# serycjon/MFT

Measured on AMD Instinct MI355X. Metric: tracked frames/sec at 512x512, 12 RAFT iters; flow EPE vs reference, higher is better.
Workload: dtype f32 (update-block products as split fp16 x 3 on the fp16 matrix cores, fp32 accumulation; error per product <= ~2^-23, see DESIGN.md section 4 and parity below); 1 GPU; MFT.track on synthetic 512x512 video, deltas [inf,1,2,4,8,16,32], 7/7.00/7 (min/mean/max) flow pairs per timed frame, 12 RAFT iters, seeded synthetic weights (BASELINE.json configs[1]); parallelism=single GPU, frames_resident_in_hbm=True, preroll_frames=32

## Files before the change

### include/mftx.h

```cpp
#ifndef MFTX_H
#define MFTX_H

#include <stddef.h>
#include <stdint.h>

#ifdef __cplusplus
extern "C" {
#endif

#define MFTX_VERSION 400

#define MFTX_E_ARG (-1)
#define MFTX_E_ALIGN (-2)
#define MFTX_E_WORKSPACE (-3)
#define MFTX_E_STATE (-4)

#define MFTX_MAX_CANDIDATES 16

int mftx_version(void);
const char *mftx_last_error_string(void);

#define MFTX_PROFILE_CATEGORIES 14
int mftx_profile_begin(void);
int mftx_profile_end(double *ms, double *work, long long *count, int n);

int mftx_corr_pyramid(const float *f1, const float *f2, int P, int C, int h, int w,
                      float *lvl0, float *lvl1, float *lvl2, float *lvl3, void *stream);
int mftx_corr_pyramid_split(const float *f1, const float *f2, int P, int C, int h, int w,
                            float *lvl0, float *lvl1, float *lvl2, float *lvl3, float *f2_scratch, void *stream);
int mftx_corr_pyramid_layout(int h, int w, long long *stride, int *block_grid);

int mftx_corr_lookup(const float *lvl0, const float *lvl1, const float *lvl2, const float *lvl3,
                     const float *coords, int P, int h, int w, int r,
                     float *out, int ld_out, void *stream);

#define MFTX_LOOKUP_CONVC1_WEIGHT_BYTES 393216
int mftx_pack_lookup_convc1_weights(const float *wpk, int ld_w, void *wfused, void *stream);
int mftx_corr_lookup_convc1(const float *lvl0, const float *lvl1, const float *lvl2, const float *lvl3,
                            const float *coords, int P, int h, int w, const void *wfused, const float *bias,
                            float *out, int ld_out, int out_split, void *stream);

#define MFTX_FLOW_BRANCH_WEIGHT_BYTES 352256
int mftx_pack_flow_branch_weights(const float *w98, const float *w2pk, void *wflow, void *stream);
int mftx_flow_branch(const float *coords, int P, int h, int w, const void *wflow, const float *b1, const float *b2,
                     float *out, int ld_out, float *hx, int ld_hx, void *stream);

int mftx_fmap_pyramid(const float *f2, int P, int C, int h, int w, float *lvl1, float *lvl2, float *lvl3, void *stream);
int mftx_corr_lookup_ondemand(const float *f1, const float *f2l0, const float *f2l1, const float *f2l2, const float *f2l3,
                              const float *coords, int P, int C, int h, int w, int r,
                              float *out, int ld_out, void *stream);

typedef struct mftx_conv_desc {
    const float *a0; int lda0; int c0;
    const float *a1; int lda1; int c1;
    const float *wpk; const float *bias;
    float *out; int ldo;
    int P, h, w;
    int N;
    int kh, kw;
    int act;
    float out_scale;
    const float *addend; int ld_addend;
    int stride, hin, win, pad_y, pad_x, residual_mode;
    int arith;
    int a_split, out_split;
} mftx_conv_desc;
#define MFTX_ARITH_F32 0
#define MFTX_ARITH_SPLIT 1
int mftx_conv2d(const mftx_conv_desc *d, void *stream);
int mftx_conv2d_tile(const mftx_conv_desc *d, int tile, void *stream);

int mftx_pack_tile_conv_weights(const float *wpk, int N, int taps, int cin, int cin_pad, void *wtile, void *stream);
int mftx_tile_conv2d(const mftx_conv_desc *d, const void *wtile, void *stream);
#define MFTX_OU_HEADS_WTILE_BYTES 6635520
int mftx_pack_ou_heads_weights(const float *w1pk, int cin_pad, const float *w2pk, void *wtile, void *wproj, void *stream);
int mftx_ou_heads(const float *a_split, int lda, int P, int h, int w, const void *wtile, const float *b1, const void *wproj, const float *b2,
                  float *T, float *out, int ld_out, void *stream);
int mftx_gru_half(const float *h_in, int ld_hin, const float *motion, int ld_mo, const void *wzr, const void *wq, const float *pre_zr,
                  const float *pre_q, float *z, const float *hf_in, float *hf_out, float *h_out, int ld_hout, int P, int h, int w, int pass,
                  void *stream);
int mftx_tile_conv_fills_chip(int P, int h, int w);
#define MFTX_FLOW_HEAD_WEIGHT_BYTES 32768
int mftx_pack_flow_head_weights(const float *w2pk, void *wproj, void *stream);
int mftx_flow_head(const float *hsplit, int ld_h, int P, int h, int w, const void *wtile, const float *b1, const void *wproj,
                   const float *b2, float *T, float *delta, float *coords, void *stream);
int mftx_split_weights(const float *wpk, void *out, long long n_floats, void *stream);
#define MFTX_SPLIT_LIMIT 65504.0f
int mftx_count_not_below(const float *x, long long n, float limit, unsigned *count, void *stream);

typedef struct mftx_raft mftx_raft;
#define MFTX_RAFT_NUM_WEIGHTS 34
int mftx_raft_create(const float *const *weights, int n_weights, mftx_raft **out);
void mftx_raft_destroy(mftx_raft *r);
size_t mftx_raft_workspace_bytes(int P, int h, int w);
int mftx_raft_set_ondemand(mftx_raft *r, int on);
int mftx_raft_set_split_weights(mftx_raft *r, const void *const *split, int n);
int mftx_raft_arith(const mftx_raft *r);
int mftx_raft_set_lookup_fused(mftx_raft *r, const void *wfused);
int mftx_raft_set_flow_fused(mftx_raft *r, const void *wflow);
int mftx_raft_set_tile_weights(mftx_raft *r, const void *const *tile, int n);
int mftx_raft_set_flow_head(mftx_raft *r, const void *wproj);
int mftx_raft_set_ou_heads(mftx_raft *r, const void *wtile, const void *wproj);
int mftx_raft_set_coords_trace(mftx_raft *r, float *trace);
#define MFTX_RAFT_OPT_FORK 0
#define MFTX_RAFT_OPT_PRESPLIT 1
#define MFTX_RAFT_OPT_GROUP 2
#define MFTX_RAFT_OPT_FUSE_LOOKUP 3
#define MFTX_RAFT_OPT_GRAPH 4
#define MFTX_RAFT_OPT_FUSE_FLOW 5
#define MFTX_RAFT_OPT_TILE_CONV 6
#define MFTX_RAFT_OPT_FUSE_HEAD 7
#define MFTX_RAFT_OPT_TILE_VOLUME 8
#define MFTX_RAFT_OPT_FUSE_GRU 9
#define MFTX_RAFT_OPT_TILE_CELLS 10
#define MFTX_RAFT_OPT_FUSE_OU 11
#define MFTX_RAFT_OPT_TILE_CONV2P 12
int mftx_raft_set_option(mftx_raft *r, int option, int value);
#define MFTX_RAFT_PLAN_FIELDS 14
#define MFTX_FLOW_FUSED 0
#define MFTX_FLOW_SIDE 1
#define MFTX_FLOW_FIRST 2
#define MFTX_FLOW_AFTER_LOOKUP 3
#define MFTX_FLOW_WITH_LOOKUP 4
int mftx_raft_plan(const mftx_raft *r, int P, int h, int w, int ctx_supplied, int *out, int n);
int mftx_raft_set_nonfinite_counter(mftx_raft *r, unsigned *counter);
int mftx_raft_clear_graphs(mftx_raft *r);
int mftx_raft_graph_stats(const mftx_raft *r, unsigned long long *captures, unsigned long long *replays);
size_t mftx_raft_workspace_bytes_for(const mftx_raft *r, int P, int h, int w);
int mftx_raft_workspace_layout(int P, int h, int w, size_t *offsets, int n);
int mftx_raft_workspace_layout_for(const mftx_raft *r, int P, int h, int w, size_t *offsets, int n);
int mftx_raft_refine(mftx_raft *r, int P, int h, int w, int iters,
                     const float *fmap1, const float *fmap2, const float *net, const float *inp,
                     const float *flow_init,
                     int pad_left, int pad_right, int pad_top, int pad_bottom,
                     float *flow, float *occl, float *sigma, float *packed, float *flow_lr,
                     void *workspace, size_t workspace_bytes, void *stream);
int mftx_raft_refine_gather(mftx_raft *r, int P, int h, int w, int iters, const float *const *fmap1,
                            const float *const *fmap2, const float *const *net, const float *const *inp,
                            const float *flow_init, int pad_left, int pad_right, int pad_top, int pad_bottom,
                            float *flow, float *occl, float *sigma, float *packed, float *flow_lr_out,
                            void *workspace, size_t workspace_bytes, void *stream);
size_t mftx_raft_frame_prepare_bytes(int h, int w);
int mftx_raft_frame_prepare(mftx_raft *r, int h, int w, const float *fmap, const float *inp, float *ctx_zr1, float *ctx_q1,
                            float *ctx_zr2, float *ctx_q2, void *fmap_split, void *scratch, size_t scratch_bytes, void *stream);
int mftx_raft_refine_gather_ex(mftx_raft *r, int P, int h, int w, int iters, const float *const *fmap1,
                               const float *const *fmap2, const float *const *net, const float *const *inp,
                               const float *const *ctx_parts, const void *const *fmap1_split, const void *fmap2_split,
                               const float *flow_init, int pad_left, int pad_right, int pad_top, int pad_bottom,
                               float *flow, float *occl, float *sigma, float *packed, float *flow_lr_out,
                               void *workspace, size_t workspace_bytes, void *stream);
int mftx_volume_query_split(const float *in, void *out, long long n_floats, void *stream);

typedef struct mftx_encoder mftx_encoder;
int mftx_encoder_create(const float *const *weights, int n_weights, int instance_norm, mftx_encoder **out);
int mftx_encoder_set_split_weights(mftx_encoder *e, const void *const *split, int n);
int mftx_encoder_set_graph(mftx_encoder *e, int on);
void mftx_encoder_destroy(mftx_encoder *e);
size_t mftx_encoder_workspace_bytes(int H0, int W0);
int mftx_encoder_forward(mftx_encoder *e, const uint8_t *img, int H0, int W0, float *out0, float *out1,
                         void *workspace, size_t workspace_bytes, void *stream);
int mftx_encoder_prep(const uint8_t *img, int H0, int W0, float *out, void *stream);
size_t mftx_instance_norm_workspace_bytes(int C);
int mftx_instance_norm(float *x, int rows, int C, const float *res, int mode, int split, void *workspace,
                       size_t workspace_bytes, void *stream);

int mftx_convex_upsample(const float *flow_lr, const float *ou, int ld_ou, const float *mask,
                         int P, int h, int w,
                         int pad_left, int pad_right, int pad_top, int pad_bottom,
                         float *flow, float *occl, float *sigma, float *packed, void *stream);

int mftx_chain(const float *flowL, const float *occlL, const float *sigmaL,
               const float *flowR, const float *occlR, const float *sigmaR,
               int H, int W, float *flowO, float *occlO, float *sigmaO, void *stream);

int mftx_warp_backward(const float *flow, const float *img, int C, int H, int W, float *out, void *stream);

int mftx_select(int K, const float *const *flow, const float *const *occl, const float *const *sigma,
                float thr, int H, int W,
                float *flowO, float *occlO, float *sigmaO, int8_t *chosen, void *stream);

int mftx_chain_select(int K,
                      const float *const *flowL, const float *const *occlL, const float *const *sigmaL,
                      const float *const *flowR, const float *const *occlR, const float *const *sigmaR,
                      float thr, int H, int W,
                      float *flowO, float *occlO, float *sigmaO, int8_t *chosen, void *stream);

int mftx_chain_select_packed(int K,
                             const float *const *flowL, const float *const *occlL, const float *const *sigmaL,
                             const float *const *packedR,
                             float thr, int H, int W,
                             float *flowO, float *occlO, float *sigmaO, int8_t *chosen, void *stream);

int mftx_chain_select_multi(int T, const int *K,
                            const float *const *flowL, const float *const *occlL, const float *const *sigmaL,
                            const float *const *packedR,
                            float thr, int H, int W,
                            float *const *flowO, float *const *occlO, float *const *sigmaO, int8_t *const *chosen,
                            void *stream);

int mftx_sample_points(int T, const float *const *flow, const float *const *occl, const float *const *sigma,
                       int H, int W, int N, const int *tmpl, const float *xy,
                       float *table, long long row_stride, int column, void *stream);

#define MFTX_SPLAT_F32 0
#define MFTX_SPLAT_U8 1
int mftx_splat_forward(const float *flow, const void *img, int img_dtype, const uint8_t *mask, int C, int H, int W,
                       int S, int V, long long *acc, void *stream);

int mftx_splat_resolve(long long *acc, int C, int H, int W, int V, float fill, int clear, float *out, void *stream);

int mftx_overlay_edit(const float *flow, const float *occl, const uint8_t *edit, const uint8_t *frame, int H, int W,
                      int S, float alpha_div, long long *acc, uint8_t *out, void *stream);

int mftx_overlay_dots(const uint8_t *frame, uint8_t *out, int H, int W, const float *table, long long row_stride,
                      int N, double radius, int b, int g, int r, void *stream);

size_t mftx_quantize_workspace_bytes(void);
int mftx_quantize_u16(const float *x, long long n, uint16_t *q, float *lohi,
                      void *workspace, size_t workspace_bytes, void *stream);
int mftx_dequantize_u16(const uint16_t *q, long long n, float lo, float hi, float *x, void *stream);

size_t mftx_trackstore_workspace_bytes(void);
int mftx_trackstore_append(const float *flow, const float *occl, const float *sigma, int H, int W,
                           uint16_t *packed, float *lohi, void *workspace, size_t workspace_bytes, void *stream);

size_t mftx_trackstore_append_multi_workspace_bytes(int T);
int mftx_trackstore_append_multi(int T, const float *const *flow, const float *const *occl, const float *const *sigma,
                                 int H, int W, uint16_t *const *packed, float *const *lohi,
                                 void *workspace, size_t workspace_bytes, void *stream);

int mftx_trackstore_unpack(const uint16_t *packed, const float *lohi, int H, int W,
                           float *flow, float *occl, float *sigma, void *stream);

int mftx_trackstore_query(const uint16_t *const *chunks, const float *const *lohi_chunks, int n_chunks, int frames_per_chunk,
                          const int *slots, int T, int H, int W, int N, const float *xy,
                          float *table, long long row_stride, int column0, void *stream);

int mftx_trackstore_locate(const uint16_t *const *frames, const float *const *lohis, const int *group_start, int G,
                           const int *order, const int *group_of, int H, int W, int N, const float *xy,
                           float occlusion_threshold, unsigned long long *keys, float *table, int *cell, void *stream);

int mftx_trackstore_invert(const uint16_t *const *frames, const float *const *lohis, int G, int H, int W,
                           float occlusion_threshold, unsigned long long *keys ,
                           float *table, int *cell, void *stream);

int mftx_trackstore_invert_atlas(const uint16_t *const *frames, const float *const *lohis, const int *first_of ,
                                 const int *rank_of , int G, int J, int H, int W, float occlusion_threshold,
                                 unsigned long long *keys , float *table, int *cell, int *entry, void *stream);

int mftx_trackstore_flow_from(const float *table, const int *entry, const int *row_of, const uint16_t *const *frames,
                              const float *const *lohis, int n_ranks, int R, int T, int H, int W, int columns_per_block,
                              float *flow, float *occl, float *sigma, void *stream);

int mftx_trackstore_flow_from_best(const float *tables, const int *cells, const int *rank_of, const int *row_of,
                                   const uint16_t *const *frames, const float *const *lohis, int E, int R, int T, int H, int W,
                                   float occlusion_threshold, int columns_per_block, float *flow, float *occl, float *sigma,
                                   int *entry, void *stream);

int mftx_copy_bytes(const void *src, void *dst, long long n, void *stream);

int mftx_png_unfilter(uint8_t *rows, int height, int row_bytes, int bpp);

#ifdef __cplusplus
}
#endif
#endif
```

### mft_amd/_lib.py

```python
from __future__ import annotations

import ctypes as C
import os
from pathlib import Path

_HERE = Path(__file__).resolve().parent
LIB_PATH = _HERE / "libmftx.so"

MAX_CANDIDATES = 16
NUM_RAFT_WEIGHTS = 34
LOOKUP_CONVC1_WEIGHT_BYTES = 393216
FLOW_BRANCH_WEIGHT_BYTES = 352256
FLOW_HEAD_WEIGHT_BYTES = 32768
OU_HEADS_WTILE_BYTES = 6635520
SPLIT_LIMIT = 65504.0


class ConvDesc(C.Structure):
    _fields_ = [("a0", C.c_void_p), ("lda0", C.c_int), ("c0", C.c_int),
                ("a1", C.c_void_p), ("lda1", C.c_int), ("c1", C.c_int),
                ("wpk", C.c_void_p), ("bias", C.c_void_p),
                ("out", C.c_void_p), ("ldo", C.c_int),
                ("P", C.c_int), ("h", C.c_int), ("w", C.c_int),
                ("N", C.c_int), ("kh", C.c_int), ("kw", C.c_int),
                ("act", C.c_int), ("out_scale", C.c_float),
                ("addend", C.c_void_p), ("ld_addend", C.c_int),
                ("stride", C.c_int), ("hin", C.c_int), ("win", C.c_int), ("pad_y", C.c_int), ("pad_x", C.c_int),
                ("residual_mode", C.c_int), ("arith", C.c_int), ("a_split", C.c_int), ("out_split", C.c_int)]


_PP = C.POINTER(C.c_void_p)

SIGNATURES = {
    "mftx_version": (C.c_int, []),
    "mftx_last_error_string": (C.c_char_p, []),
    "mftx_profile_begin": (C.c_int, []),
    "mftx_profile_end": (C.c_int, [C.POINTER(C.c_double), C.POINTER(C.c_double), C.POINTER(C.c_longlong), C.c_int]),
    "mftx_corr_pyramid": (C.c_int, [C.c_void_p, C.c_void_p, C.c_int, C.c_int, C.c_int, C.c_int,
                                    C.c_void_p, C.c_void_p, C.c_void_p, C.c_void_p, C.c_void_p]),
    "mftx_corr_pyramid_split": (C.c_int, [C.c_void_p, C.c_void_p, C.c_int, C.c_int, C.c_int, C.c_int,
                                          C.c_void_p, C.c_void_p, C.c_void_p, C.c_void_p, C.c_void_p, C.c_void_p]),
    "mftx_corr_pyramid_layout": (C.c_int, [C.c_int, C.c_int, C.POINTER(C.c_longlong), C.POINTER(C.c_int)]),
    "mftx_corr_lookup": (C.c_int, [C.c_void_p] * 5 + [C.c_int] * 4 + [C.c_void_p, C.c_int, C.c_void_p]),
    "mftx_fmap_pyramid": (C.c_int, [C.c_void_p] + [C.c_int] * 4 + [C.c_void_p] * 4),
    "mftx_corr_lookup_ondemand": (C.c_int, [C.c_void_p] * 6 + [C.c_int] * 5 + [C.c_void_p, C.c_int, C.c_void_p]),
    "mftx_raft_set_ondemand": (C.c_int, [C.c_void_p, C.c_int]),
    "mftx_raft_workspace_bytes_for": (C.c_size_t, [C.c_void_p, C.c_int, C.c_int, C.c_int]),
    "mftx_conv2d": (C.c_int, [C.POINTER(ConvDesc), C.c_void_p]),
    "mftx_conv2d_tile": (C.c_int, [C.POINTER(ConvDesc), C.c_int, C.c_void_p]),
    "mftx_encoder_set_split_weights": (C.c_int, [C.c_void_p, _PP, C.c_int]),
    "mftx_raft_set_split_weights": (C.c_int, [C.c_void_p, _PP, C.c_int]),
    "mftx_raft_arith": (C.c_int, [C.c_void_p]),
    "mftx_raft_set_lookup_fused": (C.c_int, [C.c_void_p, C.c_void_p]),
    "mftx_raft_set_flow_fused": (C.c_int, [C.c_void_p, C.c_void_p]),
    "mftx_raft_set_tile_weights": (C.c_int, [C.c_void_p, _PP, C.c_int]),
    "mftx_raft_set_flow_head": (C.c_int, [C.c_void_p, C.c_void_p]),
    "mftx_raft_set_ou_heads": (C.c_int, [C.c_void_p, C.c_void_p, C.c_void_p]),
    "mftx_pack_ou_heads_weights": (C.c_int, [C.c_void_p, C.c_int, C.c_void_p, C.c_void_p, C.c_void_p, C.c_void_p]),
    "mftx_ou_heads": (C.c_int, [C.c_void_p, C.c_int, C.c_int, C.c_int, C.c_int, C.c_void_p, C.c_void_p, C.c_void_p, C.c_void_p, C.c_void_p,
                                C.c_void_p, C.c_int, C.c_void_p]),
    "mftx_pack_flow_head_weights": (C.c_int, [C.c_void_p, C.c_void_p, C.c_void_p]),
    "mftx_flow_head": (C.c_int, [C.c_void_p, C.c_int, C.c_int, C.c_int, C.c_int] + [C.c_void_p] * 8),
    "mftx_pack_tile_conv_weights": (C.c_int, [C.c_void_p, C.c_int, C.c_int, C.c_int, C.c_int, C.c_void_p, C.c_void_p]),
    "mftx_tile_conv2d": (C.c_int, [C.POINTER(ConvDesc), C.c_void_p, C.c_void_p]),
    "mftx_pack_flow_branch_weights": (C.c_int, [C.c_void_p, C.c_void_p, C.c_void_p, C.c_void_p]),
    "mftx_flow_branch": (C.c_int, [C.c_void_p, C.c_int, C.c_int, C.c_int, C.c_void_p, C.c_void_p, C.c_void_p, C.c_void_p,
                                   C.c_int, C.c_void_p, C.c_int, C.c_void_p]),
    "mftx_raft_set_option": (C.c_int, [C.c_void_p, C.c_int, C.c_int]),
    "mftx_raft_plan": (C.c_int, [C.c_void_p, C.c_int, C.c_int, C.c_int, C.c_int, C.POINTER(C.c_int), C.c_int]),
    "mftx_raft_set_coords_trace": (C.c_int, [C.c_void_p, C.c_void_p]),
    "mftx_gru_half": (C.c_int, [C.c_void_p, C.c_int, C.c_void_p, C.c_int, C.c_void_p, C.c_void_p, C.c_void_p, C.c_void_p, C.c_void_p, C.c_void_p,
                                C.c_void_p, C.c_void_p, C.c_int, C.c_int, C.c_int, C.c_int, C.c_int, C.c_void_p]),
    "mftx_tile_conv_fills_chip": (C.c_int, [C.c_int, C.c_int, C.c_int]),
    "mftx_raft_clear_graphs": (C.c_int, [C.c_void_p]),
    "mftx_raft_set_nonfinite_counter": (C.c_int, [C.c_void_p, C.c_void_p]),
    "mftx_raft_graph_stats": (C.c_int, [C.c_void_p, C.POINTER(C.c_ulonglong), C.POINTER(C.c_ulonglong)]),
    "mftx_pack_lookup_convc1_weights": (C.c_int, [C.c_void_p, C.c_int, C.c_void_p, C.c_void_p]),
    "mftx_corr_lookup_convc1": (C.c_int, [C.c_void_p] * 5 + [C.c_int] * 3 + [C.c_void_p, C.c_void_p, C.c_void_p,
                                                                            C.c_int, C.c_int, C.c_void_p]),
    "mftx_split_weights": (C.c_int, [C.c_void_p, C.c_void_p, C.c_longlong, C.c_void_p]),
    "mftx_count_not_below": (C.c_int, [C.c_void_p, C.c_longlong, C.c_float, C.c_void_p, C.c_void_p]),
    "mftx_raft_create": (C.c_int, [_PP, C.c_int, C.POINTER(C.c_void_p)]),
    "mftx_raft_destroy": (None, [C.c_void_p]),
    "mftx_raft_workspace_bytes": (C.c_size_t, [C.c_int, C.c_int, C.c_int]),
    "mftx_raft_workspace_layout": (C.c_int, [C.c_int, C.c_int, C.c_int, C.POINTER(C.c_size_t), C.c_int]),
    "mftx_raft_workspace_layout_for": (C.c_int, [C.c_void_p, C.c_int, C.c_int, C.c_int, C.POINTER(C.c_size_t), C.c_int]),
    "mftx_raft_refine": (C.c_int, [C.c_void_p, C.c_int, C.c_int, C.c_int, C.c_int,
                                   C.c_void_p, C.c_void_p, C.c_void_p, C.c_void_p, C.c_void_p,
                                   C.c_int, C.c_int, C.c_int, C.c_int,
                                   C.c_void_p, C.c_void_p, C.c_void_p, C.c_void_p, C.c_void_p,
                                   C.c_void_p, C.c_size_t, C.c_void_p]),
    "mftx_raft_refine_gather": (C.c_int, [C.c_void_p, C.c_int, C.c_int, C.c_int, C.c_int,
                                          _PP, _PP, _PP, _PP, C.c_void_p,
                                          C.c_int, C.c_int, C.c_int, C.c_int,
                                          C.c_void_p, C.c_void_p, C.c_void_p, C.c_void_p, C.c_void_p,
                                          C.c_void_p, C.c_size_t, C.c_void_p]),
    "mftx_raft_refine_gather_ex": (C.c_int, [C.c_void_p, C.c_int, C.c_int, C.c_int, C.c_int,
                                             _PP, _PP, _PP, _PP, _PP, _PP, C.c_void_p, C.c_void_p,
                                             C.c_int, C.c_int, C.c_int, C.c_int,
                                             C.c_void_p, C.c_void_p, C.c_void_p, C.c_void_p, C.c_void_p,
                                             C.c_void_p, C.c_size_t, C.c_void_p]),
    "mftx_raft_frame_prepare_bytes": (C.c_size_t, [C.c_int, C.c_int]),
    "mftx_raft_frame_prepare": (C.c_int, [C.c_void_p, C.c_int, C.c_int] + [C.c_void_p] * 8 + [C.c_size_t, C.c_void_p]),
    "mftx_volume_query_split": (C.c_int, [C.c_void_p, C.c_void_p, C.c_longlong, C.c_void_p]),
    "mftx_encoder_create": (C.c_int, [_PP, C.c_int, C.c_int, C.POINTER(C.c_void_p)]),
    "mftx_encoder_destroy": (None, [C.c_void_p]),
    "mftx_encoder_set_graph": (C.c_int, [C.c_void_p, C.c_int]),
    "mftx_encoder_workspace_bytes": (C.c_size_t, [C.c_int, C.c_int]),
    "mftx_encoder_forward": (C.c_int, [C.c_void_p, C.c_void_p, C.c_int, C.c_int, C.c_void_p, C.c_void_p,
                                       C.c_void_p, C.c_size_t, C.c_void_p]),
    "mftx_encoder_prep": (C.c_int, [C.c_void_p, C.c_int, C.c_int, C.c_void_p, C.c_void_p]),
    "mftx_instance_norm_workspace_bytes": (C.c_size_t, [C.c_int]),
    "mftx_instance_norm": (C.c_int, [C.c_void_p, C.c_int, C.c_int, C.c_void_p, C.c_int, C.c_int, C.c_void_p, C.c_size_t, C.c_void_p]),
    "mftx_convex_upsample": (C.c_int, [C.c_void_p, C.c_void_p, C.c_int, C.c_void_p] + [C.c_int] * 7
                             + [C.c_void_p] * 5),
    "mftx_chain": (C.c_int, [C.c_void_p] * 6 + [C.c_int, C.c_int] + [C.c_void_p] * 4),
    "mftx_warp_backward": (C.c_int, [C.c_void_p, C.c_void_p, C.c_int, C.c_int, C.c_int, C.c_void_p, C.c_void_p]),
    "mftx_select": (C.c_int, [C.c_int, _PP, _PP, _PP, C.c_float, C.c_int, C.c_int] + [C.c_void_p] * 5),
    "mftx_chain_select": (C.c_int, [C.c_int] + [_PP] * 6 + [C.c_float, C.c_int, C.c_int] + [C.c_void_p] * 5),
    "mftx_chain_select_packed": (C.c_int, [C.c_int] + [_PP] * 4 + [C.c_float, C.c_int, C.c_int] + [C.c_void_p] * 5),
    "mftx_chain_select_multi": (C.c_int, [C.c_int, C.POINTER(C.c_int)] + [_PP] * 4 + [C.c_float, C.c_int, C.c_int] + [_PP] * 4
                                + [C.c_void_p]),
    "mftx_sample_points": (C.c_int, [C.c_int, _PP, _PP, _PP, C.c_int, C.c_int, C.c_int, C.c_void_p, C.c_void_p,
                                     C.c_void_p, C.c_longlong, C.c_int, C.c_void_p]),
    "mftx_splat_forward": (C.c_int, [C.c_void_p, C.c_void_p, C.c_int, C.c_void_p, C.c_int, C.c_int, C.c_int, C.c_int, C.c_int,
                                     C.c_void_p, C.c_void_p]),
    "mftx_splat_resolve": (C.c_int, [C.c_void_p, C.c_int, C.c_int, C.c_int, C.c_int, C.c_float, C.c_int, C.c_void_p, C.c_void_p]),
    "mftx_overlay_edit": (C.c_int, [C.c_void_p, C.c_void_p, C.c_void_p, C.c_void_p, C.c_int, C.c_int, C.c_int, C.c_float,
                                    C.c_void_p, C.c_void_p, C.c_void_p]),
    "mftx_overlay_dots": (C.c_int, [C.c_void_p, C.c_void_p, C.c_int, C.c_int, C.c_void_p, C.c_longlong, C.c_int, C.c_double,
                                    C.c_int, C.c_int, C.c_int, C.c_void_p]),
    "mftx_quantize_workspace_bytes": (C.c_size_t, []),
    "mftx_quantize_u16": (C.c_int, [C.c_void_p, C.c_longlong, C.c_void_p, C.c_void_p, C.c_void_p, C.c_size_t, C.c_void_p]),
    "mftx_dequantize_u16": (C.c_int, [C.c_void_p, C.c_longlong, C.c_float, C.c_float, C.c_void_p, C.c_void_p]),
    "mftx_trackstore_workspace_bytes": (C.c_size_t, []),
    "mftx_trackstore_append": (C.c_int, [C.c_void_p, C.c_void_p, C.c_void_p, C.c_int, C.c_int, C.c_void_p, C.c_void_p,
                                         C.c_void_p, C.c_size_t, C.c_void_p]),
    "mftx_trackstore_append_multi_workspace_bytes": (C.c_size_t, [C.c_int]),
    "mftx_trackstore_append_multi": (C.c_int, [C.c_int, _PP, _PP, _PP, C.c_int, C.c_int, _PP, _PP, C.c_void_p, C.c_size_t,
                                               C.c_void_p]),
    "mftx_trackstore_invert_atlas": (C.c_int, [C.c_void_p, C.c_void_p, C.c_void_p, C.c_void_p, C.c_int, C.c_int, C.c_int, C.c_int,
                                               C.c_float, C.c_void_p, C.c_void_p, C.c_void_p, C.c_void_p, C.c_void_p]),
    "mftx_trackstore_flow_from": (C.c_int, [C.c_void_p, C.c_void_p, C.c_void_p, C.c_void_p, C.c_void_p, C.c_int, C.c_int, C.c_int,
                                            C.c_int, C.c_int, C.c_int, C.c_void_p, C.c_void_p, C.c_void_p, C.c_void_p]),
    "mftx_trackstore_flow_from_best": (C.c_int, [C.c_void_p] * 6 + [C.c_int] * 5 + [C.c_float, C.c_int] + [C.c_void_p] * 5),
    "mftx_trackstore_unpack": (C.c_int, [C.c_void_p, C.c_void_p, C.c_int, C.c_int, C.c_void_p, C.c_void_p, C.c_void_p,
                                         C.c_void_p]),
    "mftx_trackstore_query": (C.c_int, [_PP, _PP, C.c_int, C.c_int, C.c_void_p, C.c_int, C.c_int, C.c_int, C.c_int, C.c_void_p,
                                        C.c_void_p, C.c_longlong, C.c_int, C.c_void_p]),
    "mftx_trackstore_locate": (C.c_int, [C.c_void_p, C.c_void_p, C.c_void_p, C.c_int, C.c_void_p, C.c_void_p, C.c_int, C.c_int,
                                         C.c_int, C.c_void_p, C.c_float, C.c_void_p, C.c_void_p, C.c_void_p, C.c_void_p]),
    "mftx_trackstore_invert": (C.c_int, [C.c_void_p, C.c_void_p, C.c_int, C.c_int, C.c_int, C.c_float, C.c_void_p, C.c_void_p,
                                         C.c_void_p, C.c_void_p]),
    "mftx_png_unfilter":(C.c_int, [C.c_void_p, C.c_int, C.c_int, C.c_int]),
    "mftx_copy_bytes": (C.c_int, [C.c_void_p, C.c_void_p, C.c_longlong, C.c_void_p]),
}

_lib = None


class MftxError(RuntimeError):
    pass


def load():
    global _lib
    if _lib is not None:
        return _lib
    path = Path(os.environ.get("MFTX_LIB", LIB_PATH))
    if not path.exists():
        raise MftxError(f"{path} not found: build it with `python -c 'import __graft_entry__ as g; g.build()'` "
                        "(there is no CPU fallback for the MFT hot path)")
    lib = C.CDLL(str(path))
    for name, (res, args) in SIGNATURES.items():
        fn = getattr(lib, name)
        fn.restype = res
        fn.argtypes = args
    _lib = lib
    return lib


def check(code, what):
    if code != 0:
        msg = load().mftx_last_error_string().decode(errors="replace")
        raise MftxError(f"{what} failed ({code}): {msg}")


def ptr_array(ptrs):
    arr = (C.c_void_p * len(ptrs))(*ptrs)
    return C.cast(arr, _PP), arr
```

### mft_amd/csrc/common.h

```cpp
#pragma once
#include <hip/hip_runtime.h>
#include <cstdarg>
#include <cstdio>
#include <cstdint>
#include <cstdlib>
#include "../../include/mftx.h"

namespace mftx {

void set_error(const char *fmt, ...);

inline int fail(int code, const char *fmt, ...) {
    char buf[512];
    va_list ap;
    va_start(ap, fmt);
    vsnprintf(buf, sizeof buf, fmt, ap);
    va_end(ap);
    set_error("%s", buf);
    return code;
}

inline int check_launch(const char *what) {
    hipError_t e = hipGetLastError();
    if (e != hipSuccess) {
        set_error("%s: %s", what, hipGetErrorString(e));
        return (int)e;
    }
    return 0;
}

inline int tune_env(const char *name, int dflt) {
#ifdef MFTX_TUNING
    const char *e = getenv(name);
    return e ? atoi(e) : dflt;
#else
    (void)name;
    return dflt;
#endif
}

inline bool aligned16(const void *p) { return (reinterpret_cast<uintptr_t>(p) & 15u) == 0; }
inline int cdiv(int a, int b) { return (a + b - 1) / b; }
inline int round_up(int a, int b) { return cdiv(a, b) * b; }

struct PyramidLayout {
    int h[4], w[4];
    int hb[2], wb[2];
    int sbh, sbw;
    long long stride[4];
};
inline PyramidLayout pyramid_layout(int h, int w) {
    PyramidLayout L;
    for (int l = 0; l < 4; ++l) { L.h[l] = h >> l; L.w[l] = w >> l; }
    L.sbh = (h + 7) / 8; L.sbw = (w + 15) / 16;
    L.hb[0] = 2 * L.sbh; L.wb[0] = 2 * L.sbw; L.hb[1] = L.sbh; L.wb[1] = L.sbw;
    L.stride[0] = (long long)L.hb[0] * L.wb[0] * 32;
    L.stride[1] = (long long)L.hb[1] * L.wb[1] * 32;
    L.stride[2] = ((long long)L.h[2] * L.w[2] + 3) / 4 * 4;
    L.stride[3] = ((long long)L.h[3] * L.w[3] + 3) / 4 * 4;
    return L;
}

__host__ __device__ inline int split_row_offset(int c) { return (c >> 3) * 32 + (c & 7) * 2; }
#ifdef __HIPCC__
__device__ __forceinline__ unsigned split_halves(float v) {
    const _Float16 h = (_Float16)v;
    const _Float16 l = (_Float16)((v - (float)h) * 2048.f);
    return (unsigned)__builtin_bit_cast(unsigned short, h) | ((unsigned)__builtin_bit_cast(unsigned short, l) << 16);
}
__device__ __forceinline__ void store_split_pairwise(float *row, int c, float v, bool store) {
    const unsigned mine = split_halves(v);
    const unsigned other = (unsigned)__shfl_xor((int)mine, 1);
    const bool odd = (c & 1) != 0;
    const unsigned word = odd ? ((other >> 16) | (mine & 0xffff0000u)) : ((mine & 0xffffu) | (other << 16));
    char *dst = reinterpret_cast<char *>(row) + split_row_offset(c & ~1) + (odd ? 16 : 0);
    if (store) *reinterpret_cast<unsigned *>(dst) = word;
}
__device__ __forceinline__ float4 load_split4(const float *row, int c) {
    const char *src = reinterpret_cast<const char *>(row) + split_row_offset(c);
    const uint2 h = *reinterpret_cast<const uint2 *>(src), l = *reinterpret_cast<const uint2 *>(src + 16);
    auto dec = [](unsigned hh, unsigned ll, int hi) {
        const _Float16 a = __builtin_bit_cast(_Float16, (unsigned short)(hi ? hh >> 16 : hh));
        const _Float16 b = __builtin_bit_cast(_Float16, (unsigned short)(hi ? ll >> 16 : ll));
        return (float)a + (float)b * (1.f / 2048.f);
    };
    return make_float4(dec(h.x, l.x, 0), dec(h.x, l.x, 1), dec(h.y, l.y, 0), dec(h.y, l.y, 1));
}
__device__ __forceinline__ void store_split4v(float *row, int c, float4 v) {
    const unsigned a = split_halves(v.x), b = split_halves(v.y), cc = split_halves(v.z), d = split_halves(v.w);
    char *dst = reinterpret_cast<char *>(row) + split_row_offset(c);
    *reinterpret_cast<uint2 *>(dst) = make_uint2((a & 0xffffu) | (b << 16), (cc & 0xffffu) | (d << 16));
    *reinterpret_cast<uint2 *>(dst + 16) = make_uint2((a >> 16) | (b & 0xffff0000u), (cc >> 16) | (d & 0xffff0000u));
}
#endif
__host__ __device__ inline float relu_keep_nan(float v) { return v < 0.f ? 0.f : v; }
int launch_conv(const mftx_conv_desc &d, hipStream_t s, int tile = -1);
int launch_conv_pair(const mftx_conv_desc &a, const mftx_conv_desc &b, hipStream_t s);
struct GruEpilogue {
    int mode;
    float *hx;
    int ld_hx;
    float *z;
    float *rh;
    float *hf = nullptr;
    int ld_hf = 0;
};
int launch_conv_gru(const mftx_conv_desc &d, const GruEpilogue &g, hipStream_t s);
int launch_split_weights(const float *wpk, void *out, long long n_floats, hipStream_t s);
bool conv_small_applicable(const mftx_conv_desc &d);
int launch_conv_small(const mftx_conv_desc &d, hipStream_t s, float *accum = nullptr, int ld_accum = 0);
int launch_corr_pyramid(const float *f1, const float *f2, int P, int C, int h, int w, float *const lvl[4], hipStream_t s,
                        float *f2_split = nullptr, int tile_resident = 1);
bool volume_tile_applicable(int C);
constexpr int MFTX_MAX_GATHER = 16;
struct PairPtrs { const float *p[MFTX_MAX_GATHER]; };
int launch_volume_tile(const float *f1, const float *f2s, int P, int h, int w, float *const lvl[4], hipStream_t s,
                       const PairPtrs *f1p = nullptr, long long f2_bstride = -1, bool f1_split = false);
int launch_volume_query_split(const float *in, void *out, long long n_floats, hipStream_t s);
int launch_corr_lookup(const float *const lvl[4], const float *coords, int P, int h, int w,
                       float *out, int ld_out, hipStream_t s);
int launch_pack_lookup_convc1(const float *w, int ld_w, void *out, hipStream_t s);
bool lookup_convc1_applicable(int P, int h, int w, int ld_out);
int launch_lookup_convc1(const float *const lvl[4], const float *coords, int P, int h, int w, const void *wf,
                         const float *bias, float *out, int ld_out, int out_split, hipStream_t s);
int launch_pack_flow_branch(const float *w98, const float *w2pk, void *out, hipStream_t s);
int launch_flow_branch(const float *coords, int P, int h, int w, const void *wf, const float *b1, const float *b2, float *out,
                       int ld_out, float *hx, int ld_hx, hipStream_t s, const float *T = nullptr, const float *b2h = nullptr,
                       float *coords_out = nullptr, float *delta_out = nullptr);
struct TileConvLaunch {
    const float *a0; int lda0;
    const float *a1; int lda1;
    int cin;
    const void *wf;
    const float *bias;
    const float *addend; int ld_addend;
    float *out; int ldo; int out_split;
    float *z, *rh, *hf, *hx; int ld_hf, ld_hx;
    const void *wproj; float *tout;
    int P, h, w, N, kh, kw, epi;
    int cells;
};
struct GruHalfLaunch {
    const float *h_in; int ld_hin; const float *mo; int ld_mo;
    const void *wzr, *wq;
    const float *pre_zr, *pre_q;
    const float *const *ctx;
    float *z; const float *hf_in; float *hf_out;
    float *h_out; int ld_hout;
    int P, h, w, pass;
    int cells;
};
int launch_gru_half(const GruHalfLaunch &d, hipStream_t s);
int launch_pack_flow_head(const float *w2pk, void *out, hipStream_t s);
int launch_pack_tile_conv2p(const float *wpk, int N, int cin_pad, void *out, hipStream_t s);
int launch_tile_conv2p(const float *a, int lda, const void *wf, const float *bias, float *out, int ldo, int n_valid, int P, int h, int w, int cells,
                       hipStream_t s);
constexpr size_t OU_HEAD_WTILE_BYTES = 8ull * 5 * 9 * 9 * 128 * 16, OU_HEAD_WPROJ_BYTES = 32768;
int launch_pack_ou_head(const float *w1pk, int cin_pad, const float *w2pk, void *wtile, void *wproj, hipStream_t s);
struct OuGather { const float *hx, *corr; int ld_corr; const float *coords1, *delta; float *flow_lr; };
int launch_ou_heads(const float *a, int lda, int P, int h, int w, const void *wtile, const float *b1, const void *wproj, const float *b2, float *T,
                    float *out, int ld_out, int cells, hipStream_t s, const OuGather *ga = nullptr);
int launch_flow_head_sum(const float *T, const float *b2, float *delta, const float *coords_in, float *coords_out, int P, int h, int w, hipStream_t s);
bool tile_conv_applicable(int kh, int kw, int cin, int N);
bool tile_conv_small_tiles_fill(int P, int h, int w);
bool tile_conv_fills_chip(int P, int h, int w, int kh, int kw);
int launch_pack_tile_conv(const float *wpk, int N, int taps, int cin, int cin_pad, void *out, hipStream_t s);
int launch_tile_conv(const TileConvLaunch &d, hipStream_t s);
int launch_fmap_pyramid(const float *f2, int P, int C, int h, int w, float *const lvl[3], hipStream_t s);
int launch_corr_ondemand(const float *f1, const float *const f2lvl[4], const float *coords, int P, int h, int w,
                         float *out, int ld_out, hipStream_t s);
int launch_convex_upsample(const float *flow_lr, const float *ou, int ld_ou, const float *mask,
                           int P, int h, int w, int pl, int pr, int pt, int pb,
                           float *flow, float *occl, float *sigma, float *packed, hipStream_t s, unsigned *nonfinite = nullptr);

}
```

### mft_amd/csrc/raft_engine.hip

```cpp
#include "common.h"
#include "profile.h"
#include "motion_front.h"
#include "graph_cache.h"
#include <cstdlib>
#include <new>

namespace mftx {


struct InitGather { int on; PairPtrs netp, inpp; };
struct CtxTable { const float **table; const float *own[4]; int supplied; PairPtrs parts[4]; };
__global__ void init_state_kernel(const float *__restrict__ net, const float *__restrict__ inp,
                                  const float *__restrict__ flow_init, float *hx, float *hf, float *coords1, int M, int h,
                                  int w, InitGather ga, CtxTable ct) {
    const long long i = (long long)blockIdx.x * blockDim.x + threadIdx.x;
    if (i >= (long long)M * 64) return;
    if (ct.table != nullptr && i < (long long)(M / (h * w)) * 4) {
        const int b = (int)(i >> 2), k = (int)(i & 3);
        ct.table[i] = ct.supplied ? ct.parts[k].p[b] : ct.own[k] + (long long)b * h * w * ((k & 1) ? 128 : 256);
    }
    const int m = (int)(i >> 6), q = (int)(i & 63);
    if (ga.on) {
        const int b = m / (h * w);
        net = ga.netp.p[b] - (long long)b * h * w * 128;
        inp = ga.inpp.p[b] - (long long)b * h * w * 128;
    }
    const float4 v = (q < 32) ? reinterpret_cast<const float4 *>(net)[(long long)m * 32 + q]
                              : reinterpret_cast<const float4 *>(inp)[(long long)m * 32 + (q - 32)];
    if (hf != nullptr) {
        store_split4v(hx + (long long)m * 384, 4 * q, v);
        if (q < 32) reinterpret_cast<float4 *>(hf + (long long)m * 128)[q] = v;
    } else {
        reinterpret_cast<float4 *>(hx + (long long)m * 384)[q] = v;
    }
    if (q == 0) {
        const int rem = m % (h * w);
        float cx = (float)(rem % w), cy = (float)(rem / w);
        if (flow_init != nullptr) {
            cx += flow_init[2 * (long long)m];
            cy += flow_init[2 * (long long)m + 1];
        }
        coords1[2 * (long long)m] = cx;
        coords1[2 * (long long)m + 1] = cy;
    }
}

__global__ __launch_bounds__(256) void convf1_kernel(ConvF1Args q) {
    __shared__ __attribute__((aligned(16))) float patch[2][7][48];
    const int half = threadIdx.x >> 7;
    convf1_strip(q, blockIdx.x * 2 + half, patch[half], threadIdx.x & 127);
}

__global__ __launch_bounds__(256) void lookup_convf1_kernel(LookupArgs lp, ConvF1Args q, int lookup_blocks, int f1_blocks) {
    __shared__ __attribute__((aligned(16))) float patch[2][7][48];
    const int total = lookup_blocks + f1_blocks;
    const int b = blockIdx.x;
    const int f_lo = (int)((long long)b * f1_blocks / total), f_hi = (int)((long long)(b + 1) * f1_blocks / total);
    if (f_hi > f_lo) {
        const int half = threadIdx.x >> 7;
        convf1_strip(q, f_lo * 2 + half, patch[half], threadIdx.x & 127);
    } else {
        lookup_block_body<2>(lp, b - f_lo, lookup_blocks);
    }
}

__global__ void ou_gather_kernel(const float *__restrict__ hx, const float *__restrict__ corr, int ld_corr,
                                 const float *__restrict__ coords1, const float *__restrict__ delta,
                                 float *__restrict__ ouin, float *__restrict__ flow_lr, int M, int h, int w, int split) {
    const long long i = (long long)blockIdx.x * blockDim.x + threadIdx.x;
    if (i >= (long long)M * 178) return;
    const int m = (int)(i / 178), q = (int)(i - (long long)m * 178);
    float4 v;
    if (split) {
        if (q < 64) v = load_split4(hx + (long long)m * 384, 4 * q);
        else if (q < 145) v = reinterpret_cast<const float4 *>(corr + (long long)m * ld_corr)[q - 64];
        else if (q == 145) {
            const int rem = m % (h * w);
            const float fx = coords1[2 * (long long)m] - (float)(rem % w);
            const float fy = coords1[2 * (long long)m + 1] - (float)(rem / w);
            v = make_float4(fx, fy, delta[2 * (long long)m], delta[2 * (long long)m + 1]);
            flow_lr[2 * (long long)m] = fx;
            flow_lr[2 * (long long)m + 1] = fy;
        } else v = load_split4(hx + (long long)m * 384 + 256, 4 * (q - 146));
        store_split4v(ouin + (long long)m * 712, 4 * q, v);
        return;
    }
    if (q < 64) v = reinterpret_cast<const float4 *>(hx + (long long)m * 384)[q];
    else if (q < 145) v = reinterpret_cast<const float4 *>(corr + (long long)m * ld_corr)[q - 64];
    else if (q == 145) {
        const int rem = m % (h * w);
        const float fx = coords1[2 * (long long)m] - (float)(rem % w);
        const float fy = coords1[2 * (long long)m + 1] - (float)(rem / w);
        v = make_float4(fx, fy, delta[2 * (long long)m], delta[2 * (long long)m + 1]);
        flow_lr[2 * (long long)m] = fx;
        flow_lr[2 * (long long)m + 1] = fy;
    } else v = reinterpret_cast<const float4 *>(hx + (long long)m * 384 + 256)[q - 146];
    reinterpret_cast<float4 *>(ouin + (long long)m * 712)[q] = v;
}

enum WeightSlot {
    W_CONVC1, B_CONVC1, W_CONVC2, B_CONVC2, W_CONVF1, B_CONVF1, W_CONVF2, B_CONVF2, W_CONV, B_CONV,
    W_ZR1_DYN, W_ZR1_INP, B_ZR1, W_Q1_DYN, W_Q1_INP, B_Q1, W_ZR2_DYN, W_ZR2_INP, B_ZR2, W_Q2_DYN, W_Q2_INP, B_Q2,
    W_FH1, B_FH1, W_FH2, B_FH2, W_MASK0, B_MASK0, W_MASK2, B_MASK2,
    W_OU1, B_OU1, W_OU2, B_OU2, W_COUNT
};

struct Workspace {
    float *lvl[4];
    float *f2l[3];
    float *coords1, *corr, *cor1, *corflo, *flo1, *hx, *z, *rh, *fh, *delta, *mask, *ouin, *ouh, *ou, *flow_lr;
    float *pre_zr[2], *pre_q[2];
    float *f2s;
    float *hf;
    float *hb, *hfb;
    const float **ctx;
    int ld_corr;
    size_t bytes;
};

static Workspace carve(void *base, int P, int h, int w, bool ondemand = false, bool split = false) {
    Workspace ws{};
    const size_t N = (size_t)h * w, M = (size_t)P * N;
    size_t off = 0;
    auto take = [&](size_t floats) {
        float *p = base ? reinterpret_cast<float *>(static_cast<char *>(base) + off) : nullptr;
        off += (floats * sizeof(float) + 255) & ~size_t(255);
        return p;
    };
    const PyramidLayout L = pyramid_layout(h, w);
    for (int l = 0; l < 4; ++l) ws.lvl[l] = take(ondemand ? 0 : M * (size_t)L.stride[l]);
    for (int l = 1; l < 4; ++l) ws.f2l[l - 1] = take(ondemand ? (size_t)P * (h >> l) * (w >> l) * 256 : 0);
    ws.coords1 = take(M * 2);
    ws.ld_corr = 324;
    ws.corr = take(M * ws.ld_corr);
    ws.cor1 = take(M * 256);
    ws.corflo = take(M * 256);
    ws.flo1 = take(M * 128);
    ws.hx = take(M * 384);
    ws.z = take(M * 128);
    ws.rh = take(M * 128);
    ws.fh = take(M * 256);
    ws.delta = take(M * 2);
    ws.mask = take(M * 576);
    ws.ouin = take(M * 712);
    ws.ouh = take(M * 256);
    ws.ou = take(M * 4);
    ws.flow_lr = take(M * 2);
    for (int pass = 0; pass < 2; ++pass) { ws.pre_zr[pass] = take(M * 256); ws.pre_q[pass] = take(M * 128); }
    ws.f2s = take(ondemand || !split ? 0 : M * 256);
    ws.hf = take(split ? M * 128 : 0);
    ws.hb = take(split ? M * 128 : 0);
    ws.hfb = take(split ? M * 128 : 0);
    ws.ctx = reinterpret_cast<const float **>(take(split ? (size_t)P * 8 : 0));
    ws.bytes = off;
    return ws;
}

}

using namespace mftx;

static constexpr uint32_t RAFT_MAGIC = 0x4d465458;
struct mftx_raft {
    uint32_t magic = RAFT_MAGIC;
    int ondemand = 0;
    int arith = MFTX_ARITH_F32;
    const float *w[W_COUNT] = {};
    const float *wg[W_COUNT] = {};
    hipStream_t side = nullptr;
    hipEvent_t ev_fork = nullptr, ev_join = nullptr;
    float *coords_trace = nullptr;
    GraphCache *graphs = nullptr;
    const void *wfused = nullptr;
    const void *wflow = nullptr;
    const void *wproj = nullptr;
    const void *wt[W_COUNT] = {};
    const void *wou = nullptr, *wouproj = nullptr;
    int opt[13] = { -1,  1,  1,  1,  1,  1,  1,
                    1,  1,  1,  0,  1,  1};
    unsigned *nonfinite = nullptr;
};
static_assert(MFTX_RAFT_OPT_TILE_CONV2P == 12, "mftx_raft::opt lists one default per option");
static constexpr int GEMM_SLOTS[] = {W_CONVC1, W_CONVC2, W_CONVF2, W_CONV, W_ZR1_DYN, W_ZR1_INP, W_Q1_DYN, W_Q1_INP,
                                     W_ZR2_DYN, W_ZR2_INP, W_Q2_DYN, W_Q2_INP, W_FH1, W_MASK0, W_MASK2, W_OU1};

extern "C" int mftx_raft_create(const float *const *weights, int n_weights, mftx_raft **out) {
    if (!weights || !out) return fail(MFTX_E_ARG, "raft_create: null pointer");
    if (n_weights != W_COUNT) return fail(MFTX_E_ARG, "raft_create: expected %d weight tensors, got %d", (int)W_COUNT, n_weights);
    for (int i = 0; i < W_COUNT; ++i) {
        if (!weights[i]) return fail(MFTX_E_ARG, "raft_create: weight %d is null", i);
        if (!aligned16(weights[i])) return fail(MFTX_E_ALIGN, "raft_create: weight %d not 16-byte aligned", i);
    }
    mftx_raft *r = new (std::nothrow) mftx_raft;
    if (!r) return fail(MFTX_E_ARG, "raft_create: out of host memory");
    r->graphs = new (std::nothrow) GraphCache;
    for (int i = 0; i < W_COUNT; ++i) r->w[i] = r->wg[i] = weights[i];
    *out = r;
    return 0;
}

extern "C" void mftx_raft_destroy(mftx_raft *r) {
    if (r && r->magic == RAFT_MAGIC) {
        r->magic = 0;
        if (r->ev_fork) (void)hipEventDestroy(r->ev_fork);
        if (r->ev_join) (void)hipEventDestroy(r->ev_join);
        if (r->side) (void)hipStreamDestroy(r->side);
        delete r->graphs;
        delete r;
    }
}

static int ensure_side_stream(mftx_raft *r) {
    if (r->side) return 0;
    hipError_t e = hipStreamCreateWithFlags(&r->side, hipStreamNonBlocking);
    if (e == hipSuccess) e = hipEventCreateWithFlags(&r->ev_fork, hipEventDisableTiming);
    if (e == hipSuccess) e = hipEventCreateWithFlags(&r->ev_join, hipEventDisableTiming);
    if (e != hipSuccess) return fail((int)e, "raft_refine: side stream: %s", hipGetErrorString(e));
    return 0;
}

extern "C" size_t mftx_raft_workspace_bytes(int P, int h, int w) {
    if (P <= 0 || h <= 0 || w <= 0) return 0;
    return carve(nullptr, P, h, w).bytes;
}

extern "C" int mftx_raft_set_ondemand(mftx_raft *r, int on) {
    if (!r || r->magic != RAFT_MAGIC) return fail(MFTX_E_STATE, "raft_set_ondemand: bad handle");
    r->ondemand = on ? 1 : 0;
    if (r->graphs) r->graphs->clear();
    return 0;
}

extern "C" int mftx_raft_set_split_weights(mftx_raft *r, const void *const *split, int n) {
    if (!r || r->magic != RAFT_MAGIC) return fail(MFTX_E_STATE, "raft_set_split_weights: bad handle");
    if (r->graphs) r->graphs->clear();
    if (!split) {
        for (int i = 0; i < W_COUNT; ++i) r->wg[i] = r->w[i];
        r->arith = MFTX_ARITH_F32;
        return 0;
    }
    if (n != W_COUNT) return fail(MFTX_E_ARG, "raft_set_split_weights: expected %d slots, got %d", (int)W_COUNT, n);
    for (int slot : GEMM_SLOTS) {
        if (!split[slot]) return fail(MFTX_E_ARG, "raft_set_split_weights: slot %d (a GEMM layer) is null", slot);
        if (!aligned16(split[slot])) return fail(MFTX_E_ALIGN, "raft_set_split_weights: slot %d not 16-byte aligned", slot);
    }
    for (int slot : GEMM_SLOTS) r->wg[slot] = static_cast<const float *>(split[slot]);
    r->arith = MFTX_ARITH_SPLIT;
    return 0;
}

extern "C" int mftx_raft_set_lookup_fused(mftx_raft *r, const void *wfused) {
    if (!r || r->magic != RAFT_MAGIC) return fail(MFTX_E_STATE, "raft_set_lookup_fused: bad handle");
    if (wfused && !aligned16(wfused)) return fail(MFTX_E_ALIGN, "raft_set_lookup_fused: weights not 16-byte aligned");
    r->wfused = wfused;
    if (r->graphs) r->graphs->clear();
    return 0;
}

extern "C" int mftx_raft_set_flow_fused(mftx_raft *r, const void *wflow) {
    if (!r || r->magic != RAFT_MAGIC) return fail(MFTX_E_STATE, "raft_set_flow_fused: bad handle");
    if (wflow && !aligned16(wflow)) return fail(MFTX_E_ALIGN, "raft_set_flow_fused: weights not 16-byte aligned");
    r->wflow = wflow;
    if (r->graphs) r->graphs->clear();
    return 0;
}

extern "C" int mftx_raft_set_tile_weights(mftx_raft *r, const void *const *tile, int n) {
    if (!r || r->magic != RAFT_MAGIC) return fail(MFTX_E_STATE, "raft_set_tile_weights: bad handle");
    if (r->graphs) r->graphs->clear();
    if (!tile) { for (int i = 0; i < W_COUNT; ++i) r->wt[i] = nullptr; return 0; }
    if (n != W_COUNT) return fail(MFTX_E_ARG, "raft_set_tile_weights: expected %d slots, got %d", (int)W_COUNT, n);
    for (int i = 0; i < W_COUNT; ++i)
        if (tile[i] && !aligned16(tile[i])) return fail(MFTX_E_ALIGN, "raft_set_tile_weights: slot %d not 16-byte aligned", i);
    for (int i = 0; i < W_COUNT; ++i) r->wt[i] = tile[i];
    return 0;
}

extern "C" int mftx_raft_set_flow_head(mftx_raft *r, const void *wproj) {
    if (!r || r->magic != RAFT_MAGIC) return fail(MFTX_E_STATE, "raft_set_flow_head: bad handle");
    if (wproj && !aligned16(wproj)) return fail(MFTX_E_ALIGN, "raft_set_flow_head: weights not 16-byte aligned");
    r->wproj = wproj;
    if (r->graphs) r->graphs->clear();
    return 0;
}

extern "C" int mftx_raft_set_ou_heads(mftx_raft *r, const void *wtile, const void *wproj) {
    if (!r || r->magic != RAFT_MAGIC) return fail(MFTX_E_STATE, "raft_set_ou_heads: bad handle");
    if ((wtile == nullptr) != (wproj == nullptr)) return fail(MFTX_E_ARG, "raft_set_ou_heads: both weight streams, or neither");
    if (wtile && (!aligned16(wtile) || !aligned16(wproj))) return fail(MFTX_E_ALIGN, "raft_set_ou_heads: weights not 16-byte aligned");
    r->wou = wtile; r->wouproj = wproj;
    if (r->graphs) r->graphs->clear();
    return 0;
}

extern "C" int mftx_raft_set_coords_trace(mftx_raft *r, float *trace) {
    if (!r || r->magic != RAFT_MAGIC) return fail(MFTX_E_STATE, "raft_set_coords_trace: bad handle");
    r->coords_trace = trace;
    return 0;
}

extern "C" int mftx_raft_clear_graphs(mftx_raft *r) {
    if (!r || r->magic != RAFT_MAGIC) return fail(MFTX_E_STATE, "raft_clear_graphs: bad handle");
    if (r->graphs) r->graphs->clear();
    return 0;
}

extern "C" int mftx_raft_set_nonfinite_counter(mftx_raft *r, unsigned *counter) {
    if (!r || r->magic != RAFT_MAGIC) return fail(MFTX_E_STATE, "raft_set_nonfinite_counter: bad handle");
    if (counter && (reinterpret_cast<uintptr_t>(counter) & 3)) return fail(MFTX_E_ALIGN, "raft_set_nonfinite_counter: counter not 4-byte aligned");
    r->nonfinite = counter;
    return 0;
}

extern "C" int mftx_raft_set_option(mftx_raft *r, int option, int value) {
    if (!r || r->magic != RAFT_MAGIC) return fail(MFTX_E_STATE, "raft_set_option: bad handle");
    if (option < 0 || option > MFTX_RAFT_OPT_TILE_CONV2P) return fail(MFTX_E_ARG, "raft_set_option: unknown option %d", option);
    r->opt[option] = value;
    if (r->graphs) r->graphs->clear();
    return 0;
}

extern "C" int mftx_raft_arith(const mftx_raft *r) {
    return (r && r->magic == RAFT_MAGIC) ? r->arith : -1;
}

extern "C" size_t mftx_raft_workspace_bytes_for(const mftx_raft *r, int P, int h, int w) {
    if (!r || r->magic != RAFT_MAGIC || P <= 0 || h <= 0 || w <= 0) return 0;
    return carve(nullptr, P, h, w, r->ondemand != 0, r->arith == MFTX_ARITH_SPLIT).bytes;
}

static int workspace_layout(const mftx_raft *r, int P, int h, int w, size_t *offsets, int n) {
    if (P <= 0 || h <= 0 || w <= 0 || !offsets || n != 19) return fail(MFTX_E_ARG, "workspace_layout: need 19 slots");
    char *base = reinterpret_cast<char *>(uintptr_t(1) << 40);
    Workspace ws = carve(base, P, h, w, r && r->ondemand != 0, r && r->arith == MFTX_ARITH_SPLIT);
    float *ptrs[19] = {ws.lvl[0], ws.lvl[1], ws.lvl[2], ws.lvl[3], ws.coords1, ws.corr, ws.cor1, ws.corflo, ws.flo1,
                       ws.hx, ws.z, ws.rh, ws.fh, ws.delta, ws.mask, ws.ouin, ws.ouh, ws.ou, ws.flow_lr};
    for (int i = 0; i < 19; ++i) offsets[i] = (size_t)(reinterpret_cast<char *>(ptrs[i]) - base);
    return 0;
}
extern "C" int mftx_raft_workspace_layout(int P, int h, int w, size_t *offsets, int n) {
    return workspace_layout(nullptr, P, h, w, offsets, n);
}
extern "C" int mftx_raft_workspace_layout_for(const mftx_raft *r, int P, int h, int w, size_t *offsets, int n) {
    if (!r || r->magic != RAFT_MAGIC) return fail(MFTX_E_STATE, "workspace_layout_for: bad handle");
    return workspace_layout(r, P, h, w, offsets, n);
}

#define TRY(expr) do { int _e = (expr); if (_e) return _e; } while (0)

enum FlowSchedule { FLOW_FUSED = MFTX_FLOW_FUSED, FLOW_SIDE = MFTX_FLOW_SIDE, FLOW_FIRST = MFTX_FLOW_FIRST, FLOW_AFTER_LOOKUP = MFTX_FLOW_AFTER_LOOKUP,
                    FLOW_WITH_LOOKUP = MFTX_FLOW_WITH_LOOKUP };

struct RefinePlan {
    bool SP, fuse_lookup, tiles_on, gru_fused, ctx_supplied, two_pass;
    FlowSchedule flow;
    bool pair_second;
    bool head_fused, defer_update, ou_fused, ou_materialised, use_graph, side_stream;
};

static RefinePlan refine_plan(const mftx_raft &r, int P, int h, int w, bool gather_has_ctx, bool prof, bool trace) {
    const int *opt = r.opt;
    const bool split = r.arith == MFTX_ARITH_SPLIT, ondemand = r.ondemand != 0;
    RefinePlan p{};
    p.SP = split && opt[MFTX_RAFT_OPT_PRESPLIT] != 0;
    p.fuse_lookup = p.SP && !ondemand && r.wfused != nullptr && opt[MFTX_RAFT_OPT_FUSE_LOOKUP] != 0 && lookup_convc1_applicable(P, h, w, 256);
    p.tiles_on = p.SP && opt[MFTX_RAFT_OPT_TILE_CONV] != 0 && (opt[MFTX_RAFT_OPT_TILE_CONV] == 2 ||
                 (tile_conv_fills_chip(P, h, w, 3, 3) && tile_conv_fills_chip(P, h, w, 1, 5) && tile_conv_fills_chip(P, h, w, 5, 1)));
    auto tile_w = [&](int slot) { return p.tiles_on && r.wt[slot] != nullptr; };
    p.gru_fused = tile_w(W_ZR1_DYN) && tile_w(W_Q1_DYN) && tile_w(W_ZR2_DYN) && tile_w(W_Q2_DYN) && opt[MFTX_RAFT_OPT_FUSE_GRU] != 0;
    p.ctx_supplied = gather_has_ctx && p.gru_fused;
    p.two_pass = p.tiles_on && opt[MFTX_RAFT_OPT_TILE_CONV2P] != 0 && r.wt[W_CONVC2] && r.wt[W_CONV];
    const bool grouped = opt[MFTX_RAFT_OPT_GROUP] != 0;
    const int fork = opt[MFTX_RAFT_OPT_FORK];
    const bool fuse_flow = p.SP && r.wflow != nullptr && opt[MFTX_RAFT_OPT_FUSE_FLOW] != 0 && grouped;
    const bool serial = fuse_flow || prof || !grouped || (split && (fork == 0 || fork == 2));
    const bool forked = !serial && split;
    const bool flow_first = !fuse_flow && serial && p.fuse_lookup && fork == 2 && !prof && grouped;
    const bool lookup_alone = p.fuse_lookup || prof || !grouped || ondemand;
    p.flow = fuse_flow ? FLOW_FUSED : forked ? FLOW_SIDE : flow_first ? FLOW_FIRST : lookup_alone ? FLOW_AFTER_LOOKUP : FLOW_WITH_LOOKUP;
    p.pair_second = !forked && grouped && r.arith == MFTX_ARITH_F32;
    p.head_fused = tile_w(W_FH1) && r.wproj != nullptr && opt[MFTX_RAFT_OPT_FUSE_HEAD] != 0;
    p.defer_update = p.head_fused && fuse_flow && opt[MFTX_RAFT_OPT_FUSE_HEAD] != 2 && !trace;
    p.ou_fused = p.tiles_on && r.wou != nullptr && opt[MFTX_RAFT_OPT_FUSE_OU] != 0;
    p.ou_materialised = !p.ou_fused || opt[MFTX_RAFT_OPT_FUSE_OU] == 2;
    p.use_graph = r.graphs && opt[MFTX_RAFT_OPT_GRAPH] != 0 && !prof && !trace && !ondemand;
    p.side_stream = split && fork != 0;
    return p;
}

extern "C" int mftx_raft_plan(const mftx_raft *r, int P, int h, int w, int ctx_supplied, int *out, int n) {
    if (!r || r->magic != RAFT_MAGIC) return fail(MFTX_E_STATE, "raft_plan: bad handle");
    if (P <= 0 || h <= 0 || w <= 0) return fail(MFTX_E_ARG, "raft_plan: need P, h, w >= 1");
    if (!out || n != MFTX_RAFT_PLAN_FIELDS) return fail(MFTX_E_ARG, "raft_plan: need %d slots", MFTX_RAFT_PLAN_FIELDS);
    const RefinePlan p = refine_plan(*r, P, h, w, ctx_supplied != 0, prof_enabled(), r->coords_trace != nullptr);
    const int v[MFTX_RAFT_PLAN_FIELDS] = {p.SP, p.fuse_lookup, p.tiles_on, p.gru_fused, p.ctx_supplied, p.two_pass, (int)p.flow, p.pair_second,
                                          p.head_fused, p.defer_update, p.ou_fused, p.ou_materialised, p.use_graph, p.side_stream};
    for (int i = 0; i < n; ++i) out[i] = v[i];
    return 0;
}

struct RefineGather { PairPtrs f1, f2, net, inp; bool f2_shared; bool has_ctx, has_f1s; PairPtrs ctx[4], f1s; const float *f2s; };

struct Coords { float *cur, *alt; bool pending; };
struct Seg { const float *p; int ld, c; };
struct Out { float *p; int ld, N; };
enum { ACT_NONE, ACT_RELU, ACT_GRU_ZR, ACT_GRU_Q };

struct RefineCall {
    mftx_raft *r;
    const float *const *W, *const *G;
    RefinePlan plan;
    hipStream_t s;
    int P, h, w, iters;
    Workspace ws;
    const float *lv[4];
    const float *fmap1, *f2lv[4];
    float *flow_lr;

    mftx_conv_desc conv_desc(Seg a0, Seg a1, const float *wpk, const float *bias, Out out, int kh, int kw, int act) const {
        mftx_conv_desc d{};
        d.a0 = a0.p; d.lda0 = a0.ld; d.c0 = a0.c; d.a1 = a1.p; d.lda1 = a1.ld; d.c1 = a1.c;
        d.wpk = wpk; d.bias = bias; d.out = out.p; d.ldo = out.ld; d.N = out.N; d.P = P; d.h = h; d.w = w;
        d.kh = kh; d.kw = kw; d.act = act; d.out_scale = 1.f;
        return d;
    }
    mftx_conv_desc gemm(mftx_conv_desc d, bool a = true, bool o = false) const {
        d.arith = r->arith; d.a_split = plan.SP && a; d.out_split = plan.SP && o; return d;
    }
    TileConvLaunch tile_launch(int slot, const float *bias, Seg a0, Seg a1, int N, int kh, int kw, int epi) const {
        TileConvLaunch t{};
        t.a0 = a0.p; t.lda0 = a0.ld; t.a1 = a1.p; t.lda1 = a1.ld; t.cin = a1.p ? 256 : 128; t.wf = r->wt[slot]; t.bias = bias;
        t.P = P; t.h = h; t.w = w; t.N = N; t.kh = kh; t.kw = kw; t.epi = epi;
        t.cells = r->opt[MFTX_RAFT_OPT_TILE_CELLS];
        return t;
    }
    int conv_layer(int slot, const float *bias, Seg a0, Seg a1, Out out, int kh, int kw, int act, bool out_split, const GruEpilogue *g = nullptr,
                   const float *addend = nullptr, int ld_addend = 0) const {
        if (plan.tiles_on && r->wt[slot]) {
            TileConvLaunch t = tile_launch(slot, bias, a0, a1, out.N, kh, kw, act);
            t.addend = addend; t.ld_addend = ld_addend;
            if (!g) { t.out = out.p; t.ldo = out.ld; t.out_split = out_split ? 1 : 0; }
            else {
                t.z = g->z; t.hf = g->hf; t.ld_hf = g->ld_hf;
                if (act == ACT_GRU_ZR) t.rh = g->rh; else { t.hx = g->hx; t.ld_hx = g->ld_hx; }
            }
            return launch_tile_conv(t, s);
        }
        mftx_conv_desc d = gemm(conv_desc(a0, a1, G[slot], bias, out, kh, kw, act), true, out_split);
        d.addend = addend; d.ld_addend = ld_addend;
        return g ? launch_conv_gru(d, *g, s) : launch_conv(d, s);
    }
    int context_parts(const float *inp, int ld, float *const zr[2], float *const q[2]) const {
        for (int pass = 0; pass < 2; ++pass) {
            const int kh = pass ? 5 : 1, kw = pass ? 1 : 5;
            TRY(conv_layer(pass ? W_ZR2_INP : W_ZR1_INP, W[pass ? B_ZR2 : B_ZR1], Seg{inp, ld, 128}, Seg{}, Out{zr[pass], 256, 256}, kh, kw, ACT_NONE, false));
            TRY(conv_layer(pass ? W_Q2_INP : W_Q1_INP, W[pass ? B_Q2 : B_Q1], Seg{inp, ld, 128}, Seg{}, Out{q[pass], 128, 128}, kh, kw, ACT_NONE, false));
        }
        return 0;
    }
    int volume(const float *fmap2, const RefineGather *gather) const {
        if (r->ondemand) return launch_fmap_pyramid(fmap2, P, 256, h, w, ws.f2l, s);
        if (!gather) return launch_corr_pyramid(fmap1, fmap2, P, 256, h, w, ws.lvl, s, r->arith == MFTX_ARITH_SPLIT ? ws.f2s : nullptr, r->opt[MFTX_RAFT_OPT_TILE_VOLUME]);
        const long long pair_floats = (long long)h * w * 256;
        const float *f2s = ws.f2s;
        if (gather->f2_shared && gather->f2s) f2s = gather->f2s;
        else if (gather->f2_shared) TRY(launch_split_weights(gather->f2.p[0], ws.f2s, pair_floats, s));
        else for (int b = 0; b < P; ++b) TRY(launch_split_weights(gather->f2.p[b], ws.f2s + b * pair_floats, pair_floats, s));
        return launch_volume_tile(nullptr, f2s, P, h, w, ws.lvl, s, gather->has_f1s ? &gather->f1s : &gather->f1, gather->f2_shared ? 0 : pair_floats,
                                  gather->has_f1s);
    }
    int init_state(const float *net, const float *inp, const float *flow_init, const RefineGather *gather) const {
        const int M = P * h * w;
        const long long slots = (long long)M * 64;
        ProfScope prof(PC_GLUE, s, 0);
        InitGather ga{};
        if (gather) { ga.on = 1; ga.netp = gather->net; ga.inpp = gather->inp; }
        CtxTable ct{};
        if (plan.gru_fused) {
            ct.table = ws.ctx;
            ct.own[0] = ws.pre_zr[0]; ct.own[1] = ws.pre_q[0]; ct.own[2] = ws.pre_zr[1]; ct.own[3] = ws.pre_q[1];
            ct.supplied = plan.ctx_supplied ? 1 : 0;
            if (plan.ctx_supplied) for (int k = 0; k < 4; ++k) ct.parts[k] = gather->ctx[k];
        }
        hipLaunchKernelGGL(init_state_kernel, dim3((unsigned)((slots + 255) / 256)), dim3(256), 0, s, net, inp,
                           flow_init, ws.hx, plan.SP ? ws.hf : nullptr, ws.coords1, M, h, w, ga, ct);
        return check_launch("init_state");
    }
    int conv256(int slot, const float *bias, const float *in, Out out, const mftx_conv_desc *pair = nullptr) const {
        if (plan.two_pass) return launch_tile_conv2p(in, 256, r->wt[slot], bias, out.p, out.ld, out.N, P, h, w, r->opt[MFTX_RAFT_OPT_TILE_CELLS], s);
        const mftx_conv_desc d = gemm(conv_desc(Seg{in, 256, 256}, Seg{}, G[slot], bias, out, 3, 3, ACT_RELU), true, true);
        return pair ? launch_conv_pair(d, *pair, s) : launch_conv(d, s);
    }
    int corr_branch(const float *coords, bool last, const ConvF1Args *f1 = nullptr, int f1_blocks = 0, const mftx_conv_desc *pair = nullptr) const {
        if (plan.flow == FLOW_WITH_LOOKUP) {
            const LookupArgs la = make_lookup_args(lv, coords, P, h, w, ws.corr, ws.ld_corr);
            const int lookup_blocks = cdiv(cdiv(la.cells, 2), LK_WAVES);
            hipLaunchKernelGGL(lookup_convf1_kernel, dim3(lookup_blocks + f1_blocks), dim3(256), 0, s, la, *f1, lookup_blocks, f1_blocks);
        } else {
            if (plan.fuse_lookup) {
                if (last && plan.flow != FLOW_SIDE) TRY(launch_corr_lookup(lv, coords, P, h, w, ws.corr, ws.ld_corr, s));
                TRY(launch_lookup_convc1(lv, coords, P, h, w, r->wfused, W[B_CONVC1], ws.cor1, 256, 1, s));
            } else if (r->ondemand) TRY(launch_corr_ondemand(fmap1, f2lv, coords, P, h, w, ws.corr, ws.ld_corr, s));
            else TRY(launch_corr_lookup(lv, coords, P, h, w, ws.corr, ws.ld_corr, s));
            if (f1) {
                ProfScope prof(PC_CONVF1, s, 2.0 * P * h * w * 128 * 98);
                hipLaunchKernelGGL(convf1_kernel, dim3(f1_blocks), dim3(256), 0, s, *f1);
            }
        }
        TRY(check_launch("lookup + convf1"));
        if (!plan.fuse_lookup)
            TRY(launch_conv(gemm(conv_desc(Seg{ws.corr, ws.ld_corr, ws.ld_corr}, Seg{}, G[W_CONVC1], W[B_CONVC1], Out{ws.cor1, 256, 256}, 1, 1, ACT_RELU), false, true), s));
        return conv256(W_CONVC2, W[B_CONVC2], ws.cor1, Out{ws.corflo, 256, 192}, pair);
    }
    int motion_encoder(Coords &x, bool last) const {
        const int strips = cdiv(w, F1_CELLS);
        const ConvF1Args f1{x.cur, W[W_CONVF1], W[B_CONVF1], ws.flo1, ws.hx, h, w, strips, P * h * strips, plan.SP ? 1 : 0};
        const int f1_blocks = cdiv(f1.n_strips, 2);
        const Out flo{ws.corflo + 192, 256, 64};
        const mftx_conv_desc f2 = gemm(conv_desc(Seg{ws.flo1, 128, 128}, Seg{}, G[W_CONVF2], W[B_CONVF2], flo, 3, 3, ACT_RELU), true, true);
        switch (plan.flow) {
        case FLOW_FUSED:
            if (x.pending) {
                TRY(launch_flow_branch(x.cur, P, h, w, r->wflow, W[B_CONVF1], W[B_CONVF2], flo.p, flo.ld, ws.hx, 384, s, ws.fh, W[B_FH2], x.alt, ws.delta));
                x = Coords{x.alt, x.cur, false};
            } else TRY(launch_flow_branch(x.cur, P, h, w, r->wflow, W[B_CONVF1], W[B_CONVF2], flo.p, flo.ld, ws.hx, 384, s));
            TRY(corr_branch(x.cur, last));
            break;
        case FLOW_SIDE:
            TRY(ensure_side_stream(r));
            if (hipEventRecord(r->ev_fork, s) != hipSuccess || hipStreamWaitEvent(r->side, r->ev_fork, 0) != hipSuccess)
                return fail(MFTX_E_STATE, "raft_refine: fork onto the side stream failed");
            hipLaunchKernelGGL(convf1_kernel, dim3(f1_blocks), dim3(256), 0, r->side, f1);
            TRY(check_launch("convf1"));
            TRY(launch_conv(f2, r->side));
            if (plan.fuse_lookup && last) TRY(launch_corr_lookup(lv, x.cur, P, h, w, ws.corr, ws.ld_corr, r->side));
            if (hipEventRecord(r->ev_join, r->side) != hipSuccess) return fail(MFTX_E_STATE, "raft_refine: join event failed");
            TRY(corr_branch(x.cur, last));
            if (hipStreamWaitEvent(s, r->ev_join, 0) != hipSuccess) return fail(MFTX_E_STATE, "raft_refine: join failed");
            break;
        case FLOW_FIRST:
            hipLaunchKernelGGL(convf1_kernel, dim3(f1_blocks), dim3(256), 0, s, f1);
            TRY(check_launch("convf1"));
            TRY(launch_conv(f2, s));
            TRY(corr_branch(x.cur, last));
            break;
        case FLOW_AFTER_LOOKUP: case FLOW_WITH_LOOKUP:
            TRY(corr_branch(x.cur, last, &f1, f1_blocks, plan.pair_second ? &f2 : nullptr));
            if (!plan.pair_second) TRY(launch_conv(f2, s));
            break;
        }
        return conv256(W_CONV, W[B_CONV], ws.corflo, Out{ws.hx + 256, 384, 126});
    }
    int gru() const {
        for (int pass = 0; pass < 2; ++pass) {
            const int kh = pass ? 5 : 1, kw = pass ? 1 : 5;
            const int szr = pass ? W_ZR2_DYN : W_ZR1_DYN, sq = pass ? W_Q2_DYN : W_Q1_DYN;
            if (plan.gru_fused) {
                GruHalfLaunch g{};
                g.h_in = pass ? ws.hb : ws.hx; g.ld_hin = pass ? 128 : 384; g.h_out = pass ? ws.hx : ws.hb; g.ld_hout = pass ? 384 : 128;
                g.mo = ws.hx + 256; g.ld_mo = 384; g.wzr = r->wt[szr]; g.wq = r->wt[sq]; g.pre_zr = ws.pre_zr[pass]; g.pre_q = ws.pre_q[pass]; g.ctx = ws.ctx;
                g.z = ws.z; g.hf_in = pass ? ws.hfb : ws.hf; g.hf_out = pass ? ws.hf : ws.hfb; g.P = P; g.h = h; g.w = w; g.pass = pass; g.cells = r->opt[MFTX_RAFT_OPT_TILE_CELLS];
                TRY(launch_gru_half(g, s));
                continue;
            }
            const Seg motion{ws.hx + 256, 384, 128};
            const GruEpilogue g1{1, ws.hx, 384, ws.z, ws.rh, plan.SP ? ws.hf : nullptr, 128}, g2{2, ws.hx, 384, ws.z, ws.rh, plan.SP ? ws.hf : nullptr, 128};
            TRY(conv_layer(szr, nullptr, Seg{ws.hx, 384, 128}, motion, Out{ws.z, 128, 256}, kh, kw, ACT_GRU_ZR, true, &g1, ws.pre_zr[pass], 256));
            TRY(conv_layer(sq, nullptr, Seg{ws.rh, 128, 128}, motion, Out{ws.hx, 384, 128}, kh, kw, ACT_GRU_Q, true, &g2, ws.pre_q[pass], 128));
        }
        return 0;
    }
    int flow_head(Coords &x, bool last) const {
        const Seg hidden{ws.hx, 384, 128};
        if (plan.head_fused) {
            TileConvLaunch t = tile_launch(W_FH1, W[B_FH1], hidden, Seg{}, 256, 3, 3, 4);
            t.wproj = r->wproj; t.tout = ws.fh;
            TRY(launch_tile_conv(t, s));
            if (!last && plan.defer_update) { x.pending = true; return 0; }
            float *dst = last ? ws.coords1 : x.cur;
            TRY(launch_flow_head_sum(ws.fh, W[B_FH2], ws.delta, x.cur, dst, P, h, w, s));
            x.cur = dst;
            return 0;
        }
        TRY(conv_layer(W_FH1, W[B_FH1], hidden, Seg{}, Out{ws.fh, 256, 256}, 3, 3, ACT_RELU, false));
        const mftx_conv_desc fh2 = conv_desc(Seg{ws.fh, 256, 256}, Seg{}, W[W_FH2], W[B_FH2], Out{ws.delta, 2, 2}, 3, 3, ACT_NONE);
        if (!conv_small_applicable(fh2)) return fail(MFTX_E_STATE, "raft_refine: flow-head layer does not fit the small-N kernel");
        return launch_conv_small(fh2, s, x.cur, 2);
    }
    int final_heads(const float *coords) const {
        const int M = P * h * w;
        TRY(conv_layer(W_MASK0, W[B_MASK0], Seg{ws.hx, 384, 128}, Seg{}, Out{ws.fh, 256, 256}, 3, 3, ACT_RELU, true));
        mftx_conv_desc mask2 = gemm(conv_desc(Seg{ws.fh, 256, 256}, Seg{}, G[W_MASK2], W[B_MASK2], Out{ws.mask, 576, 576}, 1, 1, ACT_NONE));
        mask2.out_scale = 0.25f;
        TRY(launch_conv(mask2, s));
        if (plan.ou_materialised) {
            const long long slots = (long long)M * 178;
            ProfScope prof(PC_GLUE, s, 0);
            hipLaunchKernelGGL(ou_gather_kernel, dim3((unsigned)((slots + 255) / 256)), dim3(256), 0, s, ws.hx,
                               ws.corr, ws.ld_corr, coords, ws.delta, ws.ouin, flow_lr, M, h, w, plan.SP ? 1 : 0);
            TRY(check_launch("ou_gather"));
        }
        if (plan.ou_fused) {
            const OuGather ga{ws.hx, ws.corr, ws.ld_corr, coords, ws.delta, flow_lr};
            return launch_ou_heads(plan.ou_materialised ? ws.ouin : nullptr, 712, P, h, w, r->wou, W[B_OU1], r->wouproj, W[B_OU2], ws.ouh, ws.ou, 4, r->opt[MFTX_RAFT_OPT_TILE_CELLS], s,
                                   plan.ou_materialised ? nullptr : &ga);
        }
        TRY(launch_conv(gemm(conv_desc(Seg{ws.ouin, 712, 712}, Seg{}, G[W_OU1], W[B_OU1], Out{ws.ouh, 256, 256}, 3, 3, ACT_RELU)), s));
        return launch_conv(conv_desc(Seg{ws.ouh, 256, 256}, Seg{}, W[W_OU2], W[B_OU2], Out{ws.ou, 4, 3}, 3, 3, ACT_NONE), s);
    }
    int core() const {
        const size_t n = (size_t)P * h * w * 2;
        float *trace = r->coords_trace;
        if (!plan.ctx_supplied) TRY(context_parts(ws.hx + 128, 384, ws.pre_zr, ws.pre_q));
        Coords x{ws.coords1, ws.flo1, false};
        for (int it = 0; it < iters; ++it) {
            const bool last = (it == iters - 1);
            if (trace && hipMemcpyAsync(trace + it * n, x.cur, n * 4, hipMemcpyDeviceToDevice, s) != hipSuccess)
                return fail(MFTX_E_STATE, "raft_refine: coords trace copy failed");
            TRY(motion_encoder(x, last));
            TRY(gru());
            TRY(flow_head(x, last));
        }
        if (trace && hipMemcpyAsync(trace + iters * n, x.cur, n * 4, hipMemcpyDeviceToDevice, s) != hipSuccess)
            return fail(MFTX_E_STATE, "raft_refine: coords trace copy failed");
        return final_heads(x.cur);
    }
};

static int refine_impl(mftx_raft *r, int P, int h, int w, int iters, const float *fmap1, const float *fmap2, const float *net,
                       const float *inp, const float *flow_init, int pad_left, int pad_right, int pad_top, int pad_bottom, float *flow, float *occl,
                       float *sigma, float *packed, float *flow_lr_out, void *workspace, size_t workspace_bytes, void *stream, const RefineGather *gather) {
    if (!r || r->magic != RAFT_MAGIC) return fail(MFTX_E_STATE, "raft_refine: bad handle");
    const bool planar = flow && occl && sigma;
    if (gather) { fmap1 = gather->f1.p[0]; fmap2 = gather->f2.p[0]; net = gather->net.p[0]; inp = gather->inp.p[0]; }
    if (!fmap1 || !fmap2 || !net || !inp || !workspace || (!planar && (flow || occl || sigma || !packed)))
        return fail(MFTX_E_ARG, "raft_refine: null pointer (outputs: flow + occl + sigma, or packed, or both)");
    if (P <= 0 || h < 16 || w < 16 || iters < 1)
        return fail(MFTX_E_ARG, "raft_refine: need P >= 1, h, w >= 16 (level 3 of the pyramid needs >= 2 cells), iters >= 1");
    if ((long long)P * h * w > (1ll << 24)) return fail(MFTX_E_ARG, "raft_refine: batch too large");
    if (!aligned16(fmap1) || !aligned16(fmap2) || !aligned16(net) || !aligned16(inp) || (reinterpret_cast<uintptr_t>(workspace) & 255))
        return fail(MFTX_E_ALIGN, "raft_refine: inputs must be 16-byte and the workspace 256-byte aligned");
    if (pad_left < 0 || pad_right < 0 || pad_top < 0 || pad_bottom < 0 || pad_left + pad_right >= 8 || pad_top + pad_bottom >= 8)
        return fail(MFTX_E_ARG, "raft_refine: bad padding");
    const RefinePlan plan = refine_plan(*r, P, h, w, gather && gather->has_ctx, prof_enabled(), r->coords_trace != nullptr);
    const Workspace ws = carve(workspace, P, h, w, r->ondemand != 0, r->arith == MFTX_ARITH_SPLIT);
    if (ws.bytes > workspace_bytes)
        return fail(MFTX_E_WORKSPACE, "raft_refine: workspace %zu < %zu bytes", workspace_bytes, ws.bytes);
    hipStream_t s = (hipStream_t)stream, caller = s;
    bool proxied = false;
    if (plan.use_graph && s == nullptr) {
        hipStream_t own = r->graphs->proxy.enter(s);
        if (own) { s = own; proxied = true; }
    }
    struct Leave { GraphCache *g; hipStream_t caller; bool on; ~Leave() { if (on) g->proxy.leave(caller); } } leave{r->graphs, caller, proxied};
    const RefineCall c{r, r->w, r->wg, plan, s, P, h, w, iters, ws, {ws.lvl[0], ws.lvl[1], ws.lvl[2], ws.lvl[3]},
                       fmap1, {fmap2, ws.f2l[0], ws.f2l[1], ws.f2l[2]}, flow_lr_out ? flow_lr_out : ws.flow_lr};
    TRY(c.volume(fmap2, gather));
    TRY(c.init_state(net, inp, flow_init, gather));
    if (plan.use_graph) {
        if (plan.side_stream) TRY(ensure_side_stream(r));
        GraphKey key{};
        key.v[0] = (uintptr_t)P; key.v[1] = (uintptr_t)h; key.v[2] = (uintptr_t)w; key.v[3] = (uintptr_t)iters;
        key.v[4] = reinterpret_cast<uintptr_t>(workspace); key.v[5] = reinterpret_cast<uintptr_t>(flow_lr_out);
        key.v[6] = (uintptr_t)r->arith; key.v[7] = reinterpret_cast<uintptr_t>(r->wfused); key.v[8] = reinterpret_cast<uintptr_t>(s);
        key.v[9] = reinterpret_cast<uintptr_t>(r->wflow); key.v[10] = reinterpret_cast<uintptr_t>(r->wt[W_ZR1_DYN]); key.v[11] = reinterpret_cast<uintptr_t>(r->wproj);
        key.v[12] = reinterpret_cast<uintptr_t>(r->wou); key.v[13] = plan.ctx_supplied ? 1 : 0;
        TRY(r->graphs->run(key, s, [&c]() { return c.core(); }));
    } else TRY(c.core());
    return launch_convex_upsample(c.flow_lr, ws.ou, 4, ws.mask, P, h, w, pad_left, pad_right, pad_top, pad_bottom,
                                  flow, occl, sigma, packed, s, r->nonfinite);
}

extern "C" int mftx_raft_refine(mftx_raft *r, int P, int h, int w, int iters, const float *fmap1,
                                const float *fmap2, const float *net, const float *inp, const float *flow_init,
                                int pad_left, int pad_right, int pad_top, int pad_bottom, float *flow, float *occl,
                                float *sigma, float *packed, float *flow_lr_out, void *workspace,
                                size_t workspace_bytes, void *stream) {
    return refine_impl(r, P, h, w, iters, fmap1, fmap2, net, inp, flow_init, pad_left, pad_right, pad_top, pad_bottom, flow, occl, sigma,
                       packed, flow_lr_out, workspace, workspace_bytes, stream, nullptr);
}

extern "C" int mftx_raft_refine_gather(mftx_raft *r, int P, int h, int w, int iters, const float *const *fmap1,
                                       const float *const *fmap2, const float *const *net, const float *const *inp,
                                       const float *flow_init, int pad_left, int pad_right, int pad_top, int pad_bottom,
                                       float *flow, float *occl, float *sigma, float *packed, float *flow_lr_out,
                                       void *workspace, size_t workspace_bytes, void *stream) {
    return mftx_raft_refine_gather_ex(r, P, h, w, iters, fmap1, fmap2, net, inp, nullptr, nullptr, nullptr, flow_init, pad_left, pad_right, pad_top,
                                      pad_bottom, flow, occl, sigma, packed, flow_lr_out, workspace, workspace_bytes, stream);
}

extern "C" int mftx_raft_refine_gather_ex(mftx_raft *r, int P, int h, int w, int iters, const float *const *fmap1,
                                          const float *const *fmap2, const float *const *net, const float *const *inp,
                                          const float *const *ctx_parts, const void *const *fmap1_split, const void *fmap2_split,
                                          const float *flow_init, int pad_left, int pad_right, int pad_top, int pad_bottom,
                                          float *flow, float *occl, float *sigma, float *packed, float *flow_lr_out,
                                          void *workspace, size_t workspace_bytes, void *stream) {
    if (!r || r->magic != RAFT_MAGIC) return fail(MFTX_E_STATE, "raft_refine_gather: bad handle");
    if (!fmap1 || !fmap2 || !net || !inp) return fail(MFTX_E_ARG, "raft_refine_gather: null pointer");
    if (P < 1 || P > MFTX_MAX_GATHER) return fail(MFTX_E_ARG, "raft_refine_gather: 1 .. %d pairs", MFTX_MAX_GATHER);
    if (r->arith != MFTX_ARITH_SPLIT || r->ondemand || r->opt[MFTX_RAFT_OPT_TILE_VOLUME] == 0)
        return fail(MFTX_E_STATE, "raft_refine_gather: needs the split arithmetic with the stored, tile-resident correlation volume (use mftx_raft_refine)");
    RefineGather g{};
    g.f2_shared = true;
    for (int b = 0; b < P; ++b) {
        if (!fmap1[b] || !fmap2[b] || !net[b] || !inp[b]) return fail(MFTX_E_ARG, "raft_refine_gather: pair %d has a null map", b);
        if (!aligned16(fmap1[b]) || !aligned16(fmap2[b]) || !aligned16(net[b]) || !aligned16(inp[b])) return fail(MFTX_E_ALIGN, "raft_refine_gather: maps must be 16-byte aligned");
        g.f1.p[b] = fmap1[b]; g.f2.p[b] = fmap2[b]; g.net.p[b] = net[b]; g.inp.p[b] = inp[b];
        if (fmap2[b] != fmap2[0]) g.f2_shared = false;
    }
    if (ctx_parts) {
        for (int i = 0; i < 4 * P; ++i)
            if (!ctx_parts[i] || !aligned16(ctx_parts[i])) return fail(MFTX_E_ALIGN, "raft_refine_gather: context part %d of pair %d null or not 16-byte aligned", i & 3, i >> 2);
        g.has_ctx = true;
        for (int b = 0; b < P; ++b) for (int k = 0; k < 4; ++k) g.ctx[k].p[b] = ctx_parts[4 * b + k];
    }
    if (fmap1_split) {
        for (int b = 0; b < P; ++b) {
            if (!fmap1_split[b] || !aligned16(fmap1_split[b])) return fail(MFTX_E_ALIGN, "raft_refine_gather: split map of pair %d null or not 16-byte aligned", b);
            g.f1s.p[b] = static_cast<const float *>(fmap1_split[b]);
        }
        g.has_f1s = true;
    }
    if (fmap2_split) {
        if (!aligned16(fmap2_split)) return fail(MFTX_E_ALIGN, "raft_refine_gather: the second map's split form must be 16-byte aligned");
        if (!g.f2_shared) return fail(MFTX_E_ARG, "raft_refine_gather: a split second map goes with ONE second map for all pairs");
        g.f2s = static_cast<const float *>(fmap2_split);
    }
    return refine_impl(r, P, h, w, iters, nullptr, nullptr, nullptr, nullptr, flow_init, pad_left, pad_right, pad_top, pad_bottom, flow, occl,
                       sigma, packed, flow_lr_out, workspace, workspace_bytes, stream, &g);
}

__global__ void split_rows_kernel(const float *__restrict__ in, float *__restrict__ out, long long slots, int c4) {
    const long long i = (long long)blockIdx.x * blockDim.x + threadIdx.x;
    if (i >= slots) return;
    const long long m = i / c4;
    const int q = (int)(i - m * c4);
    store_split4v(out + m * 4 * c4, 4 * q, reinterpret_cast<const float4 *>(in)[i]);
}

extern "C" size_t mftx_raft_frame_prepare_bytes(int h, int w) {
    if (h <= 0 || w <= 0) return 0;
    return ((size_t)h * w * 128 * sizeof(float) + 255) & ~size_t(255);
}

extern "C" int mftx_raft_frame_prepare(mftx_raft *r, int h, int w, const float *fmap, const float *inp, float *ctx_zr1, float *ctx_q1,
                                       float *ctx_zr2, float *ctx_q2, void *fmap_split, void *scratch, size_t scratch_bytes, void *stream) {
    if (!r || r->magic != RAFT_MAGIC) return fail(MFTX_E_STATE, "raft_frame_prepare: bad handle");
    if (h < 16 || w < 16 || (long long)h * w > (1ll << 24)) return fail(MFTX_E_ARG, "raft_frame_prepare: bad size");
    const bool want_ctx = ctx_zr1 || ctx_q1 || ctx_zr2 || ctx_q2;
    if (!want_ctx && !fmap_split) return fail(MFTX_E_ARG, "raft_frame_prepare: nothing to write");
    if (r->arith != MFTX_ARITH_SPLIT || r->opt[MFTX_RAFT_OPT_PRESPLIT] == 0)
        return fail(MFTX_E_STATE, "raft_frame_prepare: needs the split arithmetic with split-form activations");
    hipStream_t s = (hipStream_t)stream;
    const long long N = (long long)h * w;
    if (fmap_split) {
        if (!fmap) return fail(MFTX_E_ARG, "raft_frame_prepare: a split map needs fmap");
        TRY(launch_split_weights(fmap, fmap_split, N * 256, s));
    }
    if (!want_ctx) return 0;
    if (!inp || !ctx_zr1 || !ctx_q1 || !ctx_zr2 || !ctx_q2 || !scratch) return fail(MFTX_E_ARG, "raft_frame_prepare: the context parts need inp, all four outputs and the scratch");
    if (r->opt[MFTX_RAFT_OPT_TILE_CONV] == 1)
        return fail(MFTX_E_STATE, "raft_frame_prepare: MFTX_RAFT_OPT_TILE_CONV must be pinned (0 or 2), the batch decides otherwise");
    if (!aligned16(inp) || !aligned16(ctx_zr1) || !aligned16(ctx_q1) || !aligned16(ctx_zr2) || !aligned16(ctx_q2) ||
        (reinterpret_cast<uintptr_t>(scratch) & 255))
        return fail(MFTX_E_ALIGN, "raft_frame_prepare: maps must be 16-byte and the scratch 256-byte aligned");
    if (scratch_bytes < mftx_raft_frame_prepare_bytes(h, w))
        return fail(MFTX_E_WORKSPACE, "raft_frame_prepare: scratch %zu < %zu bytes", scratch_bytes, mftx_raft_frame_prepare_bytes(h, w));
    float *inps = static_cast<float *>(scratch);
    {
        const long long slots = N * 32;
        hipLaunchKernelGGL(split_rows_kernel, dim3((unsigned)((slots + 255) / 256)), dim3(256), 0, s, inp, inps, slots, 32);
        TRY(check_launch("split_rows"));
    }
    float *const zr[2] = {ctx_zr1, ctx_zr2}, *const q[2] = {ctx_q1, ctx_q2};
    RefinePlan plan{};
    plan.SP = true; plan.tiles_on = r->opt[MFTX_RAFT_OPT_TILE_CONV] == 2;
    const RefineCall c{r, r->w, r->wg, plan, s, 1, h, w};
    return c.context_parts(inps, 128, zr, q);
}

extern "C" int mftx_volume_query_split(const float *in, void *out, long long n_floats, void *stream) {
    if (!in || !out) return fail(MFTX_E_ARG, "volume_query_split: null pointer");
    return launch_volume_query_split(in, out, n_floats, (hipStream_t)stream);
}

extern "C" int mftx_raft_graph_stats(const mftx_raft *r, unsigned long long *captures, unsigned long long *replays) {
    if (!r || r->magic != RAFT_MAGIC || !captures || !replays) return fail(MFTX_E_STATE, "raft_graph_stats: bad arguments");
    *captures = r->graphs ? r->graphs->captures : 0;
    *replays = r->graphs ? r->graphs->replays : 0;
    return 0;
}

extern "C" int mftx_corr_pyramid(const float *f1, const float *f2, int P, int C, int h, int w, float *lvl0,
                                 float *lvl1, float *lvl2, float *lvl3, void *stream) {
    if (!f1 || !f2 || !lvl0 || !lvl1 || !lvl2 || !lvl3) return fail(MFTX_E_ARG, "corr_pyramid: null pointer");
    if (P <= 0 || C <= 0 || C % 32 || h < 8 || w < 8) return fail(MFTX_E_ARG, "corr_pyramid: need C %% 32 == 0, h, w >= 8");
    if (!aligned16(f1) || !aligned16(f2)) return fail(MFTX_E_ALIGN, "corr_pyramid: features must be 16-byte aligned");
    if (!aligned16(lvl0) || !aligned16(lvl1) || !aligned16(lvl2) || !aligned16(lvl3))
        return fail(MFTX_E_ALIGN, "corr_pyramid: levels must be 16-byte aligned");
    float *const lv[4] = {lvl0, lvl1, lvl2, lvl3};
    return launch_corr_pyramid(f1, f2, P, C, h, w, lv, (hipStream_t)stream);
}

extern "C" int mftx_corr_pyramid_split(const float *f1, const float *f2, int P, int C, int h, int w, float *lvl0,
                                       float *lvl1, float *lvl2, float *lvl3, float *f2_scratch, void *stream) {
    if (!f1 || !f2 || !lvl0 || !lvl1 || !lvl2 || !lvl3 || !f2_scratch) return fail(MFTX_E_ARG, "corr_pyramid_split: null pointer");
    if (P <= 0 || C <= 0 || C % 32 || h < 8 || w < 8) return fail(MFTX_E_ARG, "corr_pyramid_split: need C %% 32 == 0, h, w >= 8");
    if (!aligned16(f1) || !aligned16(f2) || (reinterpret_cast<uintptr_t>(f2_scratch) & 31))
        return fail(MFTX_E_ALIGN, "corr_pyramid_split: features must be 16-byte aligned, the scratch 32-byte aligned");
    if (!aligned16(lvl0) || !aligned16(lvl1) || !aligned16(lvl2) || !aligned16(lvl3))
        return fail(MFTX_E_ALIGN, "corr_pyramid_split: levels must be 16-byte aligned");
    float *const lv[4] = {lvl0, lvl1, lvl2, lvl3};
    return launch_corr_pyramid(f1, f2, P, C, h, w, lv, (hipStream_t)stream, f2_scratch);
}

extern "C" int mftx_corr_pyramid_layout(int h, int w, long long *stride, int *block_grid) {
    if (h < 8 || w < 8 || !stride || !block_grid) return fail(MFTX_E_ARG, "corr_pyramid_layout: bad arguments");
    const PyramidLayout L = pyramid_layout(h, w);
    for (int l = 0; l < 4; ++l) stride[l] = L.stride[l];
    block_grid[0] = L.hb[0]; block_grid[1] = L.wb[0]; block_grid[2] = L.hb[1]; block_grid[3] = L.wb[1];
    return 0;
}

extern "C" int mftx_corr_lookup(const float *lvl0, const float *lvl1, const float *lvl2, const float *lvl3,
                                const float *coords, int P, int h, int w, int r, float *out, int ld_out,
                                void *stream) {
    if (!lvl0 || !lvl1 || !lvl2 || !lvl3 || !coords || !out) return fail(MFTX_E_ARG, "corr_lookup: null pointer");
    if (r != 4) return fail(MFTX_E_ARG, "corr_lookup: only radius 4 (RAFT basic) is built");
    if (P <= 0 || h < 8 || w < 8 || ld_out < 324) return fail(MFTX_E_ARG, "corr_lookup: bad sizes");
    if (!aligned16(lvl0) || !aligned16(lvl1)) return fail(MFTX_E_ALIGN, "corr_lookup: levels 0 and 1 must be 16-byte aligned");
    const float *lv[4] = {lvl0, lvl1, lvl2, lvl3};
    return launch_corr_lookup(lv, coords, P, h, w, out, ld_out, (hipStream_t)stream);
}

extern "C" int mftx_pack_lookup_convc1_weights(const float *wpk, int ld_w, void *wfused, void *stream) {
    if (!wpk || !wfused) return fail(MFTX_E_ARG, "pack_lookup_convc1_weights: null pointer");
    if (ld_w < 324) return fail(MFTX_E_ARG, "pack_lookup_convc1_weights: need ld_w >= 324");
    if (!aligned16(wfused)) return fail(MFTX_E_ALIGN, "pack_lookup_convc1_weights: output must be 16-byte aligned");
    return launch_pack_lookup_convc1(wpk, ld_w, wfused, (hipStream_t)stream);
}

extern "C" int mftx_corr_lookup_convc1(const float *lvl0, const float *lvl1, const float *lvl2, const float *lvl3,
                                       const float *coords, int P, int h, int w, const void *wfused, const float *bias,
                                       float *out, int ld_out, int out_split, void *stream) {
    if (!lvl0 || !lvl1 || !lvl2 || !lvl3 || !coords || !wfused || !bias || !out) return fail(MFTX_E_ARG, "corr_lookup_convc1: null pointer");
    if (P <= 0 || h < 8 || w < 8 || ld_out < 256 || ld_out % 4) return fail(MFTX_E_ARG, "corr_lookup_convc1: bad sizes");
    if (!lookup_convc1_applicable(P, h, w, ld_out)) return fail(MFTX_E_ARG, "corr_lookup_convc1: batch too large");
    if (!aligned16(wfused) || !aligned16(bias) || !aligned16(out) || !aligned16(coords) ||
        (out_split && (ld_out % 8 || (reinterpret_cast<uintptr_t>(out) & 31))))
        return fail(MFTX_E_ALIGN, "corr_lookup_convc1: operands must be 16-byte aligned (a split-form output: 32-byte rows)");
    const float *lv[4] = {lvl0, lvl1, lvl2, lvl3};
    return launch_lookup_convc1(lv, coords, P, h, w, wfused, bias, out, ld_out, out_split ? 1 : 0, (hipStream_t)stream);
}

extern "C" int mftx_pack_tile_conv_weights(const float *wpk, int N, int taps, int cin, int cin_pad, void *wtile, void *stream) {
    if (taps == 9 && cin == 256) return launch_pack_tile_conv2p(wpk, N, cin_pad, wtile, (hipStream_t)stream);
    return launch_pack_tile_conv(wpk, N, taps, cin, cin_pad, wtile, (hipStream_t)stream);
}

extern "C" int mftx_tile_conv2d(const mftx_conv_desc *d, const void *wtile, void *stream) {
    if (!d || !wtile) return fail(MFTX_E_ARG, "tile_conv2d: null pointer");
    if (d->arith != MFTX_ARITH_SPLIT || !d->a_split) return fail(MFTX_E_ARG, "tile_conv2d: split arithmetic with a split-form input only");
    if (d->act != 0 && d->act != 1) return fail(MFTX_E_ARG, "tile_conv2d: activation none or relu");
    if (d->stride > 1 || d->residual_mode != 0 || d->out_scale != 1.f || (d->hin && d->hin != d->h) || (d->win && d->win != d->w) || d->pad_y != 0 || d->pad_x != 0)
        return fail(MFTX_E_ARG, "tile_conv2d: stride 1, same padding, no output scale");
    if (d->kh == 3 && d->kw == 3 && d->c0 == 256 && d->c1 == 0) {
        if (d->act != 1 || !d->out_split || d->addend || !d->bias) return fail(MFTX_E_ARG, "tile_conv2d: 3 x 3 over 256 channels comes with bias, relu and a split-form output");
        return launch_tile_conv2p(d->a0, d->lda0, wtile, d->bias, d->out, d->ldo, d->N, d->P, d->h, d->w, 0, (hipStream_t)stream);
    }
    if (d->c0 != 128 || (d->c1 != 0 && d->c1 != 128)) return fail(MFTX_E_ARG, "tile_conv2d: channel segments of 128");
    TileConvLaunch t{};
    t.a0 = d->a0; t.lda0 = d->lda0; t.a1 = d->c1 ? d->a1 : nullptr; t.lda1 = d->lda1; t.cin = d->c0 + d->c1; t.wf = wtile; t.bias = d->bias;
    t.addend = d->addend; t.ld_addend = d->ld_addend; t.out = d->out; t.ldo = d->ldo; t.out_split = d->out_split;
    t.P = d->P; t.h = d->h; t.w = d->w; t.N = d->N; t.kh = d->kh; t.kw = d->kw; t.epi = d->act;
    return launch_tile_conv(t, (hipStream_t)stream);
}

extern "C" int mftx_gru_half(const float *h_in, int ld_hin, const float *motion, int ld_mo, const void *wzr, const void *wq, const float *pre_zr,
                             const float *pre_q, float *z, const float *hf_in, float *hf_out, float *h_out, int ld_hout, int P, int h, int w, int pass,
                             void *stream) {
    GruHalfLaunch g{};
    g.h_in = h_in; g.ld_hin = ld_hin; g.mo = motion; g.ld_mo = ld_mo; g.wzr = wzr; g.wq = wq; g.pre_zr = pre_zr; g.pre_q = pre_q;
    g.z = z; g.hf_in = hf_in; g.hf_out = hf_out; g.h_out = h_out; g.ld_hout = ld_hout; g.P = P; g.h = h; g.w = w; g.pass = pass;
    return launch_gru_half(g, (hipStream_t)stream);
}

extern "C" int mftx_tile_conv_fills_chip(int P, int h, int w) {
    if (P <= 0 || h <= 0 || w <= 0) return 0;
    return tile_conv_fills_chip(P, h, w, 3, 3) || tile_conv_small_tiles_fill(P, h, w) ? 1 : 0;
}

extern "C" int mftx_pack_ou_heads_weights(const float *w1pk, int cin_pad, const float *w2pk, void *wtile, void *wproj, void *stream) {
    return launch_pack_ou_head(w1pk, cin_pad, w2pk, wtile, wproj, (hipStream_t)stream);
}

extern "C" int mftx_ou_heads(const float *a_split, int lda, int P, int h, int w, const void *wtile, const float *b1, const void *wproj, const float *b2,
                             float *T, float *out, int ld_out, void *stream) {
    return launch_ou_heads(a_split, lda, P, h, w, wtile, b1, wproj, b2, T, out, ld_out, 0, (hipStream_t)stream);
}

extern "C" int mftx_pack_flow_head_weights(const float *w2pk, void *wproj, void *stream) {
    return launch_pack_flow_head(w2pk, wproj, (hipStream_t)stream);
}

extern "C" int mftx_flow_head(const float *hsplit, int ld_h, int P, int h, int w, const void *wtile, const float *b1, const void *wproj,
                              const float *b2, float *T, float *delta, float *coords, void *stream) {
    if (!hsplit || !wtile || !b1 || !wproj || !b2 || !T || !delta) return fail(MFTX_E_ARG, "flow_head: null pointer");
    TileConvLaunch t{};
    t.a0 = hsplit; t.lda0 = ld_h; t.cin = 128; t.wf = wtile; t.bias = b1; t.wproj = wproj; t.tout = T;
    t.P = P; t.h = h; t.w = w; t.N = 256; t.kh = 3; t.kw = 3; t.epi = 4;
    if (int e = launch_tile_conv(t, (hipStream_t)stream)) return e;
    return launch_flow_head_sum(T, b2, delta, coords, coords, P, h, w, (hipStream_t)stream);
}

extern "C" int mftx_pack_flow_branch_weights(const float *w98, const float *w2pk, void *wflow, void *stream) {
    if (!w98 || !w2pk || !wflow) return fail(MFTX_E_ARG, "pack_flow_branch_weights: null pointer");
    if (!aligned16(wflow)) return fail(MFTX_E_ALIGN, "pack_flow_branch_weights: output not 16-byte aligned");
    return launch_pack_flow_branch(w98, w2pk, wflow, (hipStream_t)stream);
}

extern "C" int mftx_flow_branch(const float *coords, int P, int h, int w, const void *wflow, const float *b1, const float *b2,
                                float *out, int ld_out, float *hx, int ld_hx, void *stream) {
    return launch_flow_branch(coords, P, h, w, wflow, b1, b2, out, ld_out, hx, ld_hx, (hipStream_t)stream);
}

extern "C" int mftx_fmap_pyramid(const float *f2, int P, int C, int h, int w, float *lvl1, float *lvl2, float *lvl3,
                                 void *stream) {
    if (!f2 || !lvl1 || !lvl2 || !lvl3) return fail(MFTX_E_ARG, "fmap_pyramid: null pointer");
    if (P <= 0 || C <= 0 || C % 4 || h < 8 || w < 8) return fail(MFTX_E_ARG, "fmap_pyramid: need C %% 4 == 0, h, w >= 8");
    if (!aligned16(f2) || !aligned16(lvl1) || !aligned16(lvl2) || !aligned16(lvl3))
        return fail(MFTX_E_ALIGN, "fmap_pyramid: maps must be 16-byte aligned");
    float *const lv[3] = {lvl1, lvl2, lvl3};
    return launch_fmap_pyramid(f2, P, C, h, w, lv, (hipStream_t)stream);
}

extern "C" int mftx_corr_lookup_ondemand(const float *f1, const float *f2l0, const float *f2l1, const float *f2l2,
                                         const float *f2l3, const float *coords, int P, int C, int h, int w, int r,
                                         float *out, int ld_out, void *stream) {
    if (!f1 || !f2l0 || !f2l1 || !f2l2 || !f2l3 || !coords || !out) return fail(MFTX_E_ARG, "corr_lookup_ondemand: null pointer");
    if (r != 4 || C != 256) return fail(MFTX_E_ARG, "corr_lookup_ondemand: only radius 4, 256 channels (RAFT basic) are built");
    if (P <= 0 || h < 8 || w < 8 || ld_out < 324) return fail(MFTX_E_ARG, "corr_lookup_ondemand: bad sizes");
    if (!aligned16(f1) || !aligned16(f2l0) || !aligned16(f2l1) || !aligned16(f2l2) || !aligned16(f2l3))
        return fail(MFTX_E_ALIGN, "corr_lookup_ondemand: feature maps must be 16-byte aligned");
    const float *lv[4] = {f2l0, f2l1, f2l2, f2l3};
    return launch_corr_ondemand(f1, lv, coords, P, h, w, out, ld_out, (hipStream_t)stream);
}

extern "C" int mftx_split_weights(const float *wpk, void *out, long long n_floats, void *stream) {
    if (!wpk || !out) return fail(MFTX_E_ARG, "split_weights: null pointer");
    return launch_split_weights(wpk, out, n_floats, (hipStream_t)stream);
}

extern "C" int mftx_conv2d(const mftx_conv_desc *d, void *stream) {
    if (!d) return fail(MFTX_E_ARG, "conv2d: null descriptor");
    return launch_conv(*d, (hipStream_t)stream);
}

extern "C" int mftx_conv2d_tile(const mftx_conv_desc *d, int tile, void *stream) {
    if (!d) return fail(MFTX_E_ARG, "conv2d_tile: null descriptor");
    if (tile < -1 || tile > 15) return fail(MFTX_E_ARG, "conv2d_tile: tile must be -1 (the library's choice) or 0..15");
    return launch_conv(*d, (hipStream_t)stream, tile);
}

extern "C" int mftx_convex_upsample(const float *flow_lr, const float *ou, int ld_ou, const float *mask, int P,
                                    int h, int w, int pad_left, int pad_right, int pad_top, int pad_bottom,
                                    float *flow, float *occl, float *sigma, float *packed, void *stream) {
    const bool planar = flow && occl && sigma;
    if (!flow_lr || !ou || !mask || (!planar && (flow || occl || sigma || !packed)))
        return fail(MFTX_E_ARG, "convex_upsample: null pointer (outputs: flow + occl + sigma, or packed, or both)");
    if (P <= 0 || h <= 0 || w <= 0 || ld_ou < 3) return fail(MFTX_E_ARG, "convex_upsample: bad sizes");
    return launch_convex_upsample(flow_lr, ou, ld_ou, mask, P, h, w, pad_left, pad_right, pad_top, pad_bottom, flow,
                                  occl, sigma, packed, (hipStream_t)stream);
}
```

### mft_amd/csrc/volume_tile.hip

```cpp
#include "common.h"
#include "profile.h"
#include "device_prims.h"

namespace mftx {

constexpr int VT_C = 256;
constexpr int VT_ROW = VT_C * 4 + 16;
constexpr int VT_TARGETS = 128 * VT_ROW;
constexpr int VT_LDS = VT_TARGETS + 8 * 1024;

struct VolTileArgs {
    const float *f1;
    const float *f2s;
    float *lvl0, *lvl1, *lvl2, *lvl3;
    long long s0, s1, s2, s3;
    int P, N, h, w, sbw, n_sb, wb0;
    float scale;
    int qchunks, blocks_per_chunk;
    int ablate;
    int gathered;
    long long f2_bstride;
    PairPtrs f1p;
};

template <int N>
__device__ __forceinline__ float vt_shl(float v) {
    return __builtin_bit_cast(float, __builtin_amdgcn_update_dpp(0, __builtin_bit_cast(int, v), 0x100 + N, 0xf, 0xf, true));
}
template <int N>
__device__ __forceinline__ float vt_shr(float v) {
    return __builtin_bit_cast(float, __builtin_amdgcn_update_dpp(0, __builtin_bit_cast(int, v), 0x110 + N, 0xf, 0xf, true));
}

template <bool QSPLIT>
__global__ __launch_bounds__(512, 2) void volume_tile_kernel(VolTileArgs p) {
    extern __shared__ __attribute__((aligned(16))) unsigned char vt_lds[];
    unsigned char *lds = vt_lds;
    const int tid = (int)threadIdx.x, lane = tid & 63, wv = __builtin_amdgcn_readfirstlane(tid >> 6);
    const int wg = (int)blockIdx.x;
    const int qc = wg % p.qchunks, sb = (wg / p.qchunks) % p.n_sb, bz = wg / (p.qchunks * p.n_sb);
    const int sby = sb / p.sbw, sbx = sb - sby * p.sbw;
    const float k2048 = __builtin_bit_cast(float, __builtin_amdgcn_readfirstlane(0x45000000));

    {
        const float *f2p = p.f2s + (long long)bz * p.f2_bstride;
#pragma unroll 4
        for (int k = 0; k < 16; ++k) {
            const int q = k * 512 + tid, m = q >> 6, pc = q & 63;
            const int j = m >> 5, mm = m & 31;
            const int ty = 8 * sby + 4 * (j >> 1) + (mm >> 3), tx = 16 * sbx + 8 * (j & 1) + (mm & 7);
            uint4 v = make_uint4(0u, 0u, 0u, 0u);
            if (ty < p.h && tx < p.w) v = *reinterpret_cast<const uint4 *>(f2p + ((long long)ty * p.w + tx) * VT_C + pc * 4);
            *reinterpret_cast<uint4 *>(lds + m * VT_ROW + pc * 16) = v;
        }
    }
    lds_barrier();

    const unsigned char *abase = lds + (lane & 31) * VT_ROW + (lane >> 5) * 32;
    const int n_blocks = (p.N + 31) >> 5;
    const int b_lo = qc * p.blocks_per_chunk, b_hi = (b_lo + p.blocks_per_chunk < n_blocks) ? b_lo + p.blocks_per_chunk : n_blocks;
    const long long qbase = (long long)bz * p.N;
    const float inv2048 = 1.f / 2048.f;
    const int hf = lane >> 5;
    const int h2 = p.h >> 2, w2 = p.w >> 2, h3 = p.h >> 3, w3 = p.w >> 3;

    const int pp = lane & 31;
    const int l1_src = 4 * (32 * hf + 2 * (pp & 3) + 16 * ((pp >> 3) & 1) + ((pp >> 2) & 1) + 8 * (pp >> 4));
    const int l3_src = 4 * ((lane + 16) & 63);
    constexpr int PF = 3;
    f32x4 raw[PF][2];
    const float *f1base = p.gathered ? p.f1p.p[bz] : p.f1 + qbase * VT_C;
    auto row_of = [&](int qb) {
        const int q = qb * 32 + (lane & 31);
        return f1base + (long long)(q < p.N ? q : p.N - 1) * VT_C + 8 * hf;
    };
    auto prefetch = [&](const float *src) {
#pragma unroll
        for (int g = 0; g < PF; ++g) {
            raw[g][0] = *reinterpret_cast<const f32x4 *>(src + 16 * g);
            raw[g][1] = *reinterpret_cast<const f32x4 *>(src + 16 * g + 4);
        }
    };
    if (b_lo + wv < b_hi) prefetch(row_of(b_lo + wv));
    for (int qb = b_lo + wv; qb < b_hi; qb += 8) {
        const float *src = row_of(qb);
        f32x16 acc[4], accx[4];
#pragma unroll
        for (int j = 0; j < 4; ++j)
#pragma unroll
            for (int r = 0; r < 16; ++r) { acc[j][r] = 0.f; accx[j][r] = 0.f; }
        f16x8 ah[2][4], al[2][4];
        auto read_a = [&](int g, int set) {
#pragma unroll
            for (int j = 0; j < 4; ++j) {
                ah[set][j] = *reinterpret_cast<const f16x8 *>(abase + j * 32 * VT_ROW + g * 64);
                al[set][j] = *reinterpret_cast<const f16x8 *>(abase + j * 32 * VT_ROW + g * 64 + 16);
            }
        };
        read_a(0, 0);
#pragma unroll
        for (int g = 0; g < 16; ++g) {
            const int set = g & 1;
            f16x8 bh, bl;
            if constexpr (QSPLIT) {
                bh = __builtin_bit_cast(f16x8, raw[g % PF][0]);
                bl = __builtin_bit_cast(f16x8, raw[g % PF][1]);
            } else split8(raw[g % PF][0], raw[g % PF][1], k2048, bh, bl);
            __builtin_amdgcn_sched_barrier(0);
            if (g + 1 < 16) read_a(g + 1, set ^ 1);
            if (g + PF < 16) {
                raw[g % PF][0] = *reinterpret_cast<const f32x4 *>(src + 16 * (g + PF));
                raw[g % PF][1] = *reinterpret_cast<const f32x4 *>(src + 16 * (g + PF) + 4);
            }
            __builtin_amdgcn_sched_barrier(0);
#pragma unroll
            for (int j = 0; j < 4; ++j) acc[j] = mfma_f16(bh, ah[set][j], acc[j]);
#pragma unroll
            for (int j = 0; j < 4; ++j) accx[j] = mfma_f16(bh, al[set][j], accx[j]);
#pragma unroll
            for (int j = 0; j < 4; ++j) accx[j] = mfma_f16(bl, ah[set][j], accx[j]);
            __builtin_amdgcn_sched_barrier(0);
        }

        if (qb + 8 < b_hi) prefetch(row_of(qb + 8));
        __builtin_amdgcn_sched_barrier(0);

        const int m = lane & 31;
        const int q0 = qb * 32;
        const long long blk0 = ((long long)(2 * sby) * p.wb0 + 2 * sbx) * 32 + m;
        const int rows_ok = p.N - q0 < 32 ? p.N - q0 : 32;
        const __amdgpu_buffer_rsrc_t r0 = __builtin_amdgcn_make_buffer_rsrc(p.lvl0 + (qbase + q0) * p.s0, 0, (unsigned)((long long)rows_ok * p.s0 * 4), 0x00020000);
        const __amdgpu_buffer_rsrc_t r1 = __builtin_amdgcn_make_buffer_rsrc(p.lvl1 + (qbase + q0) * p.s1, 0, (unsigned)((long long)rows_ok * p.s1 * 4), 0x00020000);
        const unsigned v1off = (unsigned)((4 * hf * p.s1 + ((long long)sby * p.sbw + sbx) * 32 + m) * 4);
        const unsigned s0b = (unsigned)(p.s0 * 4), s1b = (unsigned)(p.s1 * 4), jrow = (unsigned)(p.wb0 * 128);
        int le = lane;
        asm volatile("" : "+v"(le));
        const int d2c = le & 7, d2hf = (le >> 3) & 1, d2i = le >> 4;
        const int l2_pull = 4 * (32 * d2hf + 16 * (d2c >> 2) + 2 * (d2c & 3));
        const int l2_y = 2 * sby + (d2c >> 2), l2_x = 4 * sbx + (d2c & 3);
        const bool l2_ok = l2_y < h2 && l2_x < w2;
        const int l2_off = l2_y * w2 + l2_x, l2_row = 4 * d2hf + d2i;
        const int d3c = le & 1, d3hf = (le >> 1) & 1, d3r = le >> 2;
        const int l3_pull = 4 * (32 * d3hf + 4 * d3c);
        const int l3_x = 2 * sbx + d3c;
        const bool l3_ok = sby < h3 && l3_x < w3;
        const int l3_off = sby * w3 + l3_x, l3_row = 8 * (d3r >> 2) + 4 * d3hf + (d3r & 3);
        float *slab = reinterpret_cast<float *>(lds + VT_TARGETS + wv * 1024);
        const unsigned v0off4 = (unsigned)((le >> 3) * s0b) + (unsigned)((blk0 - m) * 4) + (unsigned)(le & 7) * 16u;
        float acc2 = 0.f, acc3 = 0.f;
#pragma unroll
        for (int g = 0; g < 4; ++g) {
#ifdef MFTX_TUNING
            const bool st0g = !(p.ablate & 1);
#else
            const bool st0g = true;
#endif
            float vv[4][4];
#pragma unroll
            for (int i = 0; i < 4; ++i)
#pragma unroll
                for (int j = 0; j < 4; ++j) vv[i][j] = (acc[j][4 * g + i] + accx[j][4 * g + i] * inv2048) * p.scale;
            f32x4 line[4];
#pragma unroll
            for (int j = 0; j < 4; ++j) {
#pragma unroll
                for (int i = 0; i < 4; ++i) slab[(4 * hf + i) * 32 + m] = vv[i][j];
                line[j] = *reinterpret_cast<const f32x4 *>(slab + (le >> 3) * 32 + (le & 7) * 4);
            }
            if (st0g) {
#pragma unroll
                for (int j = 0; j < 4; ++j)
                    __builtin_amdgcn_raw_buffer_store_b128(__builtin_bit_cast(u32x4, line[j]), r0, v0off4 + (j >> 1) * jrow + (j & 1) * 128u, (unsigned)(8 * g) * s0b, 0);
            }
#pragma unroll
        for (int i = 0; i < 4; ++i) {
            const int r = 4 * g + i;
            const int qrow = q0 + 8 * (r >> 2) + 4 * hf + (r & 3);
            const bool row_ok = qrow < p.N;
#ifdef MFTX_TUNING
            const bool st1 = row_ok && !(p.ablate & 2);
#define MFTX_VT_ST23 (!(p.ablate & 10))
#else
            const bool st1 = row_ok;
#define MFTX_VT_ST23 true
#endif
            float merged = 0.f;
#pragma unroll
            for (int j = 0; j < 4; ++j) {
                const float v = vv[i][j];
                float t = v + vt_shl<1>(v);
                t = t + vt_shl<8>(v);
                t = (t + vt_shl<9>(v)) * 0.25f;
                if (j == 0) merged = t;
                else {
                    float sh = j == 1 ? vt_shr<1>(t) : (j == 2 ? vt_shr<8>(t) : vt_shr<9>(t));
                    asm volatile("" : "+v"(sh));
                    const bool take = j == 1 ? (m & 1) != 0 : (j == 2 ? ((m >> 3) & 1) && !(m & 1) : ((m >> 3) & 1) && (m & 1));
                    merged = take ? sh : merged;
                }
            }
            const float l1 = __builtin_bit_cast(float, __builtin_amdgcn_ds_bpermute(l1_src, __builtin_bit_cast(int, merged)));
            if (st1) __builtin_amdgcn_raw_buffer_store_b32(__builtin_bit_cast(unsigned, l1), r1, v1off, (unsigned)(8 * (r >> 2) + (r & 3)) * s1b, 0);
            float t2 = l1 + vt_shl<1>(l1);
            t2 = t2 + vt_shl<8>(l1);
            t2 = (t2 + vt_shl<9>(l1)) * 0.25f;
            asm volatile("" : "+v"(t2));
            {
                const float pulled = __builtin_bit_cast(float, __builtin_amdgcn_ds_bpermute(l2_pull, __builtin_bit_cast(int, t2)));
                acc2 = d2i == (r & 3) ? pulled : acc2;
                if ((r & 3) == 3) {
                    const int row2 = q0 + 8 * (r >> 2) + l2_row;
                    if (MFTX_VT_ST23 && l2_ok && row2 < p.N) p.lvl2[(qbase + row2) * p.s2 + l2_off] = acc2;
                }
            }
            const float bq = vt_shl<2>(t2);
            const float cq = __builtin_bit_cast(float, __builtin_amdgcn_ds_bpermute(l3_src, __builtin_bit_cast(int, t2)));
            const float dq = __builtin_bit_cast(float, __builtin_amdgcn_ds_bpermute(l3_src + 8, __builtin_bit_cast(int, t2)));
            float v3 = (((t2 + bq) + cq) + dq) * 0.25f;
            asm volatile("" : "+v"(v3));
            {
                const float pulled = __builtin_bit_cast(float, __builtin_amdgcn_ds_bpermute(l3_pull, __builtin_bit_cast(int, v3)));
                acc3 = d3r == r ? pulled : acc3;
                if (r == 15) {
                    const int row3 = q0 + l3_row;
                    if (MFTX_VT_ST23 && l3_ok && row3 < p.N) p.lvl3[(qbase + row3) * p.s3 + l3_off] = acc3;
                }
            }
        }
        }
    }
}

static int vt_num_cus() {
    static const int n = [] {
        int dev = 0, cus = 256;
        hipDeviceProp_t prop;
        if (hipGetDevice(&dev) == hipSuccess && hipGetDeviceProperties(&prop, dev) == hipSuccess && prop.multiProcessorCount > 0) cus = prop.multiProcessorCount;
        return cus;
    }();
    return n;
}

bool volume_tile_applicable(int C) { return C == VT_C; }

__global__ void vt_query_split_kernel(const float *__restrict__ in, uint4 *__restrict__ out, long long n8) {
    const long long i = (long long)blockIdx.x * blockDim.x + threadIdx.x;
    const float k2048 = __builtin_bit_cast(float, __builtin_amdgcn_readfirstlane(0x45000000));
    if (i >= n8) return;
    const f32x4 u = *reinterpret_cast<const f32x4 *>(in + i * 8), v = *reinterpret_cast<const f32x4 *>(in + i * 8 + 4);
    f16x8 hi, lo;
    split8(u, v, k2048, hi, lo);
    out[2 * i] = __builtin_bit_cast(uint4, hi);
    out[2 * i + 1] = __builtin_bit_cast(uint4, lo);
}

int launch_volume_query_split(const float *in, void *out, long long n, hipStream_t s) {
    if (n <= 0 || n % 8) return fail(MFTX_E_ARG, "volume_query_split: a positive multiple of 8 floats");
    if (!aligned16(in) || !aligned16(out)) return fail(MFTX_E_ALIGN, "volume_query_split: operands must be 16-byte aligned");
    const long long n8 = n / 8;
    hipLaunchKernelGGL(vt_query_split_kernel, dim3((unsigned)((n8 + 255) / 256)), dim3(256), 0, s, in, reinterpret_cast<uint4 *>(out), n8);
    return check_launch("volume_query_split");
}

int launch_volume_tile(const float *f1, const float *f2s, int P, int h, int w, float *const lvl[4], hipStream_t s, const PairPtrs *f1p, long long f2_bstride,
                       bool f1_split) {
    if (f1p && P > MFTX_MAX_GATHER) return fail(MFTX_E_ARG, "corr_pyramid: at most %d gathered pairs", MFTX_MAX_GATHER);
    const PyramidLayout L = pyramid_layout(h, w);
    VolTileArgs a{};
    a.f1 = f1; a.f2s = f2s; a.lvl0 = lvl[0]; a.lvl1 = lvl[1]; a.lvl2 = lvl[2]; a.lvl3 = lvl[3];
    a.s0 = L.stride[0]; a.s1 = L.stride[1]; a.s2 = L.stride[2]; a.s3 = L.stride[3];
    a.P = P; a.N = h * w; a.h = h; a.w = w; a.sbw = L.sbw; a.n_sb = L.sbh * L.sbw; a.wb0 = L.wb[0];
    a.scale = 1.0f / sqrtf((float)VT_C);
    a.gathered = f1p ? 1 : 0;
    if (f1p) a.f1p = *f1p;
    a.f2_bstride = f2_bstride >= 0 ? f2_bstride : (long long)a.N * VT_C;
    const int n_blocks = (a.N + 31) / 32;
    const long long base = (long long)P * a.n_sb;
    a.ablate = tune_env("MFTX_VT_ABLATE", 0);
    static const int q_forced = tune_env("MFTX_VT_QCHUNKS", 0);
    int qchunks = q_forced > 0 ? q_forced : (base * 4 >= 3LL * vt_num_cus() ? 1 : (int)((vt_num_cus() + base - 1) / base));
    if (qchunks < 1) qchunks = 1;
    if (qchunks > (n_blocks + 7) / 8) qchunks = (n_blocks + 7) / 8;
    a.blocks_per_chunk = (n_blocks + qchunks - 1) / qchunks;
    a.qchunks = (n_blocks + a.blocks_per_chunk - 1) / a.blocks_per_chunk;
    const long long wgs = base * a.qchunks;
    if (wgs > 0x7fffffffLL) return fail(MFTX_E_ARG, "corr_pyramid: too many workgroups");
    static bool attr_set = false;
    if (!attr_set) {
        if (hipFuncSetAttribute(reinterpret_cast<const void *>(volume_tile_kernel<false>), hipFuncAttributeMaxDynamicSharedMemorySize, VT_LDS) != hipSuccess ||
            hipFuncSetAttribute(reinterpret_cast<const void *>(volume_tile_kernel<true>), hipFuncAttributeMaxDynamicSharedMemorySize, VT_LDS) != hipSuccess)
            return fail(MFTX_E_STATE, "corr_pyramid: cannot reserve %d bytes of LDS", VT_LDS);
        attr_set = true;
    }
    ProfScope prof(PC_CORR_VOLUME, s, 2.0 * a.N * a.N * (double)VT_C * P);
    if (f1_split) hipLaunchKernelGGL(volume_tile_kernel<true>, dim3((unsigned)wgs), dim3(512), VT_LDS, s, a);
    else hipLaunchKernelGGL(volume_tile_kernel<false>, dim3((unsigned)wgs), dim3(512), VT_LDS, s, a);
    return check_launch("volume_tile");
}

}
```

### mft_amd/ops.py

```python
from __future__ import annotations

import ctypes as C
import math
from typing import NamedTuple

import numpy as np
import torch

from . import _lib
from ._lib import ConvDesc, MftxError, check

ACT = {None: 0, "none": 0, "relu": 1, "sigmoid": 2, "tanh": 3}


def _stream():
    return C.c_void_p(torch.cuda.current_stream().cuda_stream)


def _device_visible(t):
    return isinstance(t, torch.Tensor) and (t.is_cuda or t.is_pinned())


def copy_bytes(src: torch.Tensor, dst: torch.Tensor):
    if not (_device_visible(src) and _device_visible(dst)):
# ... 748 lines not shown
        if x.data_ptr() % 16:
            x = x.clone()
    _chk(x, "x")
    if x.numel() == 0:
        raise MftxError("quantize_u16: empty channel")
    ws = _quant_ws.get(x.device)
    if ws is None:
        ws = _quant_ws[x.device] = torch.empty(lib.mftx_quantize_workspace_bytes(), dtype=torch.uint8, device=x.device)
    q = torch.empty(x.shape, dtype=torch.uint16, device=x.device)
    lohi = torch.empty(2, dtype=torch.float32, device=x.device)
    check(lib.mftx_quantize_u16(x.data_ptr(), x.numel(), q.data_ptr(), lohi.data_ptr(), ws.data_ptr(), ws.numel(),
                                _stream()), "mftx_quantize_u16")
    return q, lohi


def dequantize_u16(q, lo, hi):
    lib = _lib.load()
    if isinstance(q, torch.Tensor) and q.is_cuda:
        q = q.contiguous()
        if q.data_ptr() % 16:
            q = q.clone()
    _chk(q, "q", torch.uint16)
    x = torch.empty(q.shape, dtype=torch.float32, device=q.device)
    check(lib.mftx_dequantize_u16(q.data_ptr(), q.numel(), float(lo), float(hi), x.data_ptr(), _stream()),
          "mftx_dequantize_u16")
    return x



_trackstore_ws = {}


def _trackstore_frame(packed, lohi, H, W):
    if tuple(packed.shape) != (H, W, 4) or tuple(lohi.shape) != (4, 2):
        raise MftxError("trackstore: packed must be [H,W,4] uint16 and lohi [4,2] float32")
    return _chk(packed, "packed", torch.uint16), _chk(lohi, "lohi")


def trackstore_append(planes, packed, lohi):
    lib = _lib.load()
    _, H, W = planes[0].shape
    H, W = int(H), int(W)
    fp, op, sp = _planes(planes, H, W)
    pp, lp = _trackstore_frame(packed, lohi, H, W)
    dev = packed.device
    ws = _trackstore_ws.get(dev)
    if ws is None:
        ws = _trackstore_ws[dev] = torch.empty(lib.mftx_trackstore_workspace_bytes(), dtype=torch.uint8, device=dev)
    check(lib.mftx_trackstore_append(fp, op, sp, H, W, pp, lp, ws.data_ptr(), ws.numel(), _stream()), "mftx_trackstore_append")
    return packed, lohi


TRACKSTORE_APPEND_MULTI_FRAMES = 64
_trackstore_multi_ws = {}


def trackstore_append_multi(frames):
    lib = _lib.load()
    frames = list(frames)
    T = len(frames)
    if T == 0:
        return
    _, H, W = frames[0][0][0].shape
    H, W = int(H), int(W)
    cols = [_planes(planes, H, W) for planes, _, _ in frames]
    outs = [_trackstore_frame(packed, lohi, H, W) for _, packed, lohi in frames]
    dev = frames[0][1].device
    need = lib.mftx_trackstore_append_multi_workspace_bytes(T)
    ws = _trackstore_multi_ws.get(dev)
    if ws is None or ws.numel() < need:
        ws = _trackstore_multi_ws[dev] = torch.empty(need, dtype=torch.uint8, device=dev)
    arrs = [_lib.ptr_array(list(c)) for c in zip(*cols)] + [_lib.ptr_array(list(c)) for c in zip(*outs)]
    check(lib.mftx_trackstore_append_multi(T, arrs[0][0], arrs[1][0], arrs[2][0], H, W, arrs[3][0], arrs[4][0], ws.data_ptr(),
                                           ws.numel(), _stream()), "mftx_trackstore_append_multi")


def trackstore_unpack(packed, lohi, out=None):
    lib = _lib.load()
    H, W = int(packed.shape[0]), int(packed.shape[1])
    pp, lp = _trackstore_frame(packed, lohi, H, W)
    if out is None:
        out = _new_result(H, W, packed.device)
    fp, op, sp = _planes(out, H, W)
    check(lib.mftx_trackstore_unpack(pp, lp, H, W, fp, op, sp, _stream()), "mftx_trackstore_unpack")
    return out


def _trackstore_chunks(chunks, lohi_chunks, name):
    chunks, lohi_chunks = list(chunks), list(lohi_chunks)
    if not chunks or len(chunks) != len(lohi_chunks):
        raise MftxError(f"{name}: as many lohi tables as chunks, at least one")
    fpc, H, W = (int(s) for s in chunks[0].shape[:3])
    for c, l in zip(chunks, lohi_chunks):
        if tuple(c.shape) != (fpc, H, W, 4) or tuple(l.shape) != (fpc, 4, 2):
            raise MftxError(f"{name}: chunks must be [frames_per_chunk,H,W,4] with lohi [frames_per_chunk,4,2]")
    return fpc, H, W, [_chk(c, "chunk", torch.uint16) for c in chunks], [_chk(l, "lohi chunk") for l in lohi_chunks]


def _slot_addresses(slots, chunk_ptrs, lohi_ptrs, frames_per_chunk, frame_bytes):
    chunk, within = slots // frames_per_chunk, slots % frames_per_chunk
    return np.asarray(chunk_ptrs, dtype=np.int64)[chunk] + within * frame_bytes, np.asarray(lohi_ptrs, dtype=np.int64)[chunk] + within * 32


def trackstore_slot_addresses(chunks, lohi_chunks, slots):
    fpc, H, W, cptr, lptr = _trackstore_chunks(chunks, lohi_chunks, "trackstore_slot_addresses")
    slots = np.asarray(slots, dtype=np.int64)
    if slots.size and (slots.min() < -1 or slots.max() >= fpc * len(cptr)):
        raise MftxError("trackstore_slot_addresses: slots must be slots of the store, or -1")
    held = slots >= 0
    packed, lohi = _slot_addresses(np.where(held, slots, 0), cptr, lptr, fpc, H * W * 8)
    return np.where(held, packed, 0), np.where(held, lohi, 0)


def _pack_tables(int64_parts, int32_parts):
    n64, n32 = sum(map(len, int64_parts)), sum(map(len, int32_parts))
    buf = np.zeros(n64 + (n32 + 1) // 2, np.int64)
    tail = buf[n64:].view(np.int32)
    offsets, at = [], 0
    for part in int64_parts:
        buf[at:at + len(part)] = part
        offsets.append(8 * at)
        at += len(part)
    at = 0
    for part in int32_parts:
        tail[at:at + len(part)] = part
        offsets.append(8 * n64 + 4 * at)
        at += len(part)
    return buf, tuple(offsets)


def _upload_tables(device, int64_parts, int32_parts):
    buf, offsets = _pack_tables(int64_parts, int32_parts)
    tables = torch.from_numpy(buf).pin_memory().to(device, non_blocking=True)
    return tables, tuple(tables.data_ptr() + o for o in offsets)


def trackstore_query(chunks, lohi_chunks, slots, xy, table, column0=0):
    lib = _lib.load()
    fpc, H, W, cptr, lptr = _trackstore_chunks(chunks, lohi_chunks, "trackstore_query")
    if xy.dim() != 2 or int(xy.shape[1]) != 2 or slots.dim() != 1:
        raise MftxError("trackstore_query: slots must be [T], xy [N, 2]")
    N, T = int(xy.shape[0]), int(slots.shape[0])
    if table.dim() != 3 or int(table.shape[0]) != N or int(table.shape[2]) != 4:
        raise MftxError("trackstore_query: the table must be [N, frames, 4]")
    carr, larr = _lib.ptr_array(cptr), _lib.ptr_array(lptr)
    if N == 0 or T == 0:
        return table
    check(lib.mftx_trackstore_query(carr[0], larr[0], len(cptr), fpc, _chk(slots, "slots", torch.int32), T, H, W, N,
                                    _chk(xy, "xy"), _chk(table, "table"), 4 * int(table.shape[1]), int(column0), _stream()),
          "mftx_trackstore_query")
    return table


def _locate_parts(point_slots, chunk_ptrs, lohi_ptrs, frames_per_chunk, frame_bytes):
    slots = np.asarray(point_slots, dtype=np.int64).reshape(-1)
    N = int(slots.shape[0])
    order = np.argsort(slots, kind="stable")
    sorted_slots = slots[order]
    first = np.flatnonzero(np.concatenate([[True], sorted_slots[1:] != sorted_slots[:-1]]))
    G = int(first.shape[0])
    group_start = np.concatenate([first, [N]])
    group_of = np.empty(N, np.int32)
    group_of[order] = np.repeat(np.arange(G, dtype=np.int32), np.diff(group_start))
    return G, _slot_addresses(sorted_slots[first], chunk_ptrs, lohi_ptrs, frames_per_chunk, frame_bytes), (group_start, order, group_of)


def locate_tables(point_slots, chunk_ptrs, lohi_ptrs, frames_per_chunk, frame_bytes):
    G, int64_parts, int32_parts = _locate_parts(point_slots, chunk_ptrs, lohi_ptrs, frames_per_chunk, frame_bytes)
    buf, offsets = _pack_tables(int64_parts, int32_parts)
    return buf, G, offsets


def _locate_call(name, slots_what, H, W, chunk_ptrs, lohi_ptrs, frames_per_chunk, point_slots, xy, table, cell, occlusion_threshold):
    lib = _lib.load()
    if xy.dim() != 2 or int(xy.shape[1]) != 2:
        raise MftxError(f"{name}: xy must be [N, 2]")
    N = int(xy.shape[0])
    slots = np.asarray(point_slots, dtype=np.int64).reshape(-1)
    if int(slots.shape[0]) != N or (N and (slots.min() < 0 or slots.max() >= frames_per_chunk * len(chunk_ptrs))):
        raise MftxError(f"{name}: {slots_what}")
    if tuple(table.shape) != (N, 4) or tuple(cell.shape) != (N,):
        raise MftxError(f"{name}: the table must be [N, 4], cell [N]")
    xp, tp, cp = _chk(xy, "xy"), _chk(table, "table"), _chk(cell, "cell", torch.int32)
    if N == 0:
        return table, cell
    G, int64_parts, int32_parts = _locate_parts(slots, chunk_ptrs, lohi_ptrs, frames_per_chunk, H * W * 8)
    tables, (frames, lohis, group_start, order, group_of) = _upload_tables(xy.device, int64_parts, int32_parts)
    keys = torch.empty(N, dtype=torch.int64, device=xy.device)
    check(lib.mftx_trackstore_locate(frames, lohis, group_start, G, order, group_of, H, W, N, xp, float(occlusion_threshold),
                                     keys.data_ptr(), tp, cp, _stream()), "mftx_trackstore_locate")
    return table, cell


def trackstore_locate(chunks, lohi_chunks, point_slots, xy, table, cell, occlusion_threshold=0.5):
    fpc, H, W, cptr, lptr = _trackstore_chunks(chunks, lohi_chunks, "trackstore_locate")
    return _locate_call("trackstore_locate", "point_slots must be N slots of the store", H, W, cptr, lptr, fpc, point_slots, xy,
                        table, cell, occlusion_threshold)


def trackstore_invert(chunks, lohi_chunks, slots, table, cell, occlusion_threshold=0.5):
    lib = _lib.load()
    fpc, H, W, cptr, lptr = _trackstore_chunks(chunks, lohi_chunks, "trackstore_invert")
    slots = np.asarray(slots, dtype=np.int64).reshape(-1)
    G = int(slots.shape[0])
    if G and (slots.min() < 0 or slots.max() >= fpc * len(cptr)):
        raise MftxError("trackstore_invert: slots must be slots of the store")
    if tuple(table.shape) != (G, H, W, 4) or tuple(cell.shape) != (G, H, W):
        raise MftxError("trackstore_invert: the table must be [G, H, W, 4], cell [G, H, W]")
    tp, cp = _chk(table, "table"), _chk(cell, "cell", torch.int32)
    if G == 0:
        return table, cell
    tables, (frames, lohis) = _upload_tables(table.device, _slot_addresses(slots, cptr, lptr, fpc, H * W * 8), ())
    keys = torch.empty(G * H * W, dtype=torch.int64, device=table.device)
    check(lib.mftx_trackstore_invert(frames, lohis, G, H, W, float(occlusion_threshold), keys.data_ptr(), tp, cp, _stream()),
          "mftx_trackstore_invert")
    return table, cell


def _trackstore_frame_ptrs(frames, name):
    frames = list(frames)
    if not frames:
        raise MftxError(f"{name}: at least one stored frame")
    H, W = int(frames[0][0].shape[0]), int(frames[0][0].shape[1])
    ptrs = [_trackstore_frame(p, l, H, W) for p, l in frames]
    return H, W, np.asarray([p for p, _ in ptrs], dtype=np.int64), np.asarray([l for _, l in ptrs], dtype=np.int64)


def trackstore_locate_frames(frames, point_frame, xy, table, cell, occlusion_threshold=0.5):
    H, W, pptr, lptr = _trackstore_frame_ptrs(frames, "trackstore_locate_frames")
    return _locate_call("trackstore_locate_frames", "point_frame must be N indices into frames", H, W, pptr, lptr, 1, point_frame,
                        xy, table, cell, occlusion_threshold)


TRACKSTORE_ATLAS_ENTRIES = 256
TRACKSTORE_ATLAS_CELLS = 1 << 24


def trackstore_invert_atlas(frames, first_of, rank_of, table, cell, entry, occlusion_threshold=0.5):
    lib = _lib.load()
    frames = list(frames)
    first_of = np.asarray(first_of, dtype=np.int64).reshape(-1)
    rank_of = np.asarray(rank_of, dtype=np.int64).reshape(-1)
    G, J = int(first_of.shape[0]) - 1, len(frames)
    if table.dim() != 4 or int(table.shape[3]) != 4 or int(table.shape[0]) != G or tuple(cell.shape) != tuple(table.shape[:3]) \
            or tuple(entry.shape) != tuple(table.shape[:3]):
        raise MftxError("trackstore_invert_atlas: the table must be [G, H, W, 4], cell and entry [G, H, W], first_of [G + 1]")
    H, W = int(table.shape[1]), int(table.shape[2])
    if G < 0 or int(rank_of.shape[0]) != J or first_of[0] != 0 or first_of[-1] != J or (np.diff(first_of) < 0).any():
        raise MftxError("trackstore_invert_atlas: first_of must ascend from 0 to the number of frames, rank_of name every frame")
    if G and np.diff(first_of).max() > TRACKSTORE_ATLAS_ENTRIES:
        raise MftxError(f"trackstore_invert_atlas: more than {TRACKSTORE_ATLAS_ENTRIES} entries in a plane")
    if (H - 1) * (W - 1) > TRACKSTORE_ATLAS_CELLS:
        raise MftxError("trackstore_invert_atlas: more than 2^24 cells")
    tp, cp, ep = _chk(table, "table"), _chk(cell, "cell", torch.int32), _chk(entry, "entry", torch.int32)
    if J:
        fH, fW, pptr, lptr = _trackstore_frame_ptrs(frames, "trackstore_invert_atlas")
        if (fH, fW) != (H, W):
            raise MftxError("trackstore_invert_atlas: the frames must be of the table's H x W")
    else:
        pptr = lptr = np.zeros(0, np.int64)
    if G == 0:
        return table, cell, entry
    tables, (fr, lh, fo, ro) = _upload_tables(table.device, (pptr, lptr), (first_of, rank_of))
    keys = torch.empty(G * H * W, dtype=torch.int64, device=table.device)
    check(lib.mftx_trackstore_invert_atlas(fr if J else None, lh if J else None, fo, ro if J else None, G, J, H, W,
                                           float(occlusion_threshold), keys.data_ptr(), tp, cp, ep, _stream()),
          "mftx_trackstore_invert_atlas")
    return table, cell, entry


TRACKSTORE_FLOW_COLUMNS = 16


def trackstore_flow_from(table, entry, row_of, frame_ptrs, lohi_ptrs, flow, occl, sigma, columns_per_block=0):
    lib = _lib.load()
    row_of = np.asarray(row_of, dtype=np.int64).reshape(-1)
    frame_ptrs, lohi_ptrs = np.asarray(frame_ptrs, dtype=np.int64), np.asarray(lohi_ptrs, dtype=np.int64)
    if table.dim() != 3 or int(table.shape[2]) != 4 or tuple(entry.shape) != tuple(table.shape[:2]):
        raise MftxError("trackstore_flow_from: the table must be [H, W, 4], entry [H, W]")
    H, W = int(table.shape[0]), int(table.shape[1])
    if frame_ptrs.ndim != 2 or frame_ptrs.shape != lohi_ptrs.shape or frame_ptrs.shape[0] < 1 or ((frame_ptrs == 0) != (lohi_ptrs == 0)).any():
        raise MftxError("trackstore_flow_from: frame_ptrs and lohi_ptrs must be [R, T] with R >= 1, zero in the same places")
    R, T = (int(s) for s in frame_ptrs.shape)
    n_ranks = int(row_of.shape[0])
    if n_ranks < 1 or row_of.min() < 0 or row_of.max() >= R:
        raise MftxError("trackstore_flow_from: row_of must name a row for at least one rank")
    if tuple(flow.shape) != (T, 2, H, W) or tuple(occl.shape) != (T, 1, H, W) or tuple(sigma.shape) != (T, 1, H, W):
        raise MftxError("trackstore_flow_from: flow must be [T, 2, H, W], occl and sigma [T, 1, H, W]")
    tp, ep = _chk(table, "table"), _chk(entry, "entry", torch.int32)
    fp, op, sp = _chk(flow, "flow"), _chk(occl, "occl"), _chk(sigma, "sigma")
    if T == 0:
        return flow, occl, sigma
    tables, (frames, lohis, rows) = _upload_tables(table.device, (frame_ptrs.reshape(-1), lohi_ptrs.reshape(-1)), (row_of,))
    check(lib.mftx_trackstore_flow_from(tp, ep, rows, frames, lohis, n_ranks, R, T, H, W, int(columns_per_block), fp, op, sp,
                                        _stream()), "mftx_trackstore_flow_from")
    return flow, occl, sigma


class RaftEngine:

    GEMM_SLOTS = (0, 2, 6, 8, 10, 11, 13, 14, 16, 17, 19, 20, 22, 26, 28, 30)

    OPTIONS = {"fork": 0, "presplit": 1, "group": 2, "fuse_lookup": 3, "graph": 4, "fuse_flow": 5, "tile_conv": 6, "fuse_head": 7, "tile_volume": 8, "fuse_gru": 9, "tile_cells": 10, "fuse_ou": 11, "tile_conv2p": 12}
    TILE_SLOTS = {2: (192, 256), 8: (128, 256), 10: (256, 256), 11: (256, 128), 13: (128, 256), 14: (128, 128), 16: (256, 256),
                  17: (256, 128), 19: (128, 256), 20: (128, 128), 22: (256, 128), 26: (256, 128)}

    def __init__(self, state_dict: dict, device, ondemand_corr=False, arith=ARITH_SPLIT, options=None):
        lib = _lib.load()
        self.device = torch.device(device)
        self.weights = pack_raft_weights(state_dict, self.device)
        arr, self._keep = _lib.ptr_array([_chk(t, "weight") for t in self.weights])
        handle = C.c_void_p()
        check(lib.mftx_raft_create(arr, len(self.weights), C.byref(handle)), "mftx_raft_create")
        self._h = handle
        self._ws = None
        self.arith = int(arith)
        if self.arith == ARITH_SPLIT:
            self.split = [split_weights(t) if i in self.GEMM_SLOTS else None for i, t in enumerate(self.weights)]
            sarr, self._keep_split = _lib.ptr_array([t.data_ptr() if t is not None else None for t in self.split])
            check(lib.mftx_raft_set_split_weights(self._h, sarr, len(self.split)), "mftx_raft_set_split_weights")
            self.wfused = pack_lookup_convc1_weights(self.weights[0])
            check(lib.mftx_raft_set_lookup_fused(self._h, self.wfused.data_ptr()), "mftx_raft_set_lookup_fused")
            self.wflow = pack_flow_branch_weights(self.weights[4], self.weights[6])
            check(lib.mftx_raft_set_flow_fused(self._h, self.wflow.data_ptr()), "mftx_raft_set_flow_fused")
            self.wtile = [pack_tile_conv_weights(t, *self.TILE_SLOTS[i]) if i in self.TILE_SLOTS else None
                          for i, t in enumerate(self.weights)]
            tarr, self._keep_tile = _lib.ptr_array([t.data_ptr() if t is not None else None for t in self.wtile])
            check(lib.mftx_raft_set_tile_weights(self._h, tarr, len(self.wtile)), "mftx_raft_set_tile_weights")
            self.wproj = pack_flow_head_weights(self.weights[24])
            check(lib.mftx_raft_set_flow_head(self._h, self.wproj.data_ptr()), "mftx_raft_set_flow_head")
            self.wou, self.wouproj = pack_ou_heads_weights(self.weights[30], self.weights[32])
            check(lib.mftx_raft_set_ou_heads(self._h, self.wou.data_ptr(), self.wouproj.data_ptr()), "mftx_raft_set_ou_heads")
        elif self.arith != ARITH_F32:
            raise MftxError(f"unknown arithmetic {arith!r}")
        self._nonfinite = torch.zeros(4, dtype=torch.int32, device=self.device)
        check(lib.mftx_raft_set_nonfinite_counter(self._h, self._nonfinite.data_ptr()), "mftx_raft_set_nonfinite_counter")
        options = dict(options or {})
        self._gather = bool(options.pop("gather", 1))
        for k, v in options.items():
            self.set_option(k, v)
        self.ondemand_corr = bool(ondemand_corr)
        if self.ondemand_corr:
            check(lib.mftx_raft_set_ondemand(self._h, 1), "mftx_raft_set_ondemand")

    def __del__(self):
        try:
            if getattr(self, "_h", None):
                _lib.load().mftx_raft_destroy(self._h)
                self._h = None
        except Exception:
            pass

    def debug_refine(self, fmap1, fmap2, net, inp, h, w, iters, pads=(0, 0, 0, 0), flow_init=None):
        lib = _lib.load()
        P = fmap1.shape[0]
        M = P * h * w
        trace = torch.empty(iters + 1, M, 2, dtype=torch.float32, device=self.device)
        check(lib.mftx_raft_set_coords_trace(self._h, trace.data_ptr()), "mftx_raft_set_coords_trace")
        try:
            out = self.refine(fmap1, fmap2, net, inp, h, w, iters, pads=pads, flow_init=flow_init)
        finally:
            check(lib.mftx_raft_set_coords_trace(self._h, None), "mftx_raft_set_coords_trace")
        if self.ondemand_corr:
            pyramid = None
        else:
            stride, _ = pyramid_layout(h, w)
            pyramid = []
            for l in range(4):
                lvl = self.region(f"lvl{l}", P, h, w, stride[l]).reshape(P, h * w, stride[l])
                pyramid.append(unblock_level(lvl, l, h, w).reshape(M, 1, h >> l, w >> l).cpu())
        to_map = lambda t: t.reshape(P, h, w, 2).permute(0, 3, 1, 2).contiguous().cpu()
        ys, xs = torch.meshgrid(torch.arange(h, dtype=torch.float32), torch.arange(w, dtype=torch.float32), indexing="ij")
        debug = {"costvolume_pyramid": pyramid,
                 "coords_left": torch.stack([xs, ys])[None].repeat(P, 1, 1, 1),
                 "iterations": [{"coords": to_map(trace[i])} for i in range(iters + 1)]}
        return out, debug

    PLAN_FIELDS = ("presplit", "fuse_lookup", "tiles_on", "gru_fused", "ctx_supplied", "two_pass", "flow", "pair_second", "head_fused",
                   "defer_update", "ou_fused", "ou_materialised", "use_graph", "side_stream")
    FLOW_SCHEDULES = ("fused", "side", "first", "after_lookup", "with_lookup")

    def plan(self, P, h, w, ctx_supplied=False):
        out = (C.c_int * len(self.PLAN_FIELDS))()
        check(_lib.load().mftx_raft_plan(self._h, P, h, w, int(bool(ctx_supplied)), out, len(out)), "mftx_raft_plan")
        plan = {k: bool(v) for k, v in zip(self.PLAN_FIELDS, out)}
        plan["flow"] = self.FLOW_SCHEDULES[out[self.PLAN_FIELDS.index("flow")]]
        return plan

    def graph_stats(self):
        c, r = C.c_ulonglong(), C.c_ulonglong()
        check(_lib.load().mftx_raft_graph_stats(self._h, C.byref(c), C.byref(r)), "mftx_raft_graph_stats")
        return int(c.value), int(r.value)

    def nonfinite_count(self, reset=False):
        n = int(self._nonfinite[0].item())
        if reset and n:
            self._nonfinite.zero_()
        return n

    def nonfinite_snapshot(self, host_words):
        copy_bytes(self._nonfinite, host_words)

    def set_option(self, name, value):
        if name not in self.OPTIONS:
            raise MftxError(f"unknown engine option {name!r} (known: {', '.join(sorted(self.OPTIONS))}, gather)")
        check(_lib.load().mftx_raft_set_option(self._h, self.OPTIONS[name], int(value)), "mftx_raft_set_option")
        if name == "tile_conv":
            self._tile_conv = int(value)
        if name == "tile_volume":
            self._tile_volume = int(value)

    def workspace(self, P, h, w):
        need = _lib.load().mftx_raft_workspace_bytes_for(self._h, P, h, w)
        if self._ws is None or self._ws.numel() < need:
            if self._ws is not None:
                check(_lib.load().mftx_raft_clear_graphs(self._h), "mftx_raft_clear_graphs")
            self._ws = torch.empty(need, dtype=torch.uint8, device=self.device)
        return self._ws

    REGIONS = ("lvl0", "lvl1", "lvl2", "lvl3", "coords1", "corr", "cor1", "corflo", "flo1", "hx", "z", "rh", "fh",
               "delta", "mask", "ouin", "ouh", "ou", "flow_lr")

    SPLIT_REGIONS = {"cor1": 256, "corflo": 256, "flo1": 128, "hx": 384, "rh": 128, "ouin": 712}

    def region(self, name, P, h, w, cols, split=None):
        offs = (C.c_size_t * 19)()
        check(_lib.load().mftx_raft_workspace_layout_for(self._h, P, h, w, offs, 19), "mftx_raft_workspace_layout_for")
        off = offs[self.REGIONS.index(name)]
        M = P * h * w
        if split is None:
            split = self.arith == ARITH_SPLIT and name in self.SPLIT_REGIONS and self.plan(P, h, w)["presplit"]
        if split:
            ld = self.SPLIT_REGIONS.get(name, cols)
            raw = self._ws[off: off + 4 * M * ld].view(torch.float32).reshape(M, ld)
            return unsplit_activations(raw)[:, :cols]
        return self._ws[off: off + 4 * M * cols].view(torch.float32).reshape(M, cols)

    MAX_GATHER = 16

    def can_gather(self, P):
        return (self.arith == ARITH_SPLIT and not self.ondemand_corr and P <= self.MAX_GATHER and
                getattr(self, "_tile_volume", 1) != 0 and getattr(self, "_gather", True))

    def prepare_frame(self, fmap, inp, h, w, context=True, split=True):
        lib = _lib.load()
        N = h * w
        dev = self.device
        ctx = fsplit = scratch = None
        if context:
            ctx = tuple(torch.empty(N, c, dtype=torch.float32, device=dev) for c in (256, 128, 256, 128))
            scratch = torch.empty(lib.mftx_raft_frame_prepare_bytes(h, w), dtype=torch.uint8, device=dev)
        if split:
            fsplit = torch.empty(N, 256, dtype=torch.float32, device=dev)
        cp = [t.data_ptr() for t in ctx] if context else [None] * 4
        check(lib.mftx_raft_frame_prepare(self._h, h, w, _chk(fmap, "fmap") if split else None, _chk(inp, "inp") if context else None,
                                          *cp, fsplit.data_ptr() if split else None,
                                          scratch.data_ptr() if context else None, scratch.numel() if context else 0, _stream()),
              "mftx_raft_frame_prepare")
        return ctx, fsplit

    def refine(self, fmap1, fmap2, net, inp, h, w, iters, pads=(0, 0, 0, 0), want_flow_lr=False, flow_init=None,
               packed=None, planar=True, prepared=None):
        lib = _lib.load()
        gathered = isinstance(fmap1, (list, tuple))
        P = len(fmap1) if gathered else fmap1.shape[0]
        pl, pr, pt, pb = pads
        H0, W0 = 8 * h - pt - pb, 8 * w - pl - pr
        dev = self.device
        if not planar and packed is None:
            raise MftxError("refine: planar=False needs a packed output")
        flow = torch.empty(P, 2, H0, W0, dtype=torch.float32, device=dev) if planar else None
        occl = torch.empty(P, 1, H0, W0, dtype=torch.float32, device=dev) if planar else None
        sigma = torch.empty(P, 1, H0, W0, dtype=torch.float32, device=dev) if planar else None
        flow_lr = torch.empty(P, h * w, 2, dtype=torch.float32, device=dev) if want_flow_lr else None
        if flow_init is not None and tuple(flow_init.shape) != (P, h * w, 2):
            raise MftxError("flow_init must be [P, h*w, 2]")
        if packed is not None and tuple(packed.shape) != (P, H0, W0, 4):
            raise MftxError("packed must be [P, H0, W0, 4]")
        ws = self.workspace(P, h, w)

        def tail():
            return (_chk(flow_init, "flow_init") if flow_init is not None else None, pl, pr, pt, pb,
                    flow.data_ptr() if planar else None, occl.data_ptr() if planar else None, sigma.data_ptr() if planar else None,
                    _chk(packed, "packed") if packed is not None else None, flow_lr.data_ptr() if want_flow_lr else None,
                    ws.data_ptr(), ws.numel(), _stream())

        if gathered:
            if not self.can_gather(P) or not (len(fmap2) == len(net) == len(inp) == P):
                raise MftxError("refine: per-pair map lists need the split arithmetic with the tile-resident volume and P <= 16")
            arrs = [_lib.ptr_array([_chk(t, "map") for t in lst]) for lst in (fmap1, fmap2, net, inp)]
            maps = [a[0] for a in arrs]
            if prepared:
                ctx, f1s, f2s = prepared.get("ctx"), prepared.get("f1s"), prepared.get("f2s")
                if (ctx is not None and len(ctx) != P) or (f1s is not None and len(f1s) != P):
                    raise MftxError("refine: prepared parts for every pair, or none")
                carr = _lib.ptr_array([_chk(t, "context part") for parts in ctx for t in parts]) if ctx is not None else (None, None)
                sarr = _lib.ptr_array([_chk(t, "split map") for t in f1s]) if f1s is not None else (None, None)
                check(lib.mftx_raft_refine_gather_ex(self._h, P, h, w, iters, *maps, carr[0], sarr[0],
                                                     _chk(f2s, "split map") if f2s is not None else None, *tail()),
                      "mftx_raft_refine_gather_ex")
            else:
                check(lib.mftx_raft_refine_gather(self._h, P, h, w, iters, *maps, *tail()), "mftx_raft_refine_gather")
        elif prepared:
            raise MftxError("refine: prepared parts go with per-pair map lists")
        else:
            check(lib.mftx_raft_refine(self._h, P, h, w, iters, _chk(fmap1, "fmap1"), _chk(fmap2, "fmap2"),
                                       _chk(net, "net"), _chk(inp, "inp"), *tail()), "mftx_raft_refine")
        return (flow, occl, sigma, flow_lr) if want_flow_lr else (flow, occl, sigma)
```

### mft_amd/raft.py

```python
from __future__ import annotations

import logging
import os
from pathlib import Path

import numpy as np
import torch
import torch.nn.functional as F

from . import ops
from .weights import make_weights, strip_module_prefix

logger = logging.getLogger(__name__)


def pad_amounts(H0, W0):
    ph = (((H0 // 8) + 1) * 8 - H0) % 8
    pw = (((W0 // 8) + 1) * 8 - W0) % 8
    return pw // 2, pw - pw // 2, ph // 2, ph - ph // 2


_STREAMS = {}


def _shared_stream(device, kind, index=0):
    device = torch.device(device)
    dev_index = device.index if device.index is not None else torch.cuda.current_device()
    key = (dev_index, kind, index)
    st = _STREAMS.get(key)
    if st is None:
        st = _STREAMS[key] = torch.cuda.Stream(device=torch.device("cuda", dev_index))
    return st


class FrameFeatures:
    __slots__ = ("fmap", "net", "inp", "h", "w", "pads", "shape", "ready", "ctx", "fsplit")

    def __init__(self, fmap, net, inp, h, w, pads, shape, ready=None):
        self.fmap, self.net, self.inp, self.h, self.w, self.pads, self.shape = fmap, net, inp, h, w, pads, shape
        self.ready = ready
        self.ctx = None
        self.fsplit = None

    def tensors(self):
        return [t for t in (self.fmap, self.net, self.inp, self.fsplit) + tuple(self.ctx or ()) if t is not None]


class RAFTWrapper:
    has_packed_output = True
    STAGING_SLOTS = 4

    def __init__(self, config, device="cuda", state_dict=None):
        self.C = config
        self.device = torch.device(device)
        if self.device.type != "cuda":
            raise RuntimeError("mft_amd.RAFTWrapper runs on an MI355X (HIP) device only; there is no CPU path")
        if state_dict is None:
            state_dict = self._load_weights(config)
        sd = {k: (v if isinstance(v, torch.Tensor) else torch.from_numpy(np.asarray(v)))
              for k, v in strip_module_prefix(state_dict).items()}
        self.sd = {k: v.to(self.device) for k, v in sd.items()}
        self._ondemand = bool(getattr(getattr(config, "raft_params", None), "alternate_corr", False))
        arith = getattr(getattr(config, "raft_params", None), "arith", None) or "split"
        if arith not in ("split", "fp32"):
            raise ValueError(f"raft_params.arith must be 'split' or 'fp32', got {arith!r}")
        self._arith = ops.ARITH_SPLIT if arith == "split" else ops.ARITH_F32
        self._engine_options = dict(getattr(getattr(config, "raft_params", None), "engine_options", None) or {})
        try:
            self._build_engines()
        except ops.SplitRangeError as e:
            logger.warning("raft_params.arith = 'split' refused (%s): falling back to arith = 'fp32'", e)
            self._arith = ops.ARITH_F32
            self._build_engines()
        self._check_finite = bool(getattr(getattr(config, "raft_params", None), "check_finite", False))
        self._split_streams = int(os.environ.get("MFTX_SPLIT_STREAMS", "") or getattr(config, "split_streams", 0) or
                                  (1 if self._arith == ops.ARITH_SPLIT else 2))
        self._engines, self._side = [], []
        self._fif = self._frames_in_flight_setting(config)
        self._lanes, self._lane_next = [], 0
        self._lanes_stale = False
        self._ahead_max = max(2, int(getattr(config, "max_batches_ahead", 0) or 16))
        self._ahead = []
        self.nominal_pairs = int(getattr(config, "nominal_pairs", 0) or 7)
        self._tile_choice = {}
        fp = os.environ.get("MFTX_FRAME_PREPARE", "")
        self._frame_prepare = bool(int(fp)) if fp else bool(getattr(config, "__dict__", {}).get("frame_prepare", True))
        self._prepare_ok = {}
        self._frames = {}
        self._staging = {}
        ae = getattr(config, "__dict__", {}).get("async_encode", None)
        self._enc_waits_for_device_frames = ae is None
        if ae is None:
            ae = self._frames_in_flight_setting(config) > 1
        self._enc_stream = _shared_stream(self.device, "enc") if ae else None

    def _frames_in_flight_setting(self, config):
        return max(1, int(os.environ.get("MFTX_FRAMES_IN_FLIGHT", "") or getattr(config, "frames_in_flight", 0) or
                          (2 if self._arith == ops.ARITH_SPLIT else 1)))

    def _build_engines(self):
        graph = bool(self._engine_options.get("graph", 1))
        self.fnet_engine = ops.EncoderEngine(self.sd, "fnet", True, self.device, arith=self._arith, graph=graph)
        self.cnet_engine = ops.EncoderEngine(self.sd, "cnet", False, self.device, arith=self._arith, graph=graph)
        self.engine = ops.RaftEngine(self.sd, self.device, ondemand_corr=self._ondemand, arith=self._arith,
                                     options=self._engine_options)

    def set_nominal_pairs(self, n):
        n = max(1, int(n))
        if n != self.nominal_pairs:
            self.nominal_pairs = n
            self._tile_choice = {}

    def _pin_kernels(self, h, w):
        if self._arith != ops.ARITH_SPLIT or "tile_conv" in self._engine_options:
            return
        v = self._tile_choice.get((h, w))
        if v is None:
            v = self._tile_choice[(h, w)] = 2 if ops._lib.load().mftx_tile_conv_fills_chip(self.nominal_pairs, h, w) else 0
        for e in self._all_engines():
            if getattr(e, "_tile_conv", None) != v:
                e.set_option("tile_conv", v)

    PREPARED_FRAMES = 34

    def _prepare(self, f):
        if not self._frame_prepare or f.net is None or not self.engine.can_gather(1) or f.h < 16 or f.w < 16:
            return
        opt = self._engine_options
        if int(opt.get("presplit", 1)) == 0:
            return
        self._pin_kernels(f.h, f.w)
        fits = self._prepare_ok.get((f.h, f.w))
        if fits is None:
            per_frame = f.h * f.w * 4096
            need = self.PREPARED_FRAMES * per_frame
            ws_bytes = int(ops._lib.load().mftx_raft_workspace_bytes_for(self.engine._h, self.nominal_pairs, f.h, f.w))
            for k in range(self._fif):
                e = self._lanes[k][0] if k < len(self._lanes) else (self.engine if k == 0 else None)
                have = e._ws.numel() if e is not None and e._ws is not None else 0
                need += max(0, ws_bytes - have)
            free, total = torch.cuda.mem_get_info(self.device)
            cached = torch.cuda.memory_reserved(self.device) - torch.cuda.memory_allocated(self.device)
            fits = self._prepare_ok[(f.h, f.w)] = need <= free + cached - total // 10
            if not fits:
                logger.warning("frame_prepare: %.1f MB of prepared parts per cached frame of %d x %d cells do not fit beside the "
                               "workspaces (%.1f GB free): computing them per pair", per_frame / 1e6, f.h, f.w, (free + cached) / 1e9)
        if not fits:
            return
        context = getattr(self.engine, "_tile_conv", 1) == 2 and int(opt.get("fuse_gru", 1)) != 0
        f.ctx, f.fsplit = self.engine.prepare_frame(f.fmap, f.inp, f.h, f.w, context=context, split=True)

    def _prepared(self, fls, frs, flow_init):
        if not self._frame_prepare or flow_init is not None:
            return None
        ctx = [f.ctx for f in fls] if all(f.ctx is not None for f in fls) and getattr(self.engine, "_tile_conv", 1) == 2 else None
        f1s = [f.fsplit for f in fls] if all(f.fsplit is not None for f in fls) else None
        f2s = frs[0].fsplit if all(f is frs[0] for f in frs) else None
        if ctx is None and f1s is None and f2s is None:
            return None
        return {"ctx": ctx, "f1s": f1s, "f2s": f2s}

    def _all_engines(self):
        return list(dict.fromkeys([self.engine] + list(self._engines) + [e for e, _ in self._lanes]))

    def _lane(self):
        while len(self._lanes) < self._fif:
            eng = self.engine if not self._lanes else ops.RaftEngine(self.sd, self.device, ondemand_corr=self._ondemand,
                                                                      arith=self._arith, options=self._engine_options)
            self._lanes.append((eng, _shared_stream(self.device, "lane", len(self._lanes))))
            self._lanes_stale = True
        lane = self._lanes[self._lane_next % self._fif]
        self._lane_next += 1
        return lane

    def _lanes_fit(self, P, h, w):
        while self._fif > max(1, len(self._lanes)):
            k = max(1, len(self._lanes))
            need = int(ops._lib.load().mftx_raft_workspace_bytes_for(self.engine._h, P, h, w))
            free, total = torch.cuda.mem_get_info(self.device)
            cached = torch.cuda.memory_reserved(self.device) - torch.cuda.memory_allocated(self.device)
            if need <= free + cached - total // 10:
                return
            logger.warning("frames_in_flight = %d needs %.1f GB more workspace (lane %d, %d pairs of %d x %d cells) but only %.1f GB of "
                           "the device's %.1f GB are free: running with %d frame(s) in flight", self._fif, need / 1e9, k, P, h, w,
                           (free + cached) / 1e9, total / 1e9, k)
            self._fif = k

    def nonfinite_count(self, reset=False):
        return sum(e.nonfinite_count(reset=reset) for e in self._all_engines())

    def nonfinite_snapshot(self, host_words):
        for i, e in enumerate(self._all_engines()):
            e.nonfinite_snapshot(host_words[i])

    def nonfinite_error(self, bad):
        return FloatingPointError(
            f"flow network: {bad} output pixels with a non-finite value (a NaN, or an infinite flow / occlusion)" + (
                " -- an activation left the fp16 range of the split arithmetic (|x| >= 65504); "
                "set raft_params.arith = 'fp32'" if self._arith == ops.ARITH_SPLIT else ""))

    def raise_if_nonfinite(self):
        bad = self.nonfinite_count(reset=True)
        if bad:
            raise self.nonfinite_error(bad)

    @property
    def arith(self):
        return "split" if self._arith == ops.ARITH_SPLIT else "fp32"

    @staticmethod
    def _load_weights(config):
        model = getattr(config, "model", None)
        seed = getattr(config, "synthetic_weights_seed", None)
        if model:
            if not Path(str(model)).exists():
                raise FileNotFoundError(
                    f"flow checkpoint {model!r} not found (set flow_config.model = None and "
                    "flow_config.synthetic_weights_seed = <int> to run on seeded synthetic weights)")
            logger.info("loading checkpoint %s", model)
            return torch.load(model, map_location="cpu")
        if not isinstance(seed, int) or isinstance(seed, bool):
            raise ValueError("no flow checkpoint configured: set flow_config.model, or "
                             "flow_config.synthetic_weights_seed = <int> for seeded synthetic weights")
        logger.warning("no checkpoint configured: using seeded synthetic weights (seed %d)", seed)
        return make_weights(seed)

    @staticmethod
    def _geometry(H0, W0):
        pads = pad_amounts(H0, W0)
        return (H0 + pads[2] + pads[3]) // 8, (W0 + pads[0] + pads[1]) // 8, pads

    def _device_image(self, img_bgr):
        img = img_bgr if isinstance(img_bgr, torch.Tensor) else torch.from_numpy(np.ascontiguousarray(img_bgr))
        if img.is_cuda:
            return img.to(self.device, non_blocking=True).contiguous()
        if img.dtype == torch.uint8 and not (img.is_pinned() and img.is_contiguous() and img.data_ptr() % 16 == 0):
            img = self._stage_host_frame(img)
        if img.is_pinned() and img.is_contiguous() and img.dtype == torch.uint8 and img.data_ptr() % 16 == 0:
            dev = torch.empty(img.shape, dtype=torch.uint8, device=self.device)
            ops.copy_bytes(img, dev)
            st = getattr(img, "_mftx_slot", None)
            if st is not None:
                st[1] = torch.cuda.current_stream(self.device).record_event()
            return dev
        return img.to(self.device, non_blocking=True).contiguous()

    def _stage_host_frame(self, img):
        key = tuple(img.shape)
        ring = self._staging.get(key)
        if ring is None:
            if len(self._staging) >= 4:
                for slot in self._staging.pop(next(iter(self._staging)))["slots"]:
                    if slot[1] is not None:
                        slot[1].synchronize()
            ring = self._staging[key] = {"n": 0, "slots": []}
        if len(ring["slots"]) < self.STAGING_SLOTS:
            buf = torch.empty(key, dtype=torch.uint8).pin_memory()
            slot = [buf, None]
            buf._mftx_slot = slot
            ring["slots"].append(slot)
        else:
            slot = ring["slots"][ring["n"] % self.STAGING_SLOTS]
        ring["n"] += 1
        if slot[1] is not None:
            slot[1].synchronize()
            slot[1] = None
        np.copyto(slot[0].numpy(), img.numpy() if img.is_contiguous() else np.ascontiguousarray(img.numpy()))
        return slot[0]

    @torch.no_grad()
    def encode(self, img_bgr, want_context=True) -> FrameFeatures:
        H0, W0 = img_bgr.shape[:2]
        img = self._device_image(img_bgr)
        h, w, pads = self._geometry(H0, W0)
        fmap, _ = self.fnet_engine.forward(img)
        net = inp = None
        if want_context:
            net, inp = self.cnet_engine.forward(img)
        return FrameFeatures(fmap, net, inp, h, w, pads, (H0, W0))

    def ensure_encode_stream(self):
        if self._enc_stream is None:
            self._enc_stream = _shared_stream(self.device, "enc")
            self._enc_stream.wait_stream(torch.cuda.current_stream(self.device))
        return self._enc_stream

    @torch.no_grad()
    def encode_packed(self, img_bgr, wait=True):
        H0, W0 = img_bgr.shape[:2]
        h, w, _ = self._geometry(H0, W0)
        N = h * w

        def run():
            img = self._device_image(img_bgr)
            buf = torch.empty(N * 512, dtype=torch.float32, device=self.device)
            self.fnet_engine.forward(img, out=(buf[: N * 256].view(N, 256), None))
            self.cnet_engine.forward(img, out=(buf[N * 256: N * 384].view(N, 128), buf[N * 384:].view(N, 128)))
            return buf

        if self._enc_stream is None or torch.cuda.current_stream(self.device) == self._enc_stream:
            cur = torch.cuda.current_stream(self.device)
            self._encode_begin(cur)
            buf = run()
            self._encode_end(cur.record_event(), cur)
            return buf, (h, w)
        main = torch.cuda.current_stream(self.device)
        self._encode_begin(self._enc_stream)
        with torch.cuda.stream(self._enc_stream):
            buf = run()
            self._encode_end(self._enc_stream.record_event(), self._enc_stream)
        if wait:
            main.wait_stream(self._enc_stream)
            buf.record_stream(main)
        return buf, (h, w)

    @torch.no_grad()
    def encode_half(self, img_bgr, part, wait=True):
        H0, W0 = img_bgr.shape[:2]
        h, w, _ = self._geometry(H0, W0)
        N = h * w

        def run():
            img = self._device_image(img_bgr)
            buf = torch.empty(N * 256, dtype=torch.float32, device=self.device)
            if part == 0:
                self.fnet_engine.forward(img, out=(buf.view(N, 256), None))
            else:
                self.cnet_engine.forward(img, out=(buf[: N * 128].view(N, 128), buf[N * 128:].view(N, 128)))
            return buf

        if self._enc_stream is None or torch.cuda.current_stream(self.device) == self._enc_stream:
            cur = torch.cuda.current_stream(self.device)
            self._encode_begin(cur)
            buf = run()
            self._encode_end(cur.record_event(), cur)
            return buf, (h, w)
        main = torch.cuda.current_stream(self.device)
        self._encode_begin(self._enc_stream)
        with torch.cuda.stream(self._enc_stream):
            buf = run()
            self._encode_end(self._enc_stream.record_event(), self._enc_stream)
        if wait:
            main.wait_stream(self._enc_stream)
            buf.record_stream(main)
        return buf, (h, w)

    def adopt_halves(self, frame_id, fbuf, cbuf, img_bgr, ready=None):
        H0, W0 = img_bgr.shape[:2]
        h, w, pads = self._geometry(H0, W0)
        N = h * w
        assert fbuf.numel() == N * 256 and cbuf.numel() == N * 256
        fbuf, cbuf = fbuf.reshape(-1), cbuf.reshape(-1)
        self._frames[frame_id] = FrameFeatures(fbuf.view(N, 256), cbuf[: N * 128].view(N, 128), cbuf[N * 128:].view(N, 128),
                                               h, w, pads, (H0, W0), ready=ready)

    def packed_numel(self, img_bgr):
        h, w, _ = self._geometry(*img_bgr.shape[:2])
        return h * w * 512

    def adopt_packed(self, frame_id, buf, img_bgr, ready=None):
        H0, W0 = img_bgr.shape[:2]
        h, w, pads = self._geometry(H0, W0)
        N = h * w
        assert buf.numel() == N * 512
        buf = buf.reshape(-1)
        self._frames[frame_id] = FrameFeatures(buf[: N * 256].view(N, 256), buf[N * 256: N * 384].view(N, 128),
                                               buf[N * 384:].view(N, 128), h, w, pads, (H0, W0), ready=ready)

    def reset_cache(self):
        self._frames = {}

    def retain(self, frame_ids):
        keep = set(frame_ids)
        for k in [k for k in self._frames if k not in keep]:
            del self._frames[k]

    def _encode(self, img, prepare=False):
        if self._enc_stream is None:
            cur = torch.cuda.current_stream()
            self._encode_begin(cur)
            f = self.encode(img)
            if prepare:
                self._prepare(f)
            f.ready = cur.record_event()
            self._encode_end(f.ready, cur)
            return f
        main = torch.cuda.current_stream()
        if self._enc_waits_for_device_frames and isinstance(img, torch.Tensor) and img.is_cuda:
            self._encode_begin(main)
            f = self.encode(img)
            if prepare:
                self._prepare(f)
            f.ready = main.record_event()
            self._encode_end(f.ready, main)
            return f
        self._encode_begin(self._enc_stream)
        with torch.cuda.stream(self._enc_stream):
            f = self.encode(img)
            if prepare:
                self._prepare(f)
            f.ready = self._enc_stream.record_event()
        self._encode_end(f.ready, self._enc_stream)
        main.wait_stream(self._enc_stream)
        for t in f.tensors():
            t.record_stream(main)
        return f

    def _encode_begin(self, stream):
        prev = getattr(self, "_last_encode", None)
        if prev is not None and prev[1] != stream:
            stream.wait_event(prev[0])

    def _encode_end(self, event, stream):
        self._last_encode = (event, stream)

    def _features(self, key, img):
        if key is None:
            return self._encode(img)
        f = self._frames.get(key)
        if f is None or f.shape != img.shape[:2]:
            f = self._encode(img, prepare=True)
            self._frames[key] = f
        return f

    @torch.no_grad()
    def compute_pairs(self, pairs, iters=None, init_flow=None, packed_out=None, planar=True):
        iters = int(iters if iters is not None else self.C.flow_iters)
        fls = [self._features(lk, li) for lk, li, _, _ in pairs]
        frs = [self._features(rk, ri) for _, _, rk, ri in pairs]
        ref = fls[0]
        for f in fls + frs:
            if f.shape != ref.shape:
                raise ValueError("all frames of a batch must have the same size")
        P = len(pairs)
        gather = self.engine.can_gather(P) and not (self._split_streams > 1 and P >= 6 and init_flow is None)
        if gather:
            fmap1, fmap2 = [f.fmap for f in fls], [f.fmap for f in frs]
            net, inp = [f.net for f in fls], [f.inp for f in fls]
        else:
            fmap1 = torch.stack([f.fmap for f in fls])
            fmap2 = torch.stack([f.fmap for f in frs])
            net = torch.stack([f.net for f in fls])
            inp = torch.stack([f.inp for f in fls])
        flow_init = None
        if init_flow is not None:
            flow_init = self._init_flow_lr(init_flow, ref)
        packed = None
        H0, W0 = ref.shape
        want_planar = planar or packed_out is None or packed_out is False
        self._pin_kernels(ref.h, ref.w)
        prepared = self._prepared(fls, frs, flow_init) if gather else None
        if (self._fif > 1 and gather and flow_init is None and not self._check_finite
                and (packed_out is None or isinstance(packed_out, bool))):
            return self._refine_on_lane(fls, frs, fmap1, fmap2, net, inp, ref, iters, bool(packed_out), want_planar, prepared)
        if packed_out is not None and packed_out is not False:
            packed = packed_out if isinstance(packed_out, torch.Tensor) else \
                torch.empty(P, H0, W0, 4, dtype=torch.float32, device=self.device)
        self._pin_kernels(ref.h, ref.w)
        if self._lanes:
            for _, s_ in self._lanes:
                torch.cuda.current_stream(self.device).wait_stream(s_)
            self._lanes_stale = True
        if self._split_streams > 1 and P >= 6 and flow_init is None:
# ... 131 lines not shown
```

Before: 191.3 frames/s.

## Precompute fragment-ordered query maps per frame and XCD-local volume tile ordering

Adds a per-frame pre-pass that rearranges the split query feature map into the matrix-core fragment order, so the correlation-volume tile kernel can load operands directly instead of shuffling them in registers. It also adds a workgroup ordering for the volume kernel that groups tiles of the same pair onto the same XCD for L2 locality, exposed as options. Both are enabled by default through frame preparation. The cost is extra HBM per cached frame and one more conversion kernel per frame.

After: 192.3 frames/s (median of 6 runs). About the same (+0.5%).

```diff
diff --git a/include/mftx.h b/include/mftx.h
--- a/include/mftx.h
+++ b/include/mftx.h
@@ -116,6 +116,7 @@
 #define MFTX_RAFT_OPT_FUSE_OU 11
 #define MFTX_RAFT_OPT_TILE_CONV2P 12
 int mftx_raft_set_option(mftx_raft *r, int option, int value);
+int mftx_raft_set_volume_options(mftx_raft *r, int xcd_order, int fragments);
 #define MFTX_RAFT_PLAN_FIELDS 14
 #define MFTX_FLOW_FUSED 0
 #define MFTX_FLOW_SIDE 1
@@ -142,14 +143,23 @@
                             void *workspace, size_t workspace_bytes, void *stream);
 size_t mftx_raft_frame_prepare_bytes(int h, int w);
 int mftx_raft_frame_prepare(mftx_raft *r, int h, int w, const float *fmap, const float *inp, float *ctx_zr1, float *ctx_q1,
-                            float *ctx_zr2, float *ctx_q2, void *fmap_split, void *scratch, size_t scratch_bytes, void *stream);
+                            float *ctx_zr2, float *ctx_q2, void *fmap_split, void *fmap_frag, void *scratch, size_t scratch_bytes,
+                            void *stream);
 int mftx_raft_refine_gather_ex(mftx_raft *r, int P, int h, int w, int iters, const float *const *fmap1,
                                const float *const *fmap2, const float *const *net, const float *const *inp,
-                               const float *const *ctx_parts, const void *const *fmap1_split, const void *fmap2_split,
-                               const float *flow_init, int pad_left, int pad_right, int pad_top, int pad_bottom,
+                               const float *const *ctx_parts, const void *const *fmap1_split, const void *const *fmap1_frag,
+                               const void *fmap2_split, const float *flow_init, int pad_left, int pad_right, int pad_top, int pad_bottom,
                                float *flow, float *occl, float *sigma, float *packed, float *flow_lr_out,
                                void *workspace, size_t workspace_bytes, void *stream);
 int mftx_volume_query_split(const float *in, void *out, long long n_floats, void *stream);
+size_t mftx_volume_query_fragments_bytes(int n_rows);
+int mftx_volume_query_fragments(const void *split_rows, void *out, int n_rows, void *stream);
+int mftx_volume_query_fragments_host(const void *split_rows, void *out, int n_rows);
+int mftx_volume_tile_order(int P, int n_sb, int qchunks, int n_xcd, int *out);
+int mftx_volume_tile_xcds(int P, int n_sb, int qchunks, int cus);
+int mftx_corr_pyramid_gathered(const float *const *f1, const void *const *f1_split, const void *const *f1_frag, const void *f2_split,
+                               long long f2_pair_stride, int P, int h, int w, float *lvl0, float *lvl1, float *lvl2, float *lvl3, int xcd_order,
+                               int fragments, void *stream);
 
 typedef struct mftx_encoder mftx_encoder;
 int mftx_encoder_create(const float *const *weights, int n_weights, int instance_norm, mftx_encoder **out);
diff --git a/mft_amd/_lib.py b/mft_amd/_lib.py
--- a/mft_amd/_lib.py
+++ b/mft_amd/_lib.py
@@ -96,13 +96,20 @@
                                           C.c_void_p, C.c_void_p, C.c_void_p, C.c_void_p, C.c_void_p,
                                           C.c_void_p, C.c_size_t, C.c_void_p]),
     "mftx_raft_refine_gather_ex": (C.c_int, [C.c_void_p, C.c_int, C.c_int, C.c_int, C.c_int,
-                                             _PP, _PP, _PP, _PP, _PP, _PP, C.c_void_p, C.c_void_p,
+                                             _PP, _PP, _PP, _PP, _PP, _PP, _PP, C.c_void_p, C.c_void_p,
                                              C.c_int, C.c_int, C.c_int, C.c_int,
                                              C.c_void_p, C.c_void_p, C.c_void_p, C.c_void_p, C.c_void_p,
                                              C.c_void_p, C.c_size_t, C.c_void_p]),
     "mftx_raft_frame_prepare_bytes": (C.c_size_t, [C.c_int, C.c_int]),
-    "mftx_raft_frame_prepare": (C.c_int, [C.c_void_p, C.c_int, C.c_int] + [C.c_void_p] * 8 + [C.c_size_t, C.c_void_p]),
+    "mftx_raft_frame_prepare": (C.c_int, [C.c_void_p, C.c_int, C.c_int] + [C.c_void_p] * 9 + [C.c_size_t, C.c_void_p]),
     "mftx_volume_query_split": (C.c_int, [C.c_void_p, C.c_void_p, C.c_longlong, C.c_void_p]),
+    "mftx_volume_query_fragments_bytes": (C.c_size_t, [C.c_int]),
+    "mftx_volume_query_fragments": (C.c_int, [C.c_void_p, C.c_void_p, C.c_int, C.c_void_p]),
+    "mftx_volume_query_fragments_host": (C.c_int, [C.c_void_p, C.c_void_p, C.c_int]),
+    "mftx_volume_tile_order": (C.c_int, [C.c_int, C.c_int, C.c_int, C.c_int, C.POINTER(C.c_int)]),
+    "mftx_raft_set_volume_options": (C.c_int, [C.c_void_p, C.c_int, C.c_int]),
+    "mftx_volume_tile_xcds": (C.c_int, [C.c_int, C.c_int, C.c_int, C.c_int]),
+    "mftx_corr_pyramid_gathered": (C.c_int, [_PP, _PP, _PP, C.c_void_p, C.c_longlong, C.c_int, C.c_int, C.c_int] + [C.c_void_p] * 4 + [C.c_int, C.c_int, C.c_void_p]),
     "mftx_encoder_create": (C.c_int, [_PP, C.c_int, C.c_int, C.POINTER(C.c_void_p)]),
     "mftx_encoder_destroy": (None, [C.c_void_p]),
     "mftx_encoder_set_graph": (C.c_int, [C.c_void_p, C.c_int]),
diff --git a/mft_amd/csrc/common.h b/mft_amd/csrc/common.h
--- a/mft_amd/csrc/common.h
+++ b/mft_amd/csrc/common.h
@@ -114,9 +114,14 @@
 bool volume_tile_applicable(int C);
 constexpr int MFTX_MAX_GATHER = 16;
 struct PairPtrs { const float *p[MFTX_MAX_GATHER]; };
+enum { VT_Q_RAW = 0, VT_Q_SPLIT = 1, VT_Q_FRAG = 2 };
 int launch_volume_tile(const float *f1, const float *f2s, int P, int h, int w, float *const lvl[4], hipStream_t s,
-                       const PairPtrs *f1p = nullptr, long long f2_bstride = -1, bool f1_split = false);
+                       const PairPtrs *f1p = nullptr, long long f2_bstride = -1, int q_form = VT_Q_RAW, int xcd_order = 1);
+int launch_volume_tile_gathered(const PairPtrs *raw, const PairPtrs *split, const PairPtrs *frag, const float *f2s, long long f2_bstride, int P, int h,
+                                int w, float *const lvl[4], hipStream_t s, int xcd_order = 1, bool use_frag = true);
 int launch_volume_query_split(const float *in, void *out, long long n_floats, hipStream_t s);
+int launch_volume_query_fragments(const void *split_rows, void *out, long long n_rows, hipStream_t s);
+void volume_query_fragments_host(const void *split_rows, void *out, long long n_rows);
 int launch_corr_lookup(const float *const lvl[4], const float *coords, int P, int h, int w,
                        float *out, int ld_out, hipStream_t s);
 int launch_pack_lookup_convc1(const float *w, int ld_w, void *out, hipStream_t s);
diff --git a/mft_amd/csrc/raft_engine.hip b/mft_amd/csrc/raft_engine.hip
--- a/mft_amd/csrc/raft_engine.hip
+++ b/mft_amd/csrc/raft_engine.hip
@@ -2,6 +2,7 @@
 #include "profile.h"
 #include "motion_front.h"
 #include "graph_cache.h"
+#include "volume_order.h"
 #include <cstdlib>
 #include <new>
 
@@ -178,6 +179,7 @@
     const void *wou = nullptr, *wouproj = nullptr;
     int opt[13] = { -1,  1,  1,  1,  1,  1,  1,
                     1,  1,  1,  0,  1,  1};
+    int volume_xcd = 1, volume_frag = 1;
     unsigned *nonfinite = nullptr;
 };
 static_assert(MFTX_RAFT_OPT_TILE_CONV2P == 12, "mftx_raft::opt lists one default per option");
@@ -399,7 +401,7 @@
     return 0;
 }
 
-struct RefineGather { PairPtrs f1, f2, net, inp; bool f2_shared; bool has_ctx, has_f1s; PairPtrs ctx[4], f1s; const float *f2s; };
+struct RefineGather { PairPtrs f1, f2, net, inp; bool f2_shared; bool has_ctx, has_f1s, has_f1q; PairPtrs ctx[4], f1s, f1q; const float *f2s; };
 
 struct Coords { float *cur, *alt; bool pending; };
 struct Seg { const float *p; int ld, c; };
@@ -466,8 +468,8 @@
         if (gather->f2_shared && gather->f2s) f2s = gather->f2s;
         else if (gather->f2_shared) TRY(launch_split_weights(gather->f2.p[0], ws.f2s, pair_floats, s));
         else for (int b = 0; b < P; ++b) TRY(launch_split_weights(gather->f2.p[b], ws.f2s + b * pair_floats, pair_floats, s));
-        return launch_volume_tile(nullptr, f2s, P, h, w, ws.lvl, s, gather->has_f1s ? &gather->f1s : &gather->f1, gather->f2_shared ? 0 : pair_floats,
-                                  gather->has_f1s);
+        return launch_volume_tile_gathered(&gather->f1, gather->has_f1s ? &gather->f1s : nullptr, gather->has_f1q ? &gather->f1q : nullptr, f2s,
+                                           gather->f2_shared ? 0 : pair_floats, P, h, w, ws.lvl, s, r->volume_xcd, r->volume_frag != 0);
     }
     int init_state(const float *net, const float *inp, const float *flow_init, const RefineGather *gather) const {
         const int M = P * h * w;
@@ -685,14 +687,14 @@
                                        const float *flow_init, int pad_left, int pad_right, int pad_top, int pad_bottom,
                                        float *flow, float *occl, float *sigma, float *packed, float *flow_lr_out,
                                        void *workspace, size_t workspace_bytes, void *stream) {
-    return mftx_raft_refine_gather_ex(r, P, h, w, iters, fmap1, fmap2, net, inp, nullptr, nullptr, nullptr, flow_init, pad_left, pad_right, pad_top,
+    return mftx_raft_refine_gather_ex(r, P, h, w, iters, fmap1, fmap2, net, inp, nullptr, nullptr, nullptr, nullptr, flow_init, pad_left, pad_right, pad_top,
                                       pad_bottom, flow, occl, sigma, packed, flow_lr_out, workspace, workspace_bytes, stream);
 }
 
 extern "C" int mftx_raft_refine_gather_ex(mftx_raft *r, int P, int h, int w, int iters, const float *const *fmap1,
                                           const float *const *fmap2, const float *const *net, const float *const *inp,
-                                          const float *const *ctx_parts, const void *const *fmap1_split, const void *fmap2_split,
-                                          const float *flow_init, int pad_left, int pad_right, int pad_top, int pad_bottom,
+                                          const float *const *ctx_parts, const void *const *fmap1_split, const void *const *fmap1_frag,
+                                          const void *fmap2_split, const float *flow_init, int pad_left, int pad_right, int pad_top, int pad_bottom,
                                           float *flow, float *occl, float *sigma, float *packed, float *flow_lr_out,
                                           void *workspace, size_t workspace_bytes, void *stream) {
     if (!r || r->magic != RAFT_MAGIC) return fail(MFTX_E_STATE, "raft_refine_gather: bad handle");
@@ -721,6 +723,13 @@
         }
         g.has_f1s = true;
     }
+    if (fmap1_frag) {
+        for (int b = 0; b < P; ++b) {
+            if (!fmap1_frag[b] || !aligned16(fmap1_frag[b])) return fail(MFTX_E_ALIGN, "raft_refine_gather: fragment-ordered map of pair %d null or not 16-byte aligned", b);
+            g.f1q.p[b] = static_cast<const float *>(fmap1_frag[b]);
+        }
+        g.has_f1q = true;
+    }
     if (fmap2_split) {
         if (!aligned16(fmap2_split)) return fail(MFTX_E_ALIGN, "raft_refine_gather: the second map's split form must be 16-byte aligned");
         if (!g.f2_shared) return fail(MFTX_E_ARG, "raft_refine_gather: a split second map goes with ONE second map for all pairs");
@@ -743,12 +752,16 @@
     return ((size_t)h * w * 128 * sizeof(float) + 255) & ~size_t(255);
 }
 
+extern "C" size_t mftx_volume_query_fragments_bytes(int n_rows) { return n_rows > 0 ? (size_t)vt_frag_bytes(n_rows) : 0; }
+
 extern "C" int mftx_raft_frame_prepare(mftx_raft *r, int h, int w, const float *fmap, const float *inp, float *ctx_zr1, float *ctx_q1,
-                                       float *ctx_zr2, float *ctx_q2, void *fmap_split, void *scratch, size_t scratch_bytes, void *stream) {
+                                       float *ctx_zr2, float *ctx_q2, void *fmap_split, void *fmap_frag, void *scratch, size_t scratch_bytes,
+                                       void *stream) {
     if (!r || r->magic != RAFT_MAGIC) return fail(MFTX_E_STATE, "raft_frame_prepare: bad handle");
     if (h < 16 || w < 16 || (long long)h * w > (1ll << 24)) return fail(MFTX_E_ARG, "raft_frame_prepare: bad size");
     const bool want_ctx = ctx_zr1 || ctx_q1 || ctx_zr2 || ctx_q2;
     if (!want_ctx && !fmap_split) return fail(MFTX_E_ARG, "raft_frame_prepare: nothing to write");
+    if (fmap_frag && !fmap_split) return fail(MFTX_E_ARG, "raft_frame_prepare: the fragment-ordered map is made from the split map");
     if (r->arith != MFTX_ARITH_SPLIT || r->opt[MFTX_RAFT_OPT_PRESPLIT] == 0)
         return fail(MFTX_E_STATE, "raft_frame_prepare: needs the split arithmetic with split-form activations");
     hipStream_t s = (hipStream_t)stream;
@@ -756,6 +769,7 @@
     if (fmap_split) {
         if (!fmap) return fail(MFTX_E_ARG, "raft_frame_prepare: a split map needs fmap");
         TRY(launch_split_weights(fmap, fmap_split, N * 256, s));
+        if (fmap_frag) TRY(launch_volume_query_fragments(fmap_split, fmap_frag, N, s));
     }
     if (!want_ctx) return 0;
     if (!inp || !ctx_zr1 || !ctx_q1 || !ctx_zr2 || !ctx_q2 || !scratch) return fail(MFTX_E_ARG, "raft_frame_prepare: the context parts need inp, all four outputs and the scratch");
@@ -784,6 +798,57 @@
     return launch_volume_query_split(in, out, n_floats, (hipStream_t)stream);
 }
 
+extern "C" int mftx_volume_query_fragments(const void *split_rows, void *out, int n_rows, void *stream) {
+    if (!split_rows || !out) return fail(MFTX_E_ARG, "volume_query_fragments: null pointer");
+    return launch_volume_query_fragments(split_rows, out, n_rows, (hipStream_t)stream);
+}
+
+extern "C" int mftx_volume_query_fragments_host(const void *split_rows, void *out, int n_rows) {
+    if (!split_rows || !out || n_rows <= 0) return fail(MFTX_E_ARG, "volume_query_fragments_host: bad arguments");
+    volume_query_fragments_host(split_rows, out, n_rows);
+    return 0;
+}
+
+extern "C" int mftx_raft_set_volume_options(mftx_raft *r, int xcd_order, int fragments) {
+    if (!r || r->magic != RAFT_MAGIC) return fail(MFTX_E_STATE, "raft_set_volume_options: bad handle");
+    if (xcd_order < 0 || xcd_order > 2 || fragments < 0 || fragments > 1) return fail(MFTX_E_ARG, "raft_set_volume_options: xcd_order 0 .. 2, fragments 0 | 1");
+    r->volume_xcd = xcd_order; r->volume_frag = fragments;
+    return 0;
+}
+
+extern "C" int mftx_volume_tile_xcds(int P, int n_sb, int qchunks, int cus) {
+    if (P < 1 || n_sb < 1 || qchunks < 1 || cus < 1) { fail(MFTX_E_ARG, "volume_tile_xcds: need P, n_sb, qchunks, cus >= 1"); return -1; }
+    return vt_xcd_local_pays(P, (long long)P * n_sb * qchunks, cus) ? 8 : 1;
+}
+
+extern "C" int mftx_corr_pyramid_gathered(const float *const *f1, const void *const *f1_split, const void *const *f1_frag, const void *f2_split,
+                                          long long f2_pair_stride, int P, int h, int w, float *lvl0, float *lvl1, float *lvl2, float *lvl3, int xcd_order,
+                                          int fragments, void *stream) {
+    if (!f2_split || !lvl0 || !lvl1 || !lvl2 || !lvl3 || (!f1 && !f1_split && !f1_frag)) return fail(MFTX_E_ARG, "corr_pyramid_gathered: null pointer");
+    if (P < 1 || P > MFTX_MAX_GATHER || h < 8 || w < 8) return fail(MFTX_E_ARG, "corr_pyramid_gathered: need 1 .. %d pairs, h, w >= 8", MFTX_MAX_GATHER);
+    if (f2_pair_stride != 0 && f2_pair_stride != (long long)h * w * 256) return fail(MFTX_E_ARG, "corr_pyramid_gathered: second maps shared (0) or one after the other");
+    if (!aligned16(f2_split) || !aligned16(lvl0) || !aligned16(lvl1) || !aligned16(lvl2) || !aligned16(lvl3))
+        return fail(MFTX_E_ALIGN, "corr_pyramid_gathered: operands must be 16-byte aligned");
+    PairPtrs pp[3] = {};
+    const void *const *src[3] = {reinterpret_cast<const void *const *>(f1), f1_split, f1_frag};
+    for (int k = 0; k < 3; ++k)
+        for (int b = 0; src[k] && b < P; ++b) {
+            if (!src[k][b] || !aligned16(src[k][b])) return fail(MFTX_E_ALIGN, "corr_pyramid_gathered: query map of pair %d null or not 16-byte aligned", b);
+            pp[k].p[b] = static_cast<const float *>(src[k][b]);
+        }
+    float *const lv[4] = {lvl0, lvl1, lvl2, lvl3};
+    return launch_volume_tile_gathered(f1 ? &pp[0] : nullptr, f1_split ? &pp[1] : nullptr, f1_frag ? &pp[2] : nullptr, static_cast<const float *>(f2_split),
+                                       f2_pair_stride, P, h, w, lv, (hipStream_t)stream, xcd_order, fragments != 0);
+}
+
+extern "C" int mftx_volume_tile_order(int P, int n_sb, int qchunks, int n_xcd, int *out) {
+    if (P < 1 || n_sb < 1 || qchunks < 1 || n_xcd < 1 || !out) return fail(MFTX_E_ARG, "volume_tile_order: need P, n_sb, qchunks, n_xcd >= 1");
+    const long long total = (long long)P * n_sb * qchunks;
+    if (total > 0x7fffffffLL) return fail(MFTX_E_ARG, "volume_tile_order: too many workgroups");
+    for (long long wg = 0; wg < total; ++wg) vt_order((unsigned)wg, P, n_sb, qchunks, n_xcd, out[3 * wg], out[3 * wg + 1], out[3 * wg + 2]);
+    return 0;
+}
+
 extern "C" int mftx_raft_graph_stats(const mftx_raft *r, unsigned long long *captures, unsigned long long *replays) {
     if (!r || r->magic != RAFT_MAGIC || !captures || !replays) return fail(MFTX_E_STATE, "raft_graph_stats: bad arguments");
     *captures = r->graphs ? r->graphs->captures : 0;
diff --git a/mft_amd/csrc/volume_order.h b/mft_amd/csrc/volume_order.h
--- /dev/null
+++ b/mft_amd/csrc/volume_order.h
@@ -0,0 +1,39 @@
+#pragma once
+
+#if defined(__HIPCC__) || defined(__CUDACC__)
+#define MFTX_HD __host__ __device__
+#else
+#define MFTX_HD
+#endif
+
+namespace mftx {
+
+MFTX_HD inline unsigned vt_order_position(unsigned wg, unsigned total, unsigned n_xcd) {
+    if (n_xcd <= 1u || total <= n_xcd) return wg;
+    const unsigned x = wg % n_xcd, k = wg / n_xcd;
+    const unsigned per = total / n_xcd, rem = total % n_xcd;
+    return x * per + (x < rem ? x : rem) + k;
+}
+
+MFTX_HD inline void vt_order(unsigned wg, int P, int n_sb, int qchunks, int n_xcd, int &bz, int &sb, int &qc) {
+    const unsigned per_pair = (unsigned)n_sb * (unsigned)qchunks;
+    const unsigned pos = P > 1 ? vt_order_position(wg, (unsigned)P * per_pair, (unsigned)(n_xcd > 0 ? n_xcd : 1)) : wg;
+    qc = (int)(pos % (unsigned)qchunks);
+    sb = (int)((pos / (unsigned)qchunks) % (unsigned)n_sb);
+    bz = (int)(pos / per_pair);
+}
+
+MFTX_HD inline bool vt_xcd_local_pays(int P, long long total, int cus) { return P > 1 && total <= (long long)cus; }
+
+constexpr int VT_FRAG_ROWS = 32;
+constexpr int VT_FRAG_BLOCK = 32 * 1024;
+
+MFTX_HD inline long long vt_frag_bytes(long long n_rows) { return (n_rows + VT_FRAG_ROWS - 1) / VT_FRAG_ROWS * VT_FRAG_BLOCK; }
+
+MFTX_HD inline long long vt_frag_offset(long long row, int piece) {
+    const int c8 = piece >> 1, lo = piece & 1, g = c8 >> 1, hf = c8 & 1;
+    const int lane = (int)(row & 31) + 32 * hf;
+    return (row >> 5) * VT_FRAG_BLOCK + g * 2048 + lo * 1024 + lane * 16;
+}
+
+}
diff --git a/mft_amd/csrc/volume_tile.hip b/mft_amd/csrc/volume_tile.hip
--- a/mft_amd/csrc/volume_tile.hip
+++ b/mft_amd/csrc/volume_tile.hip
@@ -1,6 +1,8 @@
 #include "common.h"
 #include "profile.h"
 #include "device_prims.h"
+#include "volume_order.h"
+#include <cstring>
 
 namespace mftx {
 
@@ -8,6 +10,7 @@
 constexpr int VT_ROW = VT_C * 4 + 16;
 constexpr int VT_TARGETS = 128 * VT_ROW;
 constexpr int VT_LDS = VT_TARGETS + 8 * 1024;
+constexpr int VT_XCDS = 8;
 
 struct VolTileArgs {
     const float *f1;
@@ -19,6 +22,7 @@
     int qchunks, blocks_per_chunk;
     int ablate;
     int gathered;
+    int n_xcd;
     long long f2_bstride;
     PairPtrs f1p;
 };
@@ -32,13 +36,13 @@
     return __builtin_bit_cast(float, __builtin_amdgcn_update_dpp(0, __builtin_bit_cast(int, v), 0x110 + N, 0xf, 0xf, true));
 }
 
-template <bool QSPLIT>
+template <int QMODE>
 __global__ __launch_bounds__(512, 2) void volume_tile_kernel(VolTileArgs p) {
     extern __shared__ __attribute__((aligned(16))) unsigned char vt_lds[];
     unsigned char *lds = vt_lds;
     const int tid = (int)threadIdx.x, lane = tid & 63, wv = __builtin_amdgcn_readfirstlane(tid >> 6);
-    const int wg = (int)blockIdx.x;
-    const int qc = wg % p.qchunks, sb = (wg / p.qchunks) % p.n_sb, bz = wg / (p.qchunks * p.n_sb);
+    int bz, sb, qc;
+    vt_order((unsigned)blockIdx.x, p.P, p.n_sb, p.qchunks, p.n_xcd, bz, sb, qc);
     const int sby = sb / p.sbw, sbx = sb - sby * p.sbw;
     const float k2048 = __builtin_bit_cast(float, __builtin_amdgcn_readfirstlane(0x45000000));
 
@@ -70,15 +74,17 @@
     constexpr int PF = 3;
     f32x4 raw[PF][2];
     const float *f1base = p.gathered ? p.f1p.p[bz] : p.f1 + qbase * VT_C;
+    constexpr int GS = QMODE == VT_Q_FRAG ? 512 : 16, LO = QMODE == VT_Q_FRAG ? 256 : 4;
     auto row_of = [&](int qb) {
+        if constexpr (QMODE == VT_Q_FRAG) return f1base + (long long)qb * (VT_FRAG_BLOCK / 4) + 4 * lane;
         const int q = qb * 32 + (lane & 31);
         return f1base + (long long)(q < p.N ? q : p.N - 1) * VT_C + 8 * hf;
     };
     auto prefetch = [&](const float *src) {
 #pragma unroll
         for (int g = 0; g < PF; ++g) {
-            raw[g][0] = *reinterpret_cast<const f32x4 *>(src + 16 * g);
-            raw[g][1] = *reinterpret_cast<const f32x4 *>(src + 16 * g + 4);
+            raw[g][0] = *reinterpret_cast<const f32x4 *>(src + GS * g);
+            raw[g][1] = *reinterpret_cast<const f32x4 *>(src + GS * g + LO);
         }
     };
     if (b_lo + wv < b_hi) prefetch(row_of(b_lo + wv));
@@ -102,15 +108,15 @@
         for (int g = 0; g < 16; ++g) {
             const int set = g & 1;
             f16x8 bh, bl;
-            if constexpr (QSPLIT) {
+            if constexpr (QMODE != VT_Q_RAW) {
                 bh = __builtin_bit_cast(f16x8, raw[g % PF][0]);
                 bl = __builtin_bit_cast(f16x8, raw[g % PF][1]);
             } else split8(raw[g % PF][0], raw[g % PF][1], k2048, bh, bl);
             __builtin_amdgcn_sched_barrier(0);
             if (g + 1 < 16) read_a(g + 1, set ^ 1);
             if (g + PF < 16) {
-                raw[g % PF][0] = *reinterpret_cast<const f32x4 *>(src + 16 * (g + PF));
-                raw[g % PF][1] = *reinterpret_cast<const f32x4 *>(src + 16 * (g + PF) + 4);
+                raw[g % PF][0] = *reinterpret_cast<const f32x4 *>(src + GS * (g + PF));
+                raw[g % PF][1] = *reinterpret_cast<const f32x4 *>(src + GS * (g + PF) + LO);
             }
             __builtin_amdgcn_sched_barrier(0);
 #pragma unroll
@@ -262,8 +268,35 @@
     return check_launch("volume_query_split");
 }
 
+__global__ void vt_query_fragments_kernel(const uint4 *__restrict__ in, uint4 *__restrict__ out, long long n_rows, long long n_pieces) {
+    const long long i = (long long)blockIdx.x * blockDim.x + threadIdx.x;
+    if (i >= n_pieces) return;
+    const long long row = i >> 6;
+    const int piece = (int)(i & 63);
+    uint4 v = make_uint4(0u, 0u, 0u, 0u);
+    if (row < n_rows) v = in[i];
+    out[vt_frag_offset(row, piece) >> 4] = v;
+}
+
+int launch_volume_query_fragments(const void *split_rows, void *out, long long n_rows, hipStream_t s) {
+    if (n_rows <= 0 || n_rows > (1ll << 24)) return fail(MFTX_E_ARG, "volume_query_fragments: 1 .. 2^24 rows");
+    if (!aligned16(split_rows) || !aligned16(out)) return fail(MFTX_E_ALIGN, "volume_query_fragments: operands must be 16-byte aligned");
+    const long long n_pieces = vt_frag_bytes(n_rows) / 16;
+    hipLaunchKernelGGL(vt_query_fragments_kernel, dim3((unsigned)((n_pieces + 255) / 256)), dim3(256), 0, s, static_cast<const uint4 *>(split_rows),
+                       static_cast<uint4 *>(out), n_rows, n_pieces);
+    return check_launch("volume_query_fragments");
+}
+
+void volume_query_fragments_host(const void *split_rows, void *out, long long n_rows) {
+    const unsigned char *in = static_cast<const unsigned char *>(split_rows);
+    unsigned char *o = static_cast<unsigned char *>(out);
+    memset(o, 0, (size_t)vt_frag_bytes(n_rows));
+    for (long long row = 0; row < n_rows; ++row)
+        for (int piece = 0; piece < 64; ++piece) memcpy(o + vt_frag_offset(row, piece), in + (row * 64 + piece) * 16, 16);
+}
+
 int launch_volume_tile(const float *f1, const float *f2s, int P, int h, int w, float *const lvl[4], hipStream_t s, const PairPtrs *f1p, long long f2_bstride,
-                       bool f1_split) {
+                       int q_form, int xcd_order) {
     if (f1p && P > MFTX_MAX_GATHER) return fail(MFTX_E_ARG, "corr_pyramid: at most %d gathered pairs", MFTX_MAX_GATHER);
     const PyramidLayout L = pyramid_layout(h, w);
     VolTileArgs a{};
@@ -272,6 +305,7 @@
     a.P = P; a.N = h * w; a.h = h; a.w = w; a.sbw = L.sbw; a.n_sb = L.sbh * L.sbw; a.wb0 = L.wb[0];
     a.scale = 1.0f / sqrtf((float)VT_C);
     a.gathered = f1p ? 1 : 0;
+    if (q_form == VT_Q_FRAG && !f1p) return fail(MFTX_E_ARG, "corr_pyramid: fragment-ordered queries come per pair");
     if (f1p) a.f1p = *f1p;
     a.f2_bstride = f2_bstride >= 0 ? f2_bstride : (long long)a.N * VT_C;
     const int n_blocks = (a.N + 31) / 32;
@@ -284,18 +318,29 @@
     a.blocks_per_chunk = (n_blocks + qchunks - 1) / qchunks;
     a.qchunks = (n_blocks + a.blocks_per_chunk - 1) / a.blocks_per_chunk;
     const long long wgs = base * a.qchunks;
+    a.n_xcd = xcd_order == 0 ? 1 : (xcd_order == 2 || vt_xcd_local_pays(P, wgs, vt_num_cus()) ? VT_XCDS : 1);
     if (wgs > 0x7fffffffLL) return fail(MFTX_E_ARG, "corr_pyramid: too many workgroups");
     static bool attr_set = false;
     if (!attr_set) {
-        if (hipFuncSetAttribute(reinterpret_cast<const void *>(volume_tile_kernel<false>), hipFuncAttributeMaxDynamicSharedMemorySize, VT_LDS) != hipSuccess ||
-            hipFuncSetAttribute(reinterpret_cast<const void *>(volume_tile_kernel<true>), hipFuncAttributeMaxDynamicSharedMemorySize, VT_LDS) != hipSuccess)
+        if (hipFuncSetAttribute(reinterpret_cast<const void *>(volume_tile_kernel<VT_Q_RAW>), hipFuncAttributeMaxDynamicSharedMemorySize, VT_LDS) != hipSuccess ||
+            hipFuncSetAttribute(reinterpret_cast<const void *>(volume_tile_kernel<VT_Q_SPLIT>), hipFuncAttributeMaxDynamicSharedMemorySize, VT_LDS) != hipSuccess ||
+            hipFuncSetAttribute(reinterpret_cast<const void *>(volume_tile_kernel<VT_Q_FRAG>), hipFuncAttributeMaxDynamicSharedMemorySize, VT_LDS) != hipSuccess)
             return fail(MFTX_E_STATE, "corr_pyramid: cannot reserve %d bytes of LDS", VT_LDS);
         attr_set = true;
     }
     ProfScope prof(PC_CORR_VOLUME, s, 2.0 * a.N * a.N * (double)VT_C * P);
-    if (f1_split) hipLaunchKernelGGL(volume_tile_kernel<true>, dim3((unsigned)wgs), dim3(512), VT_LDS, s, a);
-    else hipLaunchKernelGGL(volume_tile_kernel<false>, dim3((unsigned)wgs), dim3(512), VT_LDS, s, a);
+    if (q_form == VT_Q_FRAG) hipLaunchKernelGGL(volume_tile_kernel<VT_Q_FRAG>, dim3((unsigned)wgs), dim3(512), VT_LDS, s, a);
+    else if (q_form == VT_Q_SPLIT) hipLaunchKernelGGL(volume_tile_kernel<VT_Q_SPLIT>, dim3((unsigned)wgs), dim3(512), VT_LDS, s, a);
+    else hipLaunchKernelGGL(volume_tile_kernel<VT_Q_RAW>, dim3((unsigned)wgs), dim3(512), VT_LDS, s, a);
     return check_launch("volume_tile");
 }
 
-}
+int launch_volume_tile_gathered(const PairPtrs *raw, const PairPtrs *split, const PairPtrs *frag, const float *f2s, long long f2_bstride, int P, int h,
+                                int w, float *const lvl[4], hipStream_t s, int xcd_order, bool use_frag) {
+    if (frag && !use_frag) frag = split || raw ? nullptr : frag;
+    if (!frag && !split && !raw) return fail(MFTX_E_ARG, "corr_pyramid: no query maps");
+    return launch_volume_tile(nullptr, f2s, P, h, w, lvl, s, frag ? frag : split ? split : raw, f2_bstride, frag ? VT_Q_FRAG : split ? VT_Q_SPLIT : VT_Q_RAW,
+                              xcd_order);
+}
+
+}
diff --git a/mft_amd/ops.py b/mft_amd/ops.py
--- a/mft_amd/ops.py
+++ b/mft_amd/ops.py
@@ -1074,6 +1074,7 @@
     GEMM_SLOTS = (0, 2, 6, 8, 10, 11, 13, 14, 16, 17, 19, 20, 22, 26, 28, 30)
 
     OPTIONS = {"fork": 0, "presplit": 1, "group": 2, "fuse_lookup": 3, "graph": 4, "fuse_flow": 5, "tile_conv": 6, "fuse_head": 7, "tile_volume": 8, "fuse_gru": 9, "tile_cells": 10, "fuse_ou": 11, "tile_conv2p": 12}
+    VOLUME_OPTIONS = ("volume_xcd", "volume_frag")
     TILE_SLOTS = {2: (192, 256), 8: (128, 256), 10: (256, 256), 11: (256, 128), 13: (128, 256), 14: (128, 128), 16: (256, 256),
                   17: (256, 128), 19: (128, 256), 20: (128, 128), 22: (256, 128), 26: (256, 128)}
 
@@ -1174,6 +1175,12 @@
         copy_bytes(self._nonfinite, host_words)
 
     def set_option(self, name, value):
+        if name in self.VOLUME_OPTIONS:
+            cur = getattr(self, "_volume_options", {"volume_xcd": 1, "volume_frag": 1})
+            cur[name] = int(value)
+            check(_lib.load().mftx_raft_set_volume_options(self._h, cur["volume_xcd"], cur["volume_frag"]), "mftx_raft_set_volume_options")
+            self._volume_options = cur
+            return
         if name not in self.OPTIONS:
             raise MftxError(f"unknown engine option {name!r} (known: {', '.join(sorted(self.OPTIONS))}, gather)")
         check(_lib.load().mftx_raft_set_option(self._h, self.OPTIONS[name], int(value)), "mftx_raft_set_option")
@@ -1214,22 +1221,26 @@
         return (self.arith == ARITH_SPLIT and not self.ondemand_corr and P <= self.MAX_GATHER and
                 getattr(self, "_tile_volume", 1) != 0 and getattr(self, "_gather", True))
 
-    def prepare_frame(self, fmap, inp, h, w, context=True, split=True):
+    def prepare_frame(self, fmap, inp, h, w, context=True, split=True, fragments=False):
         lib = _lib.load()
         N = h * w
         dev = self.device
-        ctx = fsplit = scratch = None
+        ctx = fsplit = ffrag = scratch = None
+        if fragments and not split:
+            raise MftxError("prepare_frame: fragments=True goes with split=True")
         if context:
             ctx = tuple(torch.empty(N, c, dtype=torch.float32, device=dev) for c in (256, 128, 256, 128))
             scratch = torch.empty(lib.mftx_raft_frame_prepare_bytes(h, w), dtype=torch.uint8, device=dev)
         if split:
             fsplit = torch.empty(N, 256, dtype=torch.float32, device=dev)
+        if fragments:
+            ffrag = torch.empty(lib.mftx_volume_query_fragments_bytes(N), dtype=torch.uint8, device=dev)
         cp = [t.data_ptr() for t in ctx] if context else [None] * 4
         check(lib.mftx_raft_frame_prepare(self._h, h, w, _chk(fmap, "fmap") if split else None, _chk(inp, "inp") if context else None,
-                                          *cp, fsplit.data_ptr() if split else None,
+                                          *cp, fsplit.data_ptr() if split else None, ffrag.data_ptr() if fragments else None,
                                           scratch.data_ptr() if context else None, scratch.numel() if context else 0, _stream()),
               "mftx_raft_frame_prepare")
-        return ctx, fsplit
+        return (ctx, fsplit, ffrag) if fragments else (ctx, fsplit)
 
     def refine(self, fmap1, fmap2, net, inp, h, w, iters, pads=(0, 0, 0, 0), want_flow_lr=False, flow_init=None,
                packed=None, planar=True, prepared=None):
@@ -1264,11 +1275,16 @@
             maps = [a[0] for a in arrs]
             if prepared:
                 ctx, f1s, f2s = prepared.get("ctx"), prepared.get("f1s"), prepared.get("f2s")
-                if (ctx is not None and len(ctx) != P) or (f1s is not None and len(f1s) != P):
+                f1q = prepared.get("f1q")
+                if (ctx is not None and len(ctx) != P) or (f1s is not None and len(f1s) != P) or (f1q is not None and len(f1q) != P):
                     raise MftxError("refine: prepared parts for every pair, or none")
                 carr = _lib.ptr_array([_chk(t, "context part") for parts in ctx for t in parts]) if ctx is not None else (None, None)
                 sarr = _lib.ptr_array([_chk(t, "split map") for t in f1s]) if f1s is not None else (None, None)
-                check(lib.mftx_raft_refine_gather_ex(self._h, P, h, w, iters, *maps, carr[0], sarr[0],
+                need = lib.mftx_volume_query_fragments_bytes(h * w)
+                if f1q is not None and any(t.dtype != torch.uint8 or t.numel() != need for t in f1q):
+                    raise MftxError(f"refine: a fragment-ordered map of {h} x {w} cells is {need} bytes of uint8")
+                qarr = _lib.ptr_array([_chk(t, "fragment-ordered map", dtype=torch.uint8) for t in f1q]) if f1q is not None else (None, None)
+                check(lib.mftx_raft_refine_gather_ex(self._h, P, h, w, iters, *maps, carr[0], sarr[0], qarr[0],
                                                      _chk(f2s, "split map") if f2s is not None else None, *tail()),
                       "mftx_raft_refine_gather_ex")
             else:
diff --git a/mft_amd/raft.py b/mft_amd/raft.py
--- a/mft_amd/raft.py
+++ b/mft_amd/raft.py
@@ -34,16 +34,17 @@
 
 
 class FrameFeatures:
-    __slots__ = ("fmap", "net", "inp", "h", "w", "pads", "shape", "ready", "ctx", "fsplit")
+    __slots__ = ("fmap", "net", "inp", "h", "w", "pads", "shape", "ready", "ctx", "fsplit", "ffrag")
 
     def __init__(self, fmap, net, inp, h, w, pads, shape, ready=None):
         self.fmap, self.net, self.inp, self.h, self.w, self.pads, self.shape = fmap, net, inp, h, w, pads, shape
         self.ready = ready
         self.ctx = None
         self.fsplit = None
+        self.ffrag = None
 
     def tensors(self):
-        return [t for t in (self.fmap, self.net, self.inp, self.fsplit) + tuple(self.ctx or ()) if t is not None]
+        return [t for t in (self.fmap, self.net, self.inp, self.fsplit, self.ffrag) + tuple(self.ctx or ()) if t is not None]
 
 
 class RAFTWrapper:
@@ -66,6 +67,10 @@
             raise ValueError(f"raft_params.arith must be 'split' or 'fp32', got {arith!r}")
         self._arith = ops.ARITH_SPLIT if arith == "split" else ops.ARITH_F32
         self._engine_options = dict(getattr(getattr(config, "raft_params", None), "engine_options", None) or {})
+        for env, opt in (("MFTX_VT_XCD_ORDER", "volume_xcd"), ("MFTX_VT_FRAGMENTS", "volume_frag")):
+            v = os.environ.get(env, "")
+            if v and opt not in self._engine_options:
+                self._engine_options[opt] = int(v)
         try:
             self._build_engines()
         except ops.SplitRangeError as e:
@@ -132,7 +137,7 @@
         self._pin_kernels(f.h, f.w)
         fits = self._prepare_ok.get((f.h, f.w))
         if fits is None:
-            per_frame = f.h * f.w * 4096
+            per_frame = f.h * f.w * 4096 + int(ops._lib.load().mftx_volume_query_fragments_bytes(f.h * f.w))
             need = self.PREPARED_FRAMES * per_frame
             ws_bytes = int(ops._lib.load().mftx_raft_workspace_bytes_for(self.engine._h, self.nominal_pairs, f.h, f.w))
             for k in range(self._fif):
@@ -148,7 +153,7 @@
         if not fits:
             return
         context = getattr(self.engine, "_tile_conv", 1) == 2 and int(opt.get("fuse_gru", 1)) != 0
-        f.ctx, f.fsplit = self.engine.prepare_frame(f.fmap, f.inp, f.h, f.w, context=context, split=True)
+        f.ctx, f.fsplit, f.ffrag = self.engine.prepare_frame(f.fmap, f.inp, f.h, f.w, context=context, split=True, fragments=True)
 
     def _prepared(self, fls, frs, flow_init):
         if not self._frame_prepare or flow_init is not None:
@@ -156,9 +161,10 @@
         ctx = [f.ctx for f in fls] if all(f.ctx is not None for f in fls) and getattr(self.engine, "_tile_conv", 1) == 2 else None
         f1s = [f.fsplit for f in fls] if all(f.fsplit is not None for f in fls) else None
         f2s = frs[0].fsplit if all(f is frs[0] for f in frs) else None
+        f1q = [f.ffrag for f in fls] if all(f.ffrag is not None for f in fls) else None
         if ctx is None and f1s is None and f2s is None:
             return None
-        return {"ctx": ctx, "f1s": f1s, "f2s": f2s}
+        return {"ctx": ctx, "f1s": f1s, "f1q": f1q, "f2s": f2s}
 
     def _all_engines(self):
         return list(dict.fromkeys([self.engine] + list(self._engines) + [e for e, _ in self._lanes]))
```
